# thilinarmtb/lsbench

Hardware: AMD Instinct MI355X
Metric: cg_solves_per_sec (higher is better)
Workload: dtype f64

## Files before the change

### include/lsbench_hip.h

```cpp
#ifndef LSBENCH_HIP_H
#define LSBENCH_HIP_H

#include "lsbench.h"
#include <stddef.h>

#ifdef __cplusplus
extern "C" {
#endif


struct lsbench {
  char *matrix;
  lsbench_solver_t solver;
  lsbench_ordering_t ordering;
  lsbench_precision_t precision;
  unsigned verbose, trials;
};

struct csr {
  unsigned nrows, base;
  unsigned *offs, *cols;
  double *vals;
};

// ... 200 lines not shown
void lsb_amg_free(struct lsb_amg_hier *h);
#define LSB_AMG_MCGS_COLOURS 16
int *lsb_amg_colour(const struct csr *A, unsigned *ncolours);
struct lsb_mcgs {
  unsigned n, ncolours;
  unsigned *cbeg;
  unsigned *rowid;
  unsigned *offs;
  unsigned *cols;
  double *vals;
};
struct lsb_mcgs *lsb_csr_mcgs(const struct csr *A, const int *colour, unsigned ncolours);
void lsb_mcgs_free(struct lsb_mcgs *M);
int lsb_mcgs_check(const struct csr *A, const int *colour, const struct lsb_mcgs *M, char *why, size_t whylen);
unsigned long long *lsb_csr_pack_f32(const struct csr *A);
#define LSB_SELL_ROWS 128
struct lsb_sell {
  unsigned nrows, nslice;
  unsigned long long stored;
  unsigned *sptr;
  int *cols;
  double *vals;
  short *codes;
  int *sbase;
  unsigned ncode_slots;
};
unsigned long long lsb_csr_sell_stored(const struct csr *A);
struct lsb_sell *lsb_csr_sellize(const struct csr *A);
struct lsb_sell *lsb_csr_sellize16(const struct csr *A, unsigned row_begin);
void lsb_sell_free(struct lsb_sell *S);
struct lsb_sell_vc {
  unsigned long long nslots;
  unsigned nval_slots;
  int *slots;
  double *vconst;
  double *vals;
};
struct lsb_sell_vc *lsb_sell16_value_slots(const struct lsb_sell *S);
void lsb_sell_vc_free(struct lsb_sell_vc *V);
#define LSB_TMPL_SLOTS 8
struct lsb_sell_tmpl {
  int nslots;
  int shaped;
  int base[LSB_TMPL_SLOTS];
  int kidx[LSB_TMPL_SLOTS];
  int kind[LSB_TMPL_SLOTS];
  int pad_[2];
  double cst[LSB_TMPL_SLOTS];
};
struct lsb_sell_tmpls {
  unsigned nslice, ntmpl, nfar;
  unsigned long long covered, shaped;
  unsigned long long nmask;
  unsigned long long kept_read;
  unsigned char *tid;
  unsigned *vbase;
  unsigned long long *mask;
  struct lsb_sell_tmpl *t;
};
struct lsb_sell_tmpls *lsb_sell16_templates(const struct lsb_sell *S, const struct lsb_sell_vc *V);
void lsb_sell_tmpls_free(struct lsb_sell_tmpls *T);
int lsb_tmpl_check(const struct lsb_sell *S, const struct lsb_sell_vc *V, const struct lsb_sell_tmpls *T,
                   unsigned row_begin, unsigned nrows, unsigned xlen, int deep, char *why, size_t whylen);
#define LSB_TMPL_COL_MAX 16
#define LSB_TMPL_COL_GRID(nfar) ((nfar) >= 2 ? 768u : 1280u)
#define LSB_TMPL_COL_TURN(nfar) (4u * LSB_TMPL_COL_GRID(nfar) / 8u)
#define LSB_SELL_GRID 1536u
#define LSB_TMPL_COL_DOWN 9
#define LSB_TMPL_COL_LOCKSTEP 0x80000000u
struct lsb_tmpl_cols {
  unsigned nitem, kmax, period;
  unsigned s_lo, s_hi;
  unsigned xbeg[9];
  unsigned *item;
  unsigned long long in_cols;
  int centre0;
  unsigned *down;
};
struct lsb_tmpl_cols *lsb_sell_tmpl_columns(const struct lsb_sell_tmpls *T, unsigned period, unsigned kmax);
struct lsb_tmpl_cols *lsb_sell_tmpl_columns_range(const struct lsb_sell_tmpls *T, unsigned period, unsigned kmax,
                                                  unsigned s_lo, unsigned s_hi);
void lsb_tmpl_cols_free(struct lsb_tmpl_cols *C);
int lsb_tmpl_cols_check(const struct lsb_sell_tmpls *T, const struct lsb_tmpl_cols *C, char *why, size_t whylen);
double lsb_csr_mean_scatter(const struct csr *A, unsigned row_begin);
void lsb_csr_col_hull(const struct csr *A, unsigned *lo, unsigned *hi);
struct lsb_xfer {
  int peer;
  size_t offset, count;
};
void lsb_plan_exchange(int me, int nall, const unsigned *hull,
                       struct lsb_xfer *recv, int *nrecv,
                       struct lsb_xfer *send, int *nsend);
struct csr *lsbench_matrix_synth(const char *spec, unsigned r0, unsigned r1,
                                 unsigned *n_global);


typedef struct lsb_hip_solver lsb_hip_solver;

lsb_hip_solver *lsb_hip_solver_create(const struct csr *A,
                                      const struct lsb_hip_opts *o);
lsb_hip_solver *lsb_hip_solver_create_dist(const struct csr *A_rows,
                                           unsigned row_begin,
                                           unsigned n_global,
                                           const struct lsb_hip_opts *o);
void lsb_hip_solver_destroy(lsb_hip_solver *s);

int lsb_hip_solver_solve(lsb_hip_solver *s, const double *b, double *x,
                         struct lsb_hip_result *res);
int lsb_hip_solver_solve_dev(lsb_hip_solver *s, const double *d_b, double *d_x,
                             struct lsb_hip_result *res);
int lsb_hip_solver_solve_x0(lsb_hip_solver *s, const double *b, double *x,
                            struct lsb_hip_result *res);
int lsb_hip_solver_solve_x0_dev(lsb_hip_solver *s, const double *d_b, double *d_x,
                                struct lsb_hip_result *res);
int lsb_hip_solver_start_relres(const lsb_hip_solver *s, unsigned nrhs, double *out);
int lsb_hip_solver_spmv_dev(lsb_hip_solver *s, const double *d_x, double *d_y);
int lsb_hip_solver_spmv_inner_dev(lsb_hip_solver *s, const double *d_x, double *d_y, double *d_dot);
int lsb_hip_solver_precond_dev(lsb_hip_solver *s, const double *d_r, double *d_z);
int lsb_hip_solver_amg_info(lsb_hip_solver *s, unsigned *levels, unsigned *tail_levels);
int lsb_hip_solver_amg_cheb_interval(lsb_hip_solver *s, unsigned level, double *lo, double *hi);
int lsb_hip_solver_amg_colours(lsb_hip_solver *s, unsigned level, unsigned *ncolours);
int lsb_hip_solver_amg_precision(lsb_hip_solver *s);
unsigned long long lsb_hip_solver_amg_cycle_bytes(const lsb_hip_solver *s);
int lsb_hip_solver_direct_info(const lsb_hip_solver *s, unsigned long long *entries, unsigned *height,
                               unsigned long long *bytes_per_round);
int lsb_hip_solver_cheb_interval(const lsb_hip_solver *s, double *lmin, double *lmax);
int lsb_hip_solver_time_spmv(lsb_hip_solver *s, int warm, int reps,
                             double *ms_avg);
int lsb_hip_solver_jacobi_sweep_dev(lsb_hip_solver *s, double w,
                                    const double *d_b, double *d_x);

int lsb_hip_solver_spmm_dev(lsb_hip_solver *s, unsigned nrhs, const double *d_X, size_t ldx,
                            double *d_Y, size_t ldy);
int lsb_hip_solver_solve_multi_dev(lsb_hip_solver *s, unsigned nrhs, const double *d_B, size_t ldb,
                                   double *d_X, size_t ldx, struct lsb_hip_result *res);
int lsb_hip_solver_solve_multi(lsb_hip_solver *s, unsigned nrhs, const double *B, size_t ldb,
                               double *X, size_t ldx, struct lsb_hip_result *res);
int lsb_hip_solver_solve_multi_x0_dev(lsb_hip_solver *s, unsigned nrhs, const double *d_B, size_t ldb,
                                      double *d_X, size_t ldx, struct lsb_hip_result *res);
unsigned long long lsb_hip_solver_multi_iteration_bytes(const lsb_hip_solver *s, unsigned nrhs);
int lsb_hip_solver_fsai_nnz(const lsb_hip_solver *s, unsigned long long *g, unsigned long long *gt);
int lsb_hip_solver_precond_multi_dev(lsb_hip_solver *s, unsigned nrhs, const double *d_R, size_t ldr,
                                     double *d_Z, size_t ldz);

int lsb_hip_solver_solve_direct_multi_dev(lsb_hip_solver *s, unsigned nrhs, const double *d_B, size_t ldb,
                                          double *d_X, size_t ldx, struct lsb_hip_result *res);
int lsb_hip_solver_solve_direct_multi(lsb_hip_solver *s, unsigned nrhs, const double *B, size_t ldb,
                                      double *X, size_t ldx, struct lsb_hip_result *res);
int lsb_hip_solver_direct_apply_multi_dev(lsb_hip_solver *s, unsigned nrhs, const double *d_R, size_t ldr,
                                          double *d_Z, size_t ldz);
unsigned long long lsb_hip_solver_direct_multi_round_bytes(const lsb_hip_solver *s, unsigned nrhs);

int lsb_hip_solver_amg_solve_multi_dev(lsb_hip_solver *s, unsigned nrhs, const double *d_B, size_t ldb,
                                       double *d_X, size_t ldx, struct lsb_hip_result *res);
int lsb_hip_solver_amg_solve_multi(lsb_hip_solver *s, unsigned nrhs, const double *B, size_t ldb,
                                   double *X, size_t ldx, struct lsb_hip_result *res);
int lsb_hip_solver_amg_cycle_multi_dev(lsb_hip_solver *s, unsigned nrhs, const double *d_R, size_t ldr,
                                       double *d_Z, size_t ldz);
unsigned long long lsb_hip_solver_amg_solve_multi_bytes(const lsb_hip_solver *s, unsigned nrhs);

int lsb_hip_solver_solve_block_dev(lsb_hip_solver *s, unsigned nrhs, const double *d_B, size_t ldb,
                                   double *d_X, size_t ldx, struct lsb_hip_result *res);
int lsb_hip_solver_solve_block(lsb_hip_solver *s, unsigned nrhs, const double *B, size_t ldb,
                               double *X, size_t ldx, struct lsb_hip_result *res);
unsigned long long lsb_hip_solver_block_iteration_bytes(const lsb_hip_solver *s, unsigned nrhs);
int lsb_hip_solver_block_norms(const lsb_hip_solver *s, unsigned nrhs, double *rr, double *bb);
// ... 79 lines not shown
```

### lsbench_amd/_lib.py

```python
import ctypes as C
import os
import subprocess

_CSRC = os.path.join(os.path.dirname(os.path.abspath(__file__)), "csrc")
LIB_PATH = os.path.join(_CSRC, "liblsbench_hip.so")
CORE_PATH = os.path.join(_CSRC, "liblsbench_core.so")
CORE_SYMBOLS = ("lsbench_matrix_read", "lsbench_matrix_print", "lsbench_matrix_free", "lsbench_init",
                "lsbench_get_matrix_name", "lsbench_bench", "lsbench_finalize")

UNIQUE_ID_BYTES = 128

SOLVER_HIP = 6
OP_CHOLMOD_UPPER, OP_RAW = 0, 1
PRECOND_JACOBI, PRECOND_NONE, PRECOND_L1JACOBI, PRECOND_CHEBYSHEV, PRECOND_BLOCKJACOBI, PRECOND_FSAI = 0, 1, 2, 3, 4, 5
PRECOND_AMG = 6
AMG_SMOOTH_L1JACOBI, AMG_SMOOTH_CHEB, AMG_SMOOTH_MCGS = 0, 1, 2
AMG_PREC_FP64, AMG_PREC_FP32 = 0, 1
KRYLOV_PCG, KRYLOV_GMRES, KRYLOV_PCG1, KRYLOV_AUTO, KRYLOV_BICGSTAB, KRYLOV_RICHARDSON = 0, 1, 2, 3, 4, 5
KRYLOV_DIRECT = 6
DIRECT_MAX_ENTRIES = 1 << 28
SPMV_AUTO, SPMV_ADAPTIVE, SPMV_SUBWAVE, SPMV_SCALAR, SPMV_PANEL, SPMV_SELL, SPMV_BINNED, SPMV_TWOPHASE = 0, 1, 2, 3, 4, 5, 6, 7
SELL_ROWS = 128
BIN_CHUNK = 2048
PB_COLS, PB_ROWS = 8192, 2048
# ... 33 lines not shown
                ("amg_theta", C.c_double), ("amg_sweeps", C.c_int), ("amg_coarse", C.c_int),
                ("amg_max_levels", C.c_int), ("amg_tail_rows", C.c_int),
                ("amg_precision", C.c_int),
                ("amg_smoother", C.c_int), ("amg_cheb_ratio", C.c_double)]
    _TAIL = {"fsai_blocks": (0, C.c_int)}
    _TAIL_BYTES = 8

    def __init__(self, *args, **kw):
        super().__init__(*args, **kw)
        C.resize(self, C.sizeof(type(self)) + self._TAIL_BYTES)
        C.memset(C.addressof(self) + C.sizeof(type(self)), 0, self._TAIL_BYTES)

    def _tail(self, name):
        off, ctype = self._TAIL[name]
        return ctype.from_address(C.addressof(self) + C.sizeof(type(self)) + off)

    fsai_blocks = property(lambda self: self._tail("fsai_blocks").value,
                           lambda self, v: setattr(self._tail("fsai_blocks"), "value", v))


class Result(C.Structure):
    _fields_ = [("iters", C.c_uint), ("status", C.c_int), ("relres", C.c_double),
                ("seconds", C.c_double), ("spmv_ms", C.c_double),
                ("spmv_samples", C.c_uint), ("corrections", C.c_uint),
                ("true_relres", C.c_double), ("spmvs", C.c_uint)]


class PanelCsr(C.Structure):
    _fields_ = [("npanels", C.c_uint), ("width", C.c_uint), ("npairs", C.c_uint),
                ("nrows", C.c_uint), ("pair_begin", C.POINTER(C.c_uint)),
                ("pair_row", C.POINTER(C.c_uint)), ("offs", C.POINTER(C.c_uint)),
                ("cols", C.POINTER(C.c_uint)), ("vals", C.POINTER(C.c_double))]


class Sell(C.Structure):
    _fields_ = [("nrows", C.c_uint), ("nslice", C.c_uint), ("stored", C.c_ulonglong),
                ("sptr", C.POINTER(C.c_uint)), ("cols", C.POINTER(C.c_int)),
                ("vals", C.POINTER(C.c_double)), ("codes", C.POINTER(C.c_short)),
                ("sbase", C.POINTER(C.c_int)), ("ncode_slots", C.c_uint)]


class SellVc(C.Structure):
    _fields_ = [("nslots", C.c_ulonglong), ("nval_slots", C.c_uint), ("slots", C.POINTER(C.c_int)),
                ("vconst", C.POINTER(C.c_double)), ("vals", C.POINTER(C.c_double))]


class FsaiPattern(C.Structure):
    _fields_ = [("n", C.c_uint), ("cap", C.c_uint), ("nnz", C.c_ulonglong), ("offs", C.POINTER(C.c_uint)),
                ("cols", C.POINTER(C.c_uint))]


class AmgLevel(C.Structure):
    _fields_ = [("n", C.c_uint), ("A", C.POINTER(CsrStruct)), ("P", C.POINTER(CsrStruct)),
                ("R", C.POINTER(CsrStruct))]


class AmgHier(C.Structure):
    _fields_ = [("nlev", C.c_uint), ("lv", C.POINTER(AmgLevel)), ("nc", C.c_uint),
                ("coarse_inv", C.POINTER(C.c_double))]


class Mcgs(C.Structure):
    _fields_ = [("n", C.c_uint), ("ncolours", C.c_uint), ("cbeg", C.POINTER(C.c_uint)),
                ("rowid", C.POINTER(C.c_uint)), ("offs", C.POINTER(C.c_uint)), ("cols", C.POINTER(C.c_uint)),
                ("vals", C.POINTER(C.c_double))]


class Skyinv(C.Structure):
    _fields_ = [("n", C.c_uint), ("perm", C.POINTER(C.c_uint)), ("first", C.POINTER(C.c_uint)),
                ("woff", C.POINTER(C.c_ulonglong)), ("vals", C.POINTER(C.c_double)),
                ("parent", C.POINTER(C.c_uint)), ("run_end", C.POINTER(C.c_uint))]


class SellTmpl(C.Structure):
    _fields_ = [("nslots", C.c_int), ("shaped", C.c_int), ("base", C.c_int * 8), ("kidx", C.c_int * 8),
                ("kind", C.c_int * 8), ("pad_", C.c_int * 2), ("cst", C.c_double * 8)]


class SellTmpls(C.Structure):
    _fields_ = [("nslice", C.c_uint), ("ntmpl", C.c_uint), ("nfar", C.c_uint), ("covered", C.c_ulonglong),
                ("shaped", C.c_ulonglong), ("nmask", C.c_ulonglong), ("kept_read", C.c_ulonglong),
                ("tid", C.POINTER(C.c_ubyte)), ("vbase", C.POINTER(C.c_uint)),
                ("mask", C.POINTER(C.c_ulonglong)), ("t", C.POINTER(SellTmpl))]


class TmplCols(C.Structure):
    _fields_ = [("nitem", C.c_uint), ("kmax", C.c_uint), ("period", C.c_uint), ("s_lo", C.c_uint), ("s_hi", C.c_uint),
                ("xbeg", C.c_uint * 9),
                ("item", C.POINTER(C.c_uint)), ("in_cols", C.c_ulonglong), ("centre0", C.c_int),
                ("down", C.POINTER(C.c_uint))]


class Binned(C.Structure):
    _fields_ = [("nbins", C.c_uint), ("width", C.c_uint), ("nrows", C.c_uint), ("nchunks", C.c_uint),
                ("chunk_cap", C.c_uint), ("nnz", C.c_ulonglong), ("bin_chunk", C.POINTER(C.c_uint)),
                ("chunk_begin", C.POINTER(C.c_uint)), ("rows", C.POINTER(C.c_uint)),
                ("cols", C.POINTER(C.c_uint)), ("vals", C.POINTER(C.c_double))]


class Pb(C.Structure):
    _fields_ = [("nrows", C.c_uint), ("ncols_lo", C.c_uint), ("nchunks", C.c_uint), ("nbins", C.c_uint),
                ("nitems", C.c_uint), ("npieces", C.c_uint), ("cols", C.c_uint), ("rows", C.c_uint),
                ("nnz", C.c_ulonglong), ("nent", C.c_ulonglong),
                ("vals", C.POINTER(C.c_double)), ("colw", C.POINTER(C.c_ushort)),
                ("grp_first", C.POINTER(C.c_uint)), ("grp_mask", C.POINTER(C.c_ulonglong)),
                ("delta", C.POINTER(C.c_uint)), ("item", C.POINTER(C.c_uint)),
                ("bin_ptr", C.POINTER(C.c_uint)), ("roww", C.POINTER(C.c_ushort))]


class Xfer(C.Structure):
    _fields_ = [("peer", C.c_int), ("offset", C.c_size_t), ("count", C.c_size_t)]


_vp, _u, _i, _d = C.c_void_p, C.c_uint, C.c_int, C.c_double
_csrp = C.POINTER(CsrStruct)

SIGNATURES = {
    "lsbench_matrix_read": (_csrp, [C.c_char_p]),
    "lsbench_matrix_print": (None, [_csrp]),
    "lsbench_matrix_free": (None, [_csrp]),
    "lsbench_init": (C.POINTER(LsbenchStruct), [_i, C.POINTER(C.c_char_p)]),
    "lsbench_get_matrix_name": (C.c_char_p, [C.POINTER(LsbenchStruct)]),
    "lsbench_bench": (None, [_csrp, C.POINTER(LsbenchStruct)]),
    "lsbench_finalize": (None, [C.POINTER(LsbenchStruct)]),
    "hip_cdna4_init": (_i, []),
    "hip_cdna4_finalize": (_i, []),
    "hip_cdna4_bench": (_i, [C.POINTER(C.c_double), _csrp, C.POINTER(C.c_double),
                             C.POINTER(LsbenchStruct)]),
    "lsb_hip_opts_default": (None, [C.POINTER(Opts)]),
    "lsb_hip_set_opts": (None, [C.POINTER(Opts)]),
    "lsb_hip_get_opts": (None, [C.POINTER(Opts)]),
    "lsb_hip_last_result": (None, [C.POINTER(Result)]),
    "lsb_hip_device_count": (_i, []),
    "lsb_csr_free": (None, [_csrp]),
    "lsb_csr_symmetrize_upper": (_csrp, [_csrp]),
    "lsb_csr_copy_base0": (_csrp, [_csrp]),
    "lsb_csr_row_slice": (_csrp, [_csrp, _u, _u]),
    "lsb_csr_partition_rows": (_i, [_csrp, _u, C.POINTER(_u)]),
    "lsb_csr_row_blocks": (_u, [_csrp, _u, C.POINTER(C.POINTER(_u))]),
    "lsb_csr_block_lanes": (None, [_csrp, C.POINTER(_u), _u, C.POINTER(C.c_ubyte)]),
    "lsb_csr_rcm": (_i, [_csrp, C.POINTER(_u)]),
    "lsb_csr_nd": (_i, [_csrp, C.POINTER(_u)]),
    "lsb_csr_nd_bounded": (_i, [_csrp, C.POINTER(_u), C.c_ulonglong, C.POINTER(C.c_ulonglong)]),
    "lsb_csr_skyline_count": (C.c_ulonglong, [_csrp, C.POINTER(_u), C.POINTER(_u)]),
    "lsb_csr_skyline_inverse": (C.POINTER(Skyinv), [_csrp, C.POINTER(_u), C.POINTER(_i)]),
    "lsb_skyinv_free": (None, [C.POINTER(Skyinv)]),
    "lsb_csr_permute_sym": (_csrp, [_csrp, C.POINTER(_u)]),
    "lsb_csr_bandwidth": (_u, [_csrp]),
    "lsb_csr_panelize": (C.POINTER(PanelCsr), [_csrp, _u]),
    "lsb_panel_csr_free": (None, [C.POINTER(PanelCsr)]),
    "lsb_csr_pbize": (C.POINTER(Pb), [_csrp]),
    "lsb_csr_pbize2": (C.POINTER(Pb), [_csrp, _u, _u]),
    "lsb_pb_free": (None, [C.POINTER(Pb)]),
    "lsb_pb_check": (_i, [C.POINTER(Pb), C.c_ulonglong, C.c_ulonglong, _i, C.c_char_p, C.c_size_t]),
    "lsb_csr_binize": (C.POINTER(Binned), [_csrp, _u]),
    "lsb_binned_free": (None, [C.POINTER(Binned)]),
    "lsb_csr_sell_stored": (C.c_ulonglong, [_csrp]),
    "lsb_csr_sellize": (C.POINTER(Sell), [_csrp]),
    "lsb_csr_sellize16": (C.POINTER(Sell), [_csrp, _u]),
    "lsb_sell_free": (None, [C.POINTER(Sell)]),
    "lsb_sell16_value_slots": (C.POINTER(SellVc), [C.POINTER(Sell)]),
    "lsb_sell_vc_free": (None, [C.POINTER(SellVc)]),
    "lsb_csr_fsai_pattern": (C.POINTER(FsaiPattern), [_csrp, _i, _u]),
    "lsb_fsai_pattern_free": (None, [C.POINTER(FsaiPattern)]),
    "lsb_amg_setup": (C.POINTER(AmgHier), [_csrp, _d, _u, _u]),
    "lsb_amg_aggregate": (C.POINTER(C.c_int), [_csrp, _d, C.POINTER(_u)]),
    "lsb_amg_free": (None, [C.POINTER(AmgHier)]),
    "lsb_amg_gershgorin": (_d, [_csrp]),
    "lsb_csr_pack_f32": (C.POINTER(C.c_ulonglong), [_csrp]),
    "lsb_amg_cheb_coeffs": (None, [_d, _d, _u, C.POINTER(_d), C.POINTER(_d)]),
    "lsb_amg_colour": (C.POINTER(C.c_int), [_csrp, C.POINTER(_u)]),
    "lsb_csr_mcgs": (C.POINTER(Mcgs), [_csrp, C.POINTER(C.c_int), _u]),
    "lsb_mcgs_free": (None, [C.POINTER(Mcgs)]),
    "lsb_mcgs_check": (_i, [_csrp, C.POINTER(C.c_int), C.POINTER(Mcgs), C.c_char_p, C.c_size_t]),
    "lsb_sell16_templates": (C.POINTER(SellTmpls), [C.POINTER(Sell), C.POINTER(SellVc)]),
    "lsb_sell_tmpls_free": (None, [C.POINTER(SellTmpls)]),
    "lsb_tmpl_check": (_i, [C.POINTER(Sell), C.POINTER(SellVc), C.POINTER(SellTmpls), _u, _u, _u, _i,
                            C.c_char_p, C.c_size_t]),
    "lsb_sell_tmpl_columns": (C.POINTER(TmplCols), [C.POINTER(SellTmpls), _u, _u]),
    "lsb_sell_tmpl_columns_range": (C.POINTER(TmplCols), [C.POINTER(SellTmpls), _u, _u, _u, _u]),
    "lsb_tmpl_cols_free": (None, [C.POINTER(TmplCols)]),
    "lsb_tmpl_cols_check": (_i, [C.POINTER(SellTmpls), C.POINTER(TmplCols), C.c_char_p, C.c_size_t]),
    "lsb_csr_mean_scatter": (_d, [_csrp, _u]),
    "lsb_csr_col_hull": (None, [_csrp, C.POINTER(_u), C.POINTER(_u)]),
    "lsb_plan_exchange": (None, [_i, _i, C.POINTER(_u), C.POINTER(Xfer), C.POINTER(_i),
                                 C.POINTER(Xfer), C.POINTER(_i)]),
    "lsbench_matrix_synth": (_csrp, [C.c_char_p, _u, _u, C.POINTER(_u)]),
    "lsb_hip_solver_create": (_vp, [_csrp, C.POINTER(Opts)]),
    "lsb_hip_solver_create_dist": (_vp, [_csrp, _u, _u, C.POINTER(Opts)]),
    "lsb_hip_solver_destroy": (None, [_vp]),
    "lsb_hip_solver_solve": (_i, [_vp, _vp, _vp, C.POINTER(Result)]),
    "lsb_hip_solver_solve_dev": (_i, [_vp, _vp, _vp, C.POINTER(Result)]),
    "lsb_hip_solver_solve_x0": (_i, [_vp, _vp, _vp, C.POINTER(Result)]),
    "lsb_hip_solver_solve_x0_dev": (_i, [_vp, _vp, _vp, C.POINTER(Result)]),
    "lsb_hip_solver_start_relres": (_i, [_vp, _u, C.POINTER(C.c_double)]),
    "lsb_hip_solver_spmv_dev": (_i, [_vp, _vp, _vp]),
    "lsb_hip_solver_spmv_inner_dev": (_i, [_vp, _vp, _vp, _vp]),
    "lsb_hip_solver_spmm_dev": (_i, [_vp, _u, _vp, C.c_size_t, _vp, C.c_size_t]),
    "lsb_hip_solver_solve_multi_dev": (_i, [_vp, _u, _vp, C.c_size_t, _vp, C.c_size_t, C.POINTER(Result)]),
    "lsb_hip_solver_solve_multi": (_i, [_vp, _u, _vp, C.c_size_t, _vp, C.c_size_t, C.POINTER(Result)]),
    "lsb_hip_solver_solve_multi_x0_dev": (_i, [_vp, _u, _vp, C.c_size_t, _vp, C.c_size_t, C.POINTER(Result)]),
    "lsb_hip_solver_multi_iteration_bytes": (C.c_ulonglong, [_vp, _u]),
    "lsb_hip_solver_solve_block_dev": (_i, [_vp, _u, _vp, C.c_size_t, _vp, C.c_size_t, C.POINTER(Result)]),
    "lsb_hip_solver_solve_block": (_i, [_vp, _u, _vp, C.c_size_t, _vp, C.c_size_t, C.POINTER(Result)]),
    "lsb_hip_solver_block_iteration_bytes": (C.c_ulonglong, [_vp, _u]),
    "lsb_hip_solver_block_norms": (_i, [_vp, _u, C.POINTER(C.c_double), C.POINTER(C.c_double)]),
    "lsb_hip_solver_solve_block_precond_dev": (_i, [_vp, _u, _vp, C.c_size_t, _vp, C.c_size_t, C.POINTER(Result)]),
    "lsb_hip_solver_solve_block_precond": (_i, [_vp, _u, _vp, C.c_size_t, _vp, C.c_size_t, C.POINTER(Result)]),
    "lsb_hip_solver_block_precond_iteration_bytes": (C.c_ulonglong, [_vp, _u]),
    "lsb_hip_solver_precond_multi_dev": (_i, [_vp, _u, _vp, C.c_size_t, _vp, C.c_size_t]),
    "lsb_hip_solver_fsai_nnz": (_i, [_vp, C.POINTER(C.c_ulonglong), C.POINTER(C.c_ulonglong)]),
    "lsb_hip_solver_precond_dev": (_i, [_vp, _vp, _vp]),
    "lsb_hip_solver_amg_info": (_i, [_vp, C.POINTER(_u), C.POINTER(_u)]),
    "lsb_hip_solver_amg_precision": (_i, [_vp]),
    "lsb_hip_solver_amg_cycle_bytes": (C.c_ulonglong, [_vp]),
    "lsb_hip_solver_direct_info": (_i, [_vp, C.POINTER(C.c_ulonglong), C.POINTER(_u), C.POINTER(C.c_ulonglong)]),
    "lsb_hip_solver_solve_direct_multi_dev": (_i, [_vp, _u, _vp, C.c_size_t, _vp, C.c_size_t, C.POINTER(Result)]),
    "lsb_hip_solver_solve_direct_multi": (_i, [_vp, _u, _vp, C.c_size_t, _vp, C.c_size_t, C.POINTER(Result)]),
    "lsb_hip_solver_direct_apply_multi_dev": (_i, [_vp, _u, _vp, C.c_size_t, _vp, C.c_size_t]),
    "lsb_hip_solver_direct_multi_round_bytes": (C.c_ulonglong, [_vp, _u]),
    "lsb_hip_solver_amg_solve_multi_dev": (_i, [_vp, _u, _vp, C.c_size_t, _vp, C.c_size_t, C.POINTER(Result)]),
    "lsb_hip_solver_amg_solve_multi": (_i, [_vp, _u, _vp, C.c_size_t, _vp, C.c_size_t, C.POINTER(Result)]),
    "lsb_hip_solver_amg_cycle_multi_dev": (_i, [_vp, _u, _vp, C.c_size_t, _vp, C.c_size_t]),
    "lsb_hip_solver_amg_solve_multi_bytes": (C.c_ulonglong, [_vp, _u]),
    "lsb_hip_solver_amg_cheb_interval": (_i, [_vp, _u, C.POINTER(_d), C.POINTER(_d)]),
    "lsb_hip_solver_amg_colours": (_i, [_vp, _u, C.POINTER(_u)]),
    "lsb_hip_solver_cheb_interval": (_i, [_vp, C.POINTER(_d), C.POINTER(_d)]),
    "lsb_hip_solver_time_spmv": (_i, [_vp, _i, _i, C.POINTER(_d)]),
    "lsb_hip_solver_jacobi_sweep_dev": (_i, [_vp, _d, _vp, _vp]),
    "lsb_hip_solver_nrows_local": (_u, [_vp]),
    "lsb_hip_solver_padded": (_i, [_vp]),
    "lsb_hip_solver_slab_mask": (_u, [_vp]),
    "lsb_csr_pad_lines": (_csrp, [_csrp, _u, C.POINTER(_u), C.POINTER(_u), C.POINTER(C.POINTER(C.c_int))]),
    "lsb_hip_solver_nrows_global": (_u, [_vp]),
    "lsb_hip_solver_nnz_local": (C.c_ulonglong, [_vp]),
    "lsb_hip_solver_nblocks": (_u, [_vp]),
    "lsb_hip_solver_spmv_variant": (_i, [_vp]),
    "lsb_hip_solver_spmv_flags": (_u, [_vp]),
    "lsb_hip_solver_spmv_grid": (_u, [_vp]),
    "lsb_hip_solver_spmv_period": (_u, [_vp]),
    "lsb_hip_solver_spmv_col_slices": (C.c_ulonglong, [_vp]),
    "lsb_hip_solver_sell_value_slots": (None, [_vp, C.POINTER(C.c_uint), C.POINTER(C.c_uint)]),
    "lsb_hip_solver_overlaps": (_i, [_vp]),
    "lsb_hip_solver_overlap": (_i, [_vp, C.POINTER(C.c_double)]),
    "lsb_hip_solver_comm_plan": (None, [_vp, C.POINTER(C.c_ulonglong)]),
    "lsb_hip_solver_spmv_layout_bytes": (C.c_ulonglong, [_vp]),
    "lsb_hip_solver_fused_p": (_i, [_vp]),
    "lsb_hip_solver_iteration_bytes": (C.c_ulonglong, [_vp]),
    "lsb_hip_solver_single_reduction": (_i, [_vp]),
    "lsb_hip_solver_blas1_nt": (_i, [_vp]),
    "lsb_hip_solver_comm": (_i, [_vp, C.POINTER(C.c_double), C.POINTER(C.c_double)]),
    "lsb_hip_stream": (_vp, []),
    "lsb_hip_comm_get_unique_id": (_i, [_vp]),
    "lsb_hip_comm_init_rank": (_i, [_vp, _i, _i]),
    "lsb_hip_comm_destroy": (_i, []),
    "lsb_hip_comm_rank": (_i, []),
    "lsb_hip_comm_size": (_i, []),
    "lsb_hip_comm_count": (_i, []),
    "hip_cdna4_set_option": (_i, [C.c_char_p, C.c_char_p]),
    "hip_cdna4_matrix_synth": (_csrp, [C.c_char_p]),
    "lsb_hip_comm_allreduce_sum_dev": (_i, [_vp, _i]),
    "lsb_hip_comm_barrier": (_i, []),
    "lsb_hip_spmv_csr_f64": (_i, [_i, _u, _vp, _vp, _vp, _vp, _vp, _u, _u, _u, _vp, _vp,
                                  _vp, _vp, _vp, _vp]),
    "lsb_hip_partials_capacity": (_u, []),
    "lsb_hip_dot_f64": (_i, [_u, _vp, _vp, _vp, _vp, _vp]),
    "lsb_hip_nrm2_f64": (_i, [_u, _vp, _vp, _vp, _vp]),
    "lsb_hip_axpy_f64": (_i, [_u, _vp, _vp, _vp, _vp]),
    "lsb_hip_xpay_f64": (_i, [_u, _vp, _vp, _vp, _vp]),
    "lsb_hip_jacobi_setup_f64": (_i, [_u, _u, _vp, _vp, _vp, _vp, _vp, _vp]),
    "lsb_hip_jacobi_apply_f64": (_i, [_u, _vp, _vp, _vp, _vp]),
    "lsb_hip_malloc": (_vp, [C.c_size_t]),
    "lsb_hip_free": (None, [_vp]),
    "lsb_hip_memcpy_h2d": (_i, [_vp, _vp, C.c_size_t]),
    "lsb_hip_memcpy_d2h": (_i, [_vp, _vp, C.c_size_t]),
    "lsb_hip_sync": (_i, []),
}

_LIB = None


def build(force=False):
    if force:
        subprocess.run(["make", "-s", "-C", _CSRC, "clean"], check=True)
    subprocess.run(["make", "-s", "-C", _CSRC, "all"], check=True)


def libc_free(ptr):
    libc = C.CDLL(None)
    libc.free.argtypes, libc.free.restype = [C.c_void_p], None
    libc.free(C.cast(ptr, C.c_void_p))


def load():
    global _LIB
    if _LIB is not None:
        return _LIB
    try:
        import torch
    except Exception:
        pass
    if not os.path.exists(LIB_PATH):
        raise LsbenchHipError(
            "%s not built: run `make -C lsbench_amd/csrc` or __graft_entry__.build(); "
            "there is no fallback path" % LIB_PATH)
    hip = C.CDLL(LIB_PATH, mode=C.RTLD_GLOBAL)
    core = C.CDLL(CORE_PATH, mode=C.RTLD_GLOBAL)

    class _Both:
        pass
    lib = _Both()
    lib.hip, lib.core = hip, core
    for name, (res, args) in SIGNATURES.items():
        fn = getattr(core if name in CORE_SYMBOLS else hip, name)
        fn.restype, fn.argtypes = res, args
        setattr(lib, name, fn)
# ... 11 lines not shown
```

### lsbench_amd/csrc/hip_kernels.hip

```cpp
#include "hip_kcommon.h"

__device__ __forceinline__ void spmv_publish(double *__restrict__ partials, double dot,
                                             double *sred, const lsb_ar_tail &tail) {
  if (!partials)
    return;
  double d[1] = {dot};
  wg_sum<1>(d, sred);
  if (tail.counter)
    ar_tail(partials, d[0], tail);
  else if (threadIdx.x == 0)
    partials[blockIdx.x] = d[0];
}

enum { SP_PREFETCH = 1, SP_NT = 2 };

template <int FLAGS, class T>
__device__ __forceinline__ T stream_load(const T *p) {
  if (FLAGS & SP_NT)
    return __builtin_nontemporal_load(p);
  return *p;
}

#define LSB_ISSUE_BLOCK(kk)                                                    \
  do {                                                                         \
// ... 1272 lines not shown
      const lsb_sell_tmpl *T = td + t;
      col_tmpl<NF> C;
      C.bc = T->base[NF + 1];
      C.k0 = T->cst[0], C.kc = T->cst[NF + 1], C.kL = T->cst[2 * NF + 2];
#pragma unroll
      for (int k = 0; k < NF - 1; k++) {
        C.bl[k] = T->base[1 + k], C.bh[k] = T->base[NF + 3 + k];
        C.kl[k] = T->cst[1 + k], C.kh[k] = T->cst[NF + 3 + k];
      }
      const int side_k[2] = {T->kidx[NF], T->kidx[NF + 2]}, side_kd[2] = {T->kind[NF], T->kind[NF + 2]};
      const bool down = col_walks_down(plan, dofs, it);
      const unsigned s0 = down ? s + (K - 1) * period : s;
      const long long D = down ? -(long long)P : (long long)P;
      const unsigned Du = (unsigned)D;
      long long gu = (long long)s0 * LSB_SELL_ROWS;
      unsigned lrow = s0 * LSB_SELL_ROWS;
      col_ops<NF> cur, nxt;
      sell_d2u cb = *(const sell_d2u *)(p + (gu + C.bc - D) + 2 * lane);
      sell_d2u c0 = *(const sell_d2u *)(p + (gu + C.bc) + 2 * lane);
      sell_d2u ca, cn;
      col_issue<NF, 2>(cur, ca, C, p, r, gu, lrow, D, n, lane, true);
      unsigned long long mk[2][2] = {{0ull, 0ull}, {0ull, 0ull}};
#pragma unroll
      for (int side = 0; side < 2; side++)
        if (side_k[side] >= 0 && side_kd[side] == 2) {
          const unsigned long long *mp = mask + 2 * ((size_t)mb + (unsigned)side_k[side]);
          mk[side][0] = mp[0], mk[side][1] = mp[1];
        }
      double vm0 = T->cst[NF], vm1 = vm0, vp0 = T->cst[NF + 2], vp1 = vp0;
      if (side_k[0] >= 0 || side_k[1] >= 0)
        tmpl_side_values(T, NF, 0u, lane, side_k, side_kd, mk, vals, 0, vm0, vm1, vp0, vp1);
      for (unsigned k = 0; k + 1 < K; k++) {
        col_issue<NF, 2>(nxt, cn, C, p, r, gu + D, lrow + Du, D, n, lane, true);
        double a0, a1;
        col_compute<NF, 0>(cur, down ? ca : cb, c0, down ? cb : ca, C, vm0, vm1, vp0, vp1, lane, a0, a1, nodot);
        COLR_FINISH(a0, a1, cur.xd, lrow);
        cb = c0, c0 = ca, ca = cn, cur = nxt;
        gu += D, lrow += Du;
      }
      double a0, a1;
      col_compute<NF, 0>(cur, down ? ca : cb, c0, down ? cb : ca, C, vm0, vm1, vp0, vp1, lane, a0, a1, nodot);
      COLR_FINISH(a0, a1, cur.xd, lrow);
    } else {
      for (unsigned k = 0; k < K; k++) {
        const unsigned sl = s + k * period, row = sl * LSB_SELL_ROWS + 2 * lane;
        const unsigned q0 = sptr[sl] / LSB_SELL_ROWS, len = (sptr[sl + 1] - sptr[sl]) / LSB_SELL_ROWS;
        const bool l0 = row < n, l1 = row + 1 < n;
        const double r0 = l0 ? r[row] : 0.0, r1 = l1 ? r[row + 1] : 0.0;
        double a0 = 0.0, a1 = 0.0;
        for (unsigned j = 0; j < len; j++) {
          const i4v rec2 = ((const i4v *)sbase)[q0 + j];
          if (rec2.z < 0) {
            const double kk = vconst[q0 + j];
            const sell_d2u pv = *(const sell_d2u *)(p + ((int)row + rec2.x));
            a0 = fma(kk, pv.x, a0), a1 = fma(kk, pv.y, a1);
          } else {
            const sell_d2v v = *((const sell_d2v *)(vals + (size_t)rec2.z * LSB_SELL_ROWS) + lane);
            const bool p0 = v.x != 0.0, p1 = v.y != 0.0;
            const double t0 = p[p0 ? (int)row + rec2.x : 0], t1 = p[p1 ? (int)row + 1 + rec2.x : 0];
            a0 = fma(v.x, p0 ? t0 : 0.0, a0), a1 = fma(v.y, p1 ? t1 : 0.0, a1);
          }
        }
        if (l0) {
          const double rn0 = r0 - alpha * a0;
          r[row] = rn0;
          acc[0] += rn0 * (dc * rn0), acc[1] += rn0 * rn0;
        }
        if (l1) {
          const double rn1 = r1 - alpha * a1;
          r[row + 1] = rn1;
          acc[0] += rn1 * (dc * rn1), acc[1] += rn1 * rn1;
        }
      }
    }
  }
#undef COLR_FINISH
  wg_sum<2>(acc, sred);
  if (threadIdx.x == 0) {
    partials2[2 * blockIdx.x + 0] = acc[0];
    partials2[2 * blockIdx.x + 1] = acc[1];
  }
}


__device__ __forceinline__ unsigned bin_pad(unsigned i) { return i + (i >> 3); }

template <int FLAGS, int BIN_U>
__global__ __launch_bounds__(WG) void k_spmv_binned(
    const unsigned *__restrict__ chunk_begin, unsigned nchunk, const unsigned *__restrict__ rows,
    const unsigned *__restrict__ cols, const double *__restrict__ vals,
    const double *__restrict__ x, double *__restrict__ y, const lsb_pcg_state *__restrict__ st) {
  constexpr unsigned CHUNK = BIN_U * WG;
  __shared__ double sprod[CHUNK + CHUNK / 8 + 8];
  __shared__ unsigned skey[CHUNK + CHUNK / 8 + 8];
  __shared__ double swv[4];
  __shared__ int swf[4];
  __shared__ double sred[4];
  const unsigned tid = threadIdx.x, lane = tid & 63u, wave = tid >> 6;
  const unsigned per = gridDim.x / NXCD;
  const unsigned w = (blockIdx.x % NXCD) * per + blockIdx.x / NXCD;
  if (w >= nchunk)
    return;
  const unsigned e0 = chunk_begin[w], cnt = chunk_begin[w + 1] - e0;
  unsigned r[BIN_U], c[BIN_U];
  double v[BIN_U];
  if (cnt <= CHUNK) {
#pragma unroll
    for (int u = 0; u < BIN_U; u++) {
      const unsigned t = tid + u * WG;
      if (t < cnt) {
        r[u] = stream_load<FLAGS>(rows + e0 + t);
        c[u] = stream_load<FLAGS>(cols + e0 + t);
        v[u] = stream_load<FLAGS>(vals + e0 + t);
      }
    }
  }
  if (st && st->status)
    return;
  if (cnt > CHUNK) {
    double s[1] = {0.0};
    for (unsigned j = e0 + tid; j < e0 + cnt; j += WG)
      s[0] += vals[j] * x[cols[j]];
    wg_sum<1>(s, sred);
    if (tid == 0)
      y[rows[e0]] += s[0];
    return;
  }
#pragma unroll
  for (int u = 0; u < BIN_U; u++) {
    const unsigned t = tid + u * WG;
    if (t < cnt) {
      double xv;
      if (FLAGS & 8)
        xv = __hip_atomic_load(x + c[u], __ATOMIC_RELAXED, __HIP_MEMORY_SCOPE_AGENT);
      else if (FLAGS & 16)
        xv = __builtin_nontemporal_load(x + c[u]);
      else
        xv = x[c[u]];
      sprod[bin_pad(t)] = v[u] * xv;
      skey[bin_pad(t)] = r[u];
    }
  }
  __syncthreads();
  const unsigned i0 = tid * BIN_U;
  const int nloc = i0 < cnt ? (int)min(cnt - i0, (unsigned)BIN_U) : 0;
  double first_sum = 0.0, acc = 0.0;
  unsigned first_key = 0, prevk = 0xFFFFFFFFu, nextk = 0xFFFFFFFEu;
  bool cont = false, has_boundary = false, closes = true;
  unsigned ok_[BIN_U];
  double ov[BIN_U];
  unsigned omask = 0;
  if (nloc > 0) {
    if (i0 > 0)
      prevk = skey[bin_pad(i0 - 1)];
    if (i0 + BIN_U < cnt)
      nextk = skey[bin_pad(i0 + BIN_U)];
    unsigned k[BIN_U + 1];
    double p[BIN_U];
#pragma unroll
    for (int j = 0; j < BIN_U; j++) {
      k[j] = j < nloc ? skey[bin_pad(i0 + j)] : 0u;
      p[j] = j < nloc ? sprod[bin_pad(i0 + j)] : 0.0;
    }
    cont = k[0] == prevk;
    first_key = k[0];
#pragma unroll
// ... 214 lines not shown
      if (epi.zout)
        kern = nt ? k_spmv_sell16<SP_NT, VT, true> : k_spmv_sell16<0, VT, true>;
      kern<<<L.g, WG, 0, s>>>(sptr, s0, ns, L.period, n, row_begin, xlen, (const short *)cols, sbase, v, vconst,
                              ulen, x, y, xdot, partials, st, L.tail, epi);
    } else {
      const auto kern = nt ? k_spmv_sell<SP_NT, VT> : k_spmv_sell<0, VT>;
      kern<<<L.g, WG, 0, s>>>(sptr, s0, ns, L.period, n, (const int *)cols, v, x, y, xdot, partials, st, L.tail);
    }
  };
  if (flags & LSB_SP_F32)
    launch((const float *)(const void *)vals);
  else
    launch(vals);
}

void lsb_k_spmv_tmpl(unsigned flags, unsigned grid_cap, unsigned period, const struct lsb_sell16_dev *c, unsigned s0,
                     unsigned ns, unsigned n, unsigned row_begin, unsigned xlen, const double *x, double *y,
                     const double *xdot, double *partials, unsigned *npartials, const struct lsb_pcg_state *st,
                     const struct lsb_ar_tail *tail_in, const struct lsb_cheb_epi *epi_in, void *stream) {
  const lsb_cheb_epi epi = epi_for(epi_in, partials || ((row_begin | s0) & 1u),
                                   "lsb_k_spmv_tmpl: the Chebyshev epilogue takes no dot and even row offsets");
  const sell_launch L = sell_prologue("lsb_k_spmv_tmpl", false, c, ns, n, grid_cap, 0, period, partials, npartials,
                                      tail_in);
  const int f32 = (flags & LSB_SP_F32) != 0, dot_is_x = xdot && xdot == x + row_begin;
  static decltype(&k_spmv_tmpl<0, false>) const kern[3][3] = {
      {k_spmv_tmpl<0, false>, k_spmv_tmpl<0, true>, k_spmv_tmpl<0, false, true>},
      {k_spmv_tmpl<1, false>, k_spmv_tmpl<1, true>, k_spmv_tmpl<1, false, true>},
      {k_spmv_tmpl<2, false>, k_spmv_tmpl<2, true>, k_spmv_tmpl<2, false, true>}};
  const int form = epi.zout ? 1 : (flags & LSB_SP_DEFER) ? 2 : 0;
  kern[c->tmpl.nfar][form]<<<L.g, WG, 0, (hipStream_t)stream>>>(
      c->sptr, s0, ns, L.period, n, row_begin, xlen, (const u4v *)c->tmpl.srec, c->tmpl.mask, c->tmpl.td, c->sbase,
      c->vals, f32, c->vconst, x, y, xdot, dot_is_x, partials, st, L.tail, epi);
}

void lsb_k_spmv_tmpl_col(unsigned flags, unsigned grid_cap, unsigned period, const unsigned *plan, unsigned nitem,
                         int centre0, unsigned n, unsigned row_begin, unsigned xlen, const struct lsb_sell16_dev *c,
                         const double *x, double *y, const double *xdot, double *partials, unsigned *npartials,
                         const struct lsb_pcg_state *st, const struct lsb_ar_tail *tail_in, void *stream) {
  if (period < NXCD || !plan)
    errx(EXIT_FAILURE, "lsb_k_spmv_tmpl_col: no column plan (period %u)", period);
  const sell_launch L = sell_prologue("lsb_k_spmv_tmpl_col", true, c, nitem, n, grid_cap, 0, period, partials,
                                      npartials, tail_in);
  const int f32 = (flags & LSB_SP_F32) != 0;
  const int dot = !partials || !xdot ? 0 : (xdot == x + row_begin && centre0) ? 1 : 2;
  static decltype(&k_spmv_tmpl_col<1, 0>) const kern[2][3] = {
      {k_spmv_tmpl_col<1, 0>, k_spmv_tmpl_col<1, 1>, k_spmv_tmpl_col<1, 2>},
      {k_spmv_tmpl_col<2, 0>, k_spmv_tmpl_col<2, 1>, k_spmv_tmpl_col<2, 2>}};
  kern[c->tmpl.nfar - 1][dot]<<<L.g, WG, 0, (hipStream_t)stream>>>(
      plan, L.period, n, row_begin, xlen, c->sptr, c->tmpl.mask, c->tmpl.td, c->sbase, c->vals, f32, c->vconst, x, y,
      xdot, partials, st, L.tail);
}

void lsb_k_pcg_col_px(unsigned grid_cap, unsigned period, const unsigned *plan, unsigned nitem, unsigned n,
                      const struct lsb_sell16_dev *c, const double *r, const double *pold, double *pnew, double *x,
                      int xupd, double dc, double *partials, unsigned *npartials, struct lsb_pcg_state *st, int parity,
                      const double *parts2, unsigned nparts2, void *stream) {
  if (period < NXCD || !plan || pold == pnew)
    errx(EXIT_FAILURE, "lsb_k_pcg_col_px: no column plan (period %u) or one direction buffer", period);
  const unsigned nfar = c->tmpl.nfar;
  const sell_launch L = sell_prologue("lsb_k_pcg_col_px", true, c, nitem, n, grid_cap, LSB_TMPL_COL_GRID(nfar), period,
                                      partials, npartials, NULL);
  static decltype(&k_pcg_col_px<1, 3, false>) const kern[2][2] = {
      {k_pcg_col_px<1, 3, false>, k_pcg_col_px<1, 3, true>},
      {k_pcg_col_px<2, 3, false>, k_pcg_col_px<2, 3, true>}};
  kern[nfar - 1][xupd != 0]<<<L.g, WG, 0, (hipStream_t)stream>>>(
      plan, L.period, n, c->sptr, c->tmpl.mask, c->tmpl.td, c->sbase, c->vals, c->vconst, r, pold, pnew, x, dc,
      partials, st, parity, parts2, nparts2);
}

void lsb_k_pcg_col_r(unsigned grid_cap, unsigned period, const unsigned *plan, unsigned nitem, unsigned n,
                     const struct lsb_sell16_dev *c, const double *p, double *r, double dc, struct lsb_pcg_state *st,
                     int parity, int pbuf, int xtwo, int rev, const double *pq_parts, unsigned npq, double *partials2,
                     unsigned *npartials, void *stream) {
  if (period < NXCD || !plan)
    errx(EXIT_FAILURE, "lsb_k_pcg_col_r: no column plan (period %u)", period);
  const sell_launch L = sell_prologue("lsb_k_pcg_col_r", true, c, nitem, n, grid_cap, LSB_TMPL_COL_GRID(1), period,
                                      partials2, npartials, NULL);
  const auto kern = c->tmpl.nfar == 1 ? k_pcg_col_r<1> : k_pcg_col_r<2>;
  kern<<<L.g, WG, 0, (hipStream_t)stream>>>(plan, L.period, n, c->sptr, c->tmpl.mask, c->tmpl.td, c->sbase, c->vals,
                                            c->vconst, p, r, dc, st, parity, pbuf, xtwo, rev != 0, pq_parts, npq,
                                            partials2);
}

}
```

### lsbench_amd/csrc/hip_pcg.c

```c
#define _GNU_SOURCE
#include "hip_solver.h"

enum pcg_form pcg_choose_form(const lsb_hip_solver *sv) {
  const struct shard *s = &sv->sh[0];
  const struct lsb_hip_opts *o = &sv->o;
  if (o->krylov == LSB_KRYLOV_GMRES || o->krylov == LSB_KRYLOV_BICGSTAB || o->krylov == LSB_KRYLOV_RICHARDSON ||
      o->krylov == LSB_KRYLOV_DIRECT)
    return PCG_NONE;
  if (o->precond == LSB_PRECOND_FSAI && !sv->multi && !s->mixed && s->variant == LSB_SPMV_SUBWAVE &&
      s->fs_g.variant == LSB_SPMV_SUBWAVE && s->fs_gt.variant == LSB_SPMV_SUBWAVE && o->sample_spmv <= 0 &&
      o->krylov != LSB_KRYLOV_PCG1 && !getenv("LSBENCH_HIP_NO_FSAI_FUSE"))
    return PCG_FSAI3;
  if (generic_precond(sv))
    return PCG_GENERIC;
  if (o->krylov == LSB_KRYLOV_PCG1 || (o->krylov == LSB_KRYLOV_AUTO && sv->multi))
    return PCG_CG1;
  if (sv->multi || s->mixed || getenv("LSBENCH_HIP_NO_FUSE_P"))
    return PCG_CLASSIC;
  if (s->sell_form == SELL_COL && s->dinv_uniform && s->c16.tmpl.nfar >= 1 && s->c16.tmpl.nfar <= 2 &&
      s->row_begin == 0 && s->n == s->n_glob && o->precond == LSB_PRECOND_JACOBI && !getenv("LSBENCH_HIP_NO_FUSE_PX"))
    return PCG_COL;
  return s->variant == LSB_SPMV_SUBWAVE && o->sample_spmv <= 0 ? PCG_SUBWAVE : PCG_CLASSIC;
}

void form_vecs(lsb_hip_solver *sv, enum pcg_form f) {
  for (int i = 0; i < sv->nshard; i++) {
    struct shard *s = &sv->sh[i];
    if (!s->d_p1 && (f == PCG_SUBWAVE || f == PCG_COL || f == PCG_CG1 || f == PCG_FSAI3))
      s->d_p1 = shard_vec(s, s->n);
    if (!s->d_s1 && f == PCG_CG1)
      s->d_s1 = shard_vec(s, s->n);
    if (!s->d_r1 && f == PCG_FSAI3)
      s->d_r1 = shard_vec(s, s->n);
  }
}

void sample_open(lsb_hip_solver *sv, int k) {
  if (k >= 0)
    LSB_CHK_HIP(hipEventRecord(sv->ev[4 * k], g_stream));
}

void sample_close(lsb_hip_solver *sv, int k) {
  for (int e = 1; e < 4 && k >= 0; e++)
    LSB_CHK_HIP(hipEventRecord(sv->ev[4 * k + e], g_stream));
}

static void spmv_pq(lsb_hip_solver *sv, int sample) {
  if (sv->multi) {
    exchange_and_spmv(sv, sample);
    allreduce_pq(sv, 1, 0);
    return;
  }
  struct shard *s = &sv->sh[0];
  sample_open(sv, sample);
  spmv_shard(s, s->d_pfull, s->d_q, s->d_pfull + s->row_begin, s->d_parts_pq, &s->npq, s->d_st);
  sample_close(sv, sample);
}

static void reduce_rz(lsb_hip_solver *sv, int gated) {
  if (!sv->multi)
    return;
  for (int i = 0; i < sv->nshard; i++) {
    struct shard *s = &sv->sh[i];
    lsb_k_reduce_final(s->d_parts2, s->np2, 2, s->d_scal + 1, 0, gated ? s->d_st : NULL, g_stream);
  }
  allreduce_scal(sv, 1, 2, gated);
}

static void init_state(lsb_hip_solver *sv) {
  reduce_rz(sv, 0);
  for (int i = 0; i < sv->nshard; i++) {
    struct shard *s = &sv->sh[i];
    lsb_k_pcg_init_state(s->d_st, sv->multi ? s->d_scal + 1 : s->d_parts2, sv->multi ? 1u : s->np2, sv->tol_run,
                         (int)sv->o.maxit, g_stream);
  }
}

static void classic_enqueue_init(lsb_hip_solver *sv, const double *d_b, double *d_x) {
  for (int i = 0; i < sv->nshard; i++) {
    struct shard *s = &sv->sh[i];
    const size_t o = s->row_begin - sv->row_first;
    lsb_k_pcg_init(s->n, d_b + o, DINV(s), d_x + o, s->d_r, s->d_pfull + s->row_begin, s->d_parts2, &s->np2,
                   g_stream);
  }
  init_state(sv);
}

static void classic_enqueue_iter(lsb_hip_solver *sv, double *d_x, int parity, int sample) {
  spmv_pq(sv, sample);
  for (int i = 0; i < sv->nshard; i++) {
    struct shard *s = &sv->sh[i];
    const size_t o = s->row_begin - sv->row_first;
    lsb_k_pcg_update_xr(s->n, s->d_pfull + s->row_begin, s->d_q, DINV(s), d_x + o, s->d_r, s->d_st, parity,
                        sv->multi ? s->d_scal : s->d_parts_pq, sv->multi ? 1u : s->npq, s->d_parts2, &s->np2,
                        sv->nt_mask, g_stream);
  }
  reduce_rz(sv, 1);
  for (int i = 0; i < sv->nshard; i++) {
    struct shard *s = &sv->sh[i];
    lsb_k_pcg_update_p(s->n, s->d_r, DINV(s), s->d_pfull + s->row_begin, s->d_pfull + s->row_begin, s->d_st,
                       parity, sv->multi ? s->d_scal + 1 : s->d_parts2, sv->multi ? 1u : s->np2, sv->nt_mask, g_stream);
  }
// ... 16 lines not shown
    lsb_k_dot2(s->n, s->d_r, s->d_z, s->d_parts2, &s->np2, NULL, g_stream);
  }
  init_state(sv);
}

static void gen_enqueue_iter(lsb_hip_solver *sv, double *d_x, int parity, int sample) {
  spmv_pq(sv, sample);
  for (int i = 0; i < sv->nshard; i++) {
    struct shard *s = &sv->sh[i];
    const size_t o = s->row_begin - sv->row_first;
    lsb_k_pcg_update_xr(s->n, s->d_pfull + s->row_begin, s->d_q, NULL, 1.0, d_x + o, s->d_r, s->d_st,
                        parity, sv->multi ? s->d_scal : s->d_parts_pq, sv->multi ? 1u : s->npq,
                        s->d_parts2, &s->np2, sv->nt_mask, g_stream);
  }
  precond_apply(sv, 1);
  for (int i = 0; i < sv->nshard; i++) {
    struct shard *s = &sv->sh[i];
    lsb_k_dot2(s->n, s->d_r, s->d_z, s->d_parts2, &s->np2, s->d_st, g_stream);
  }
  reduce_rz(sv, 1);
  for (int i = 0; i < sv->nshard; i++) {
    struct shard *s = &sv->sh[i];
    lsb_k_pcg_update_p(s->n, s->d_z, NULL, 1.0, s->d_pfull + s->row_begin, s->d_pfull + s->row_begin,
                       s->d_st, parity, sv->multi ? s->d_scal + 1 : s->d_parts2,
                       sv->multi ? 1u : s->np2, sv->nt_mask, g_stream);
  }
}

static void fsai_enqueue_iter(lsb_hip_solver *sv, double *d_x, int parity, int pos) {
  struct shard *s = &sv->sh[0];
  double *pb[2] = {s->d_pfull, s->d_p1}, *rb[2] = {s->d_r, s->d_r1};
  if (pos & 1) {
    sv->pcur = 0, sv->rcur = 0;
    spmv_shard(s, pb[0], s->d_q, pb[0], s->d_parts_pq, &s->npq, s->d_st);
  } else {
    lsb_k_spmv_subwave_p(s->n, s->csr.offs, s->csr.cols, s->csr.vals, s->lanes, s->d_z, NULL, 1.0, pb[sv->pcur],
                         pb[sv->pcur ^ 1], s->d_q, s->d_parts_pq, &s->npq, s->d_st, parity ^ 1, s->d_parts2,
                         s->np2, g_stream);
    sv->pcur ^= 1;
  }
  lsb_k_fsai_xr_gr(s->n, s->fs_g.offs, s->fs_g.cols, s->fs_g.vals, s->fs_g.lanes, pb[sv->pcur], s->d_q, d_x,
                   rb[sv->rcur], rb[sv->rcur ^ 1], s->d_fst, s->d_st, parity, s->d_parts_pq, s->npq, g_stream);
  sv->rcur ^= 1;
  lsb_k_fsai_gt_dots(s->n, s->fs_gt.offs, s->fs_gt.cols, s->fs_gt.vals, s->fs_gt.lanes, s->d_fst, s->d_z,
                     rb[sv->rcur], s->d_parts2, &s->np2, s->d_st, g_stream);
  if (pos & 2) {
    lsb_k_pcg_update_p(s->n, s->d_z, NULL, 1.0, pb[sv->pcur], pb[0], s->d_st, parity, s->d_parts2, s->np2,
                       sv->nt_mask, g_stream);
    if (sv->rcur)
      LSB_CHK_HIP(hipMemcpyAsync(s->d_r, s->d_r1, (size_t)s->n * sizeof(double), hipMemcpyDeviceToDevice,
                                 g_stream));
  }
}

static void subwave_enqueue_iter(lsb_hip_solver *sv, double *d_x, int parity, int pos) {
  struct shard *s = &sv->sh[0];
  double *buf[2] = {s->d_pfull, s->d_p1};
  if (pos & 1) {
    sv->pcur = 0;
    spmv_shard(s, buf[0], s->d_q, buf[0], s->d_parts_pq, &s->npq, s->d_st);
  } else {
    lsb_k_spmv_subwave_p(s->n, s->csr.offs, s->csr.cols, s->csr.vals, s->lanes, s->d_r, DINV(s),
                         buf[sv->pcur], buf[sv->pcur ^ 1], s->d_q, s->d_parts_pq, &s->npq, s->d_st,
                         parity ^ 1, s->d_parts2, s->np2, g_stream);
    sv->pcur ^= 1;
  }
  lsb_k_pcg_update_xr(s->n, buf[sv->pcur], s->d_q, DINV(s), d_x, s->d_r, s->d_st, parity,
                      s->d_parts_pq, s->npq, s->d_parts2, &s->np2, sv->nt_mask, g_stream);
  if (pos & 2)
    lsb_k_pcg_update_p(s->n, s->d_r, DINV(s), buf[sv->pcur], buf[0], s->d_st, parity, s->d_parts2,
                       s->np2, sv->nt_mask, g_stream);
}

static void col_enqueue_iter(lsb_hip_solver *sv, double *d_x, int parity, int pos, int sample) {
  struct shard *s = &sv->sh[0];
  double *buf[2] = {s->d_pfull, s->d_p1};
  if (sample >= 0)
    sv->samp_skip[sample] = (pos & 1) != 0;
  if (pos & 1) {
    sv->pcur = 0;
    spmv_shard(s, buf[0], s->d_q, buf[0], s->d_parts_pq, &s->npq, s->d_st);
  } else {
    sample_open(sv, sample);
    lsb_k_pcg_col_px(s->sp_grid, s->col.period, s->col.plan, s->col.items, s->n, &s->c16, s->d_r, buf[sv->pcur],
                     buf[sv->pcur ^ 1], d_x,  parity == 0,
                     s->dinv_const, s->d_parts_pq, &s->npq, s->d_st, parity ^ 1, s->d_parts2, s->np2, g_stream);
    sample_close(sv, sample);
    sv->pcur ^= 1;
  }
  lsb_k_pcg_col_r(s->sp_grid, s->col.period, s->col.plan, s->col.items, s->n, &s->c16, buf[sv->pcur], s->d_r,
                  s->dinv_const, s->d_st,
                  parity, sv->pcur,  parity != 0,  1,
                  s->d_parts_pq, s->npq, s->d_parts2, &s->np2, g_stream);
  if (pos & 2) {
    lsb_k_pcg_xfix(s->n, buf[0], buf[1], d_x, s->d_st, g_stream);
    lsb_k_pcg_update_p(s->n, s->d_r, DINV(s), buf[sv->pcur], buf[0], s->d_st, parity, s->d_parts2, s->np2,
                       sv->nt_mask, g_stream);
  }
}

static void cg1_enqueue_init(lsb_hip_solver *sv, const double *d_b, double *d_x) {
  sv->ar_fold = can_fold_allreduce(sv), sv->ar_pending = 0, sv->fold_next = 0;
  for (int i = 0; i < sv->nshard; i++) {
    struct shard *s = &sv->sh[i];
    const size_t o = s->row_begin - sv->row_first, bytes = (size_t)s->n * sizeof(double);
    if (sv->cg1_implicit)
      lsb_k_pcg_init(s->n, d_b + o, DINV(s), d_x + o, s->d_pfull + s->row_begin, s->d_r,
                     s->d_parts2, &s->np2, g_stream);
    else
      lsb_k_pcg_init(s->n, d_b + o, DINV(s), d_x + o, s->d_r, s->d_pfull + s->row_begin,
                     s->d_parts2, &s->np2, g_stream);
    LSB_CHK_HIP(hipMemsetAsync(s->d_p1, 0, bytes, g_stream));
    LSB_CHK_HIP(hipMemsetAsync(s->d_s1, 0, bytes, g_stream));
  }
  init_state(sv);
  spmv_pq(sv, -1);
}

static void cg1_enqueue_iter(lsb_hip_solver *sv, double *d_x, int parity, int sample) {
  for (int i = 0; i < sv->nshard; i++) {
    struct shard *s = &sv->sh[i];
    const size_t o = s->row_begin - sv->row_first;
    double *gr_in = s->d_parts2 + (size_t)parity * 2 * LSB_MAX_PARTIALS;
    double *gr_out = s->d_parts2 + (size_t)(parity ^ 1) * 2 * LSB_MAX_PARTIALS;
    unsigned np2 = 0;
    struct lsb_ar_collect col;
    if (sv->ar_pending)
      lsb_p2p_fold_collect(sv->p2p[i], &col);
    lsb_k_cg1_update(s->n, sv->cg1_implicit ? NULL : s->d_pfull + s->row_begin, s->d_q, DINV(s),
                     s->d_p1, s->d_s1, d_x + o,
                     sv->cg1_implicit ? s->d_pfull + s->row_begin : s->d_r, s->d_st, parity,
                     sv->multi ? s->d_scal + 1 : gr_in,
                     sv->multi ? 1u : s->np2, sv->multi ? s->d_scal : s->d_parts_pq,
                     sv->multi ? 1u : s->npq, sv->ar_pending ? &col : NULL, gr_out, &np2, sv->nt_mask, g_stream);
    s->ar2_parts = gr_out, s->ar2_n = np2, s->ar2_width = 2;
  }
  if (sv->multi) {
    sv->fold_next = sv->ar_fold == 2;
    exchange_and_spmv(sv, sample);
  } else {
    struct shard *s = &sv->sh[0];
    sample_open(sv, sample);
    spmv_shard(s, s->d_pfull, s->d_q, s->d_pfull + s->row_begin, s->d_parts_pq, &s->npq, s->d_st);
    sample_close(sv, sample);
  }
  if (sv->multi && sv->ar_fold) {
    if (sv->ar_fold == 1)
      allreduce_pq_contribute(sv);
    sv->ar_pending = 1;
  } else if (sv->multi)
    allreduce_pq(sv, 3, 1);
}

static void pcg_enqueue_init(lsb_hip_solver *sv, enum pcg_form form, const double *d_b, double *d_x) {
  form_vecs(sv, sv->form);
  switch (form) {
  case PCG_CG1:
    cg1_enqueue_init(sv, d_b, d_x);
    break;
  case PCG_GENERIC:
  case PCG_FSAI3:
    gen_enqueue_init(sv, d_b, d_x);
    break;
  default:
    classic_enqueue_init(sv, d_b, d_x);
  }
}

static void pcg_enqueue_iter(lsb_hip_solver *sv, enum pcg_form form, double *d_x, int parity, int sample, int pos) {
  switch (form) {
  case PCG_FSAI3:
    fsai_enqueue_iter(sv, d_x, parity, pos);
    break;
  case PCG_GENERIC:
    gen_enqueue_iter(sv, d_x, parity, sample);
    break;
// ... 329 lines not shown
```

### lsbench_amd/csrc/hip_solver.c

```c
#define _GNU_SOURCE
#include "hip_solver.h"
#define NXCD_HOST 8u

void choose_spmv(struct shard *s, const struct lsb_hip_opts *o) {
  const unsigned mean = s->n ? (unsigned)((s->nnz + s->n - 1) / s->n) : 1;
  int v = o->spmv_variant;
  if (v == LSB_SPMV_AUTO)
    v = s->nnz <= 500000ull ? LSB_SPMV_SUBWAVE : LSB_SPMV_ADAPTIVE;
  if (v == LSB_SPMV_PANEL && !s->panel.n)
    v = LSB_SPMV_ADAPTIVE;
  if (v == LSB_SPMV_BINNED && !s->bins.n)
    v = LSB_SPMV_ADAPTIVE;
  if (v == LSB_SPMV_TWOPHASE && !s->tp.bins)
    v = LSB_SPMV_ADAPTIVE;
  if (v == LSB_SPMV_SELL && !s->sell.sptr)
    v = LSB_SPMV_ADAPTIVE;
  s->variant = v;
  s->lanes = row_lanes(mean);
}

static float *upload_f32(const double *v, size_t cnt, int *exact) {
  float *f = (float *)malloc((cnt ? cnt : 1) * sizeof(float));
  if (!f)
    errx(EXIT_FAILURE, "hip_cdna4: out of host memory for the fp32 matrix values");
// ... 191 lines not shown
}

static struct lsb_sell *c16_build(struct shard *s, const struct csr *G, struct lsb_sell_vc **vc) {
  struct lsb_sell16_dev *c = &s->c16;
  struct lsb_sell *H = getenv("LSBENCH_HIP_NO_C16") ? NULL : lsb_csr_sellize16(G, s->row_begin);
  if (H && H->stored > s->nnz + s->nnz / 8)
    lsb_sell_free(H), H = NULL;
  if (!H)
    return NULL;
  c->sptr = (unsigned *)dev_upload(H->sptr, ((size_t)H->nslice + 1) * sizeof(unsigned));
  c->codes = (short *)dev_upload(H->codes, ((size_t)H->ncode_slots + 1) * LSB_SELL_ROWS * sizeof(short));
  c->ulen = H->nslice ? (H->sptr[1] - H->sptr[0]) / LSB_SELL_ROWS : 0;
  for (unsigned k = 0; k < H->nslice && c->ulen; k++)
    if ((H->sptr[k + 1] - H->sptr[k]) / LSB_SELL_ROWS != c->ulen)
      c->ulen = 0;
  struct lsb_sell_vc *V = getenv("LSBENCH_HIP_NO_VCONST") ? NULL : lsb_sell16_value_slots(H);
  if (V && (unsigned long long)V->nval_slots * 8 > V->nslots * 7)
    lsb_sell_vc_free(V), V = NULL;
  if (V) {
    const size_t nv = ((size_t)V->nval_slots + 1) * LSB_SELL_ROWS;
    if (s->mixed)
      for (unsigned long long q = 0; q < V->nslots; q++)
        V->vconst[q] = (double)(float)V->vconst[q];
    c->sbase = (int *)dev_upload(V->slots, 4 * ((size_t)V->nslots + 1) * sizeof(int));
    c->vconst = (double *)dev_upload(V->vconst, ((size_t)V->nslots + 1) * sizeof(double));
    c->vals = s->mixed ? (double *)upload_f32(V->vals, nv, NULL) : (double *)dev_upload(V->vals, nv * sizeof(double));
    c->vslots = V->nval_slots, c->slots = (unsigned)V->nslots;
    c->bytes = (unsigned long long)V->nslots * 24;
  } else {
    c->sbase = (int *)dev_upload(H->sbase, 2 * ((size_t)H->stored / LSB_SELL_ROWS + 1) * sizeof(int));
    c->vals = s->mixed ? (double *)upload_f32(H->vals, (size_t)H->stored + LSB_SELL_ROWS, NULL)
                       : (double *)dev_upload(H->vals, ((size_t)H->stored + LSB_SELL_ROWS) * sizeof(double));
    c->vslots = c->slots = (unsigned)(H->stored / LSB_SELL_ROWS);
    c->bytes = (unsigned long long)c->slots * 8;
  }
  c->bytes += (unsigned long long)H->ncode_slots * LSB_SELL_ROWS * sizeof(short) +
              (unsigned long long)c->vslots * LSB_SELL_ROWS * (s->mixed ? 4 : 8) +
              (c->ulen ? 0ull : ((unsigned long long)H->nslice + 1) * 4);
  *vc = V;
  return H;
}
static void tmpl_free(struct lsb_tmpl_dev *t) {
  lsb_hip_free(t->srec), lsb_hip_free(t->td), lsb_hip_free(t->mask);
  memset(t, 0, sizeof *t);
}
static void c16_free(struct lsb_sell16_dev *c) {
  lsb_hip_free(c->sptr), lsb_hip_free(c->codes), lsb_hip_free(c->sbase), lsb_hip_free(c->vals);
  lsb_hip_free(c->vconst), tmpl_free(&c->tmpl);
  memset(c, 0, sizeof *c);
}

static struct lsb_sell_tmpls *tmpl_build(struct shard *s, struct lsb_sell *H, struct lsb_sell_vc *V) {
  struct lsb_tmpl_dev *t = &s->c16.tmpl;
  struct lsb_sell_tmpls *TT = getenv("LSBENCH_HIP_NO_TMPL") ? NULL : lsb_sell16_templates(H, V);
  {
    char why[256];
    if (lsb_tmpl_check(H, V, TT, s->row_begin, s->n, s->n_glob, 0, why, sizeof why))
      errx(EXIT_FAILURE, "hip_cdna4: sliced-ELL layout breaks a bound its kernels rely on: %s", why);
  }
  if (!TT)
    return NULL;
  if (s->mixed)
    for (unsigned k = 0; k < TT->ntmpl; k++)
      for (int j = 0; j < TT->t[k].nslots; j++)
        TT->t[k].cst[j] = (double)(float)TT->t[k].cst[j];
  unsigned *rec = lsb_calloc(unsigned, 4 * ((size_t)TT->nslice + 1));
  for (unsigned k = 0; k < TT->nslice; k++)
    rec[4 * (size_t)k] = TT->tid[k], rec[4 * (size_t)k + 1] = TT->vbase[2 * (size_t)k],
                   rec[4 * (size_t)k + 2] = TT->vbase[2 * (size_t)k + 1];
  t->srec = (unsigned *)dev_upload(rec, 4 * ((size_t)TT->nslice + 1) * sizeof(unsigned));
  LSB_CHK_HIP(hipStreamSynchronize(g_stream));
  free(rec);
  t->mask = (unsigned long long *)dev_upload(TT->mask, 2 * ((size_t)TT->nmask + 1) * sizeof(unsigned long long));
  t->td = (struct lsb_sell_tmpl *)dev_upload(TT->t, (size_t)TT->ntmpl * sizeof(struct lsb_sell_tmpl));
  t->nfar = TT->nfar;
  t->bytes = 16ull * TT->nslice + (unsigned long long)TT->ntmpl * sizeof(struct lsb_sell_tmpl) + 16ull * TT->nmask +
             TT->kept_read * LSB_SELL_ROWS * (s->mixed ? 4ull : 8ull);
  for (unsigned k = 0; k < H->nslice; k++)
    if (TT->tid[k] == 255)
      t->bytes += (unsigned long long)(H->sptr[k + 1] - H->sptr[k]) / LSB_SELL_ROWS * 24 + 8;
  return TT;
}

static void col_build(struct shard *s, const struct lsb_sell *H, const struct lsb_sell_vc *V,
                      const struct lsb_sell_tmpls *TT) {
  struct shard_col *c = &s->col;
  if (!c->period || getenv("LSBENCH_HIP_NO_COL"))
    return;
  const char *ek = getenv("LSBENCH_HIP_COL_K");
  unsigned kauto = TT->nfar >= 2 ? TT->nslice / 5120u : TT->nslice / 15000u;
  kauto = kauto < 4u ? 4u : kauto > 16u ? 16u : kauto;
  const unsigned kmax = ek ? (unsigned)atoi(ek) : kauto;
  for (int w = 0; w < 2; w++) {
    if (w == 1 && !(c->plan && s->sell.split.ok && (s->sell.split.first > 0 || s->sell.split.last < TT->nslice)))
      break;
    struct lsb_tmpl_cols *CC = w == 0 ? lsb_sell_tmpl_columns(TT, c->period, kmax)
                                      : lsb_sell_tmpl_columns_range(TT, c->period, kmax, s->sell.split.first,
                                                                    s->sell.split.last);
    if (!CC)
      break;
    char why[256];
    if (lsb_tmpl_cols_check(TT, CC, why, sizeof why))
      errx(EXIT_FAILURE, "hip_cdna4: z-column plan breaks a rule its kernel relies on: %s", why);
    const size_t nw = 16 + 4 * ((size_t)CC->nitem + 1), nd = CC->down ? ((size_t)CC->nitem + 31) / 32 : 0;
    unsigned *plan = lsb_calloc(unsigned, nw + nd);
    memcpy(plan, CC->xbeg, sizeof CC->xbeg);
    memcpy(plan + 16, CC->item, 4 * (size_t)CC->nitem * sizeof(unsigned));
    if (nd) {
      plan[LSB_TMPL_COL_DOWN] = (unsigned)nw;
      memcpy(plan + nw, CC->down, nd * sizeof(unsigned));
    }
    unsigned *d = (unsigned *)dev_upload(plan, (nw + nd) * sizeof(unsigned));
    LSB_CHK_HIP(hipStreamSynchronize(g_stream));
    free(plan);
    if (w == 0) {
      c->plan = d, c->items = CC->nitem, c->centre0 = CC->centre0, c->slices = CC->in_cols;
      c->bytes = 16ull * CC->nitem + (unsigned long long)TT->ntmpl * sizeof(struct lsb_sell_tmpl);
      for (unsigned q = 0; q < CC->nitem; q++) {
        const unsigned sl = CC->item[4 * (size_t)q], run = CC->item[4 * (size_t)q + 1] & ~LSB_TMPL_COL_LOCKSTEP;
        if (run >= 2) {
          const struct lsb_sell_tmpl *t = &TT->t[TT->tid[sl]];
          for (int j = 0; j < t->nslots; j++)
            c->bytes += t->kind[j] == 2 ? 16ull : 0ull;
        } else {
          const unsigned q0 = H->sptr[sl] / LSB_SELL_ROWS, len = (H->sptr[sl + 1] - H->sptr[sl]) / LSB_SELL_ROWS;
          c->bytes += 24ull * len + 8;
          for (unsigned j = 0; j < len; j++)
            if (V->slots[4 * ((size_t)q0 + j) + 2] >= 0)
              c->bytes += LSB_SELL_ROWS * (s->mixed ? 4ull : 8ull);
        }
      }
    } else {
      c->plan_in = d, c->items_in = CC->nitem;
      c->centre0 &= CC->centre0;
    }
    lsb_tmpl_cols_free(CC);
  }
}
static void col_free(struct shard_col *c) {
  lsb_hip_free(c->plan), lsb_hip_free(c->plan_in);
  memset(c, 0, sizeof *c);
}

double *shard_vec(struct shard *s, size_t count) {
  const size_t bytes = ((count ? count : 1) * sizeof(double) + 255u) & ~(size_t)255u;
  if (s->d_slab && s->slab_used + bytes <= s->slab_cap) {
    double *p = (double *)(s->d_slab + s->slab_used);
    s->slab_used += bytes;
    return p;
  }
  return (double *)lsb_hip_malloc(bytes);
}
void shard_vec_free(struct shard *s, void *p) {
  if (p && !(s->d_slab && (char *)p >= s->d_slab && (char *)p < s->d_slab + s->slab_cap))
    lsb_hip_free(p);
}

void shard_upload(struct shard *s, const struct csr *S, unsigned r0,
                         unsigned r1, int local, unsigned row_begin,
                         unsigned n_glob, const struct lsb_hip_opts *o) {
  const unsigned a = local ? 0 : r0, b = local ? S->nrows : r1;
  const unsigned n = b - a, j0 = S->offs[a], j1 = S->offs[b];
  const unsigned base = S->base;
  s->row_begin = row_begin, s->n = n, s->nnz = j1 - j0, s->n_glob = n_glob;
  int *offs = (int *)malloc(((size_t)n + 1) * sizeof(int));
  int *cols = (int *)malloc(((size_t)s->nnz + 1) * sizeof(int));
  unsigned lo = 0xFFFFFFFFu, hi = 0;
  for (unsigned i = 0; i <= n; i++)
    offs[i] = (int)(S->offs[a + i] - j0);
  for (unsigned j = j0; j < j1; j++) {
    const unsigned c = S->cols[j] - base;
    if (c >= n_glob)
      errx(EXIT_FAILURE, "column %u outside the %u-column operator", c, n_glob);
    cols[j - j0] = (int)c;
    if (c < lo)
      lo = c;
    if (c + 1 > hi)
      hi = c + 1;
  }
  if (s->nnz == 0)
    lo = hi = row_begin;
  s->col_lo = lo, s->col_hi = hi;
  if ((unsigned long long)s->nnz > 0x7FFFFFFFull || n_glob > 0x7FFFFFFFu)
    errx(EXIT_FAILURE, "shard too large for int32 device indices");
  s->mixed = o->precision == LSB_PREC_MIXED, s->exact32 = 1;
  struct csr G = {n, 0, (unsigned *)offs, (unsigned *)cols, (double *)(S->vals + j0)};
  csr_build(s, &G);
  const char *e = getenv("LSBENCH_HIP_PANEL_COLS");
  const unsigned width = e ? (unsigned)strtoul(e, NULL, 10) : 524288u;
  const int scattered = s->nnz > 4000000ull && (double)(hi - lo) * 8.0 > 16.0e6 &&
                        lsb_csr_mean_scatter(&G, row_begin) > 1.0e6;
  if (width && o->spmv_variant == LSB_SPMV_PANEL)
    panel_build(&s->panel, &G, width);
  if (width && (o->spmv_variant == LSB_SPMV_BINNED || (o->spmv_variant == LSB_SPMV_AUTO && scattered)))
    bins_build(&s->bins, &G, width);
  if (o->spmv_variant == LSB_SPMV_TWOPHASE || (o->spmv_variant == LSB_SPMV_AUTO && scattered))
    tp_build(&s->tp, &G, n_glob);
  sell_build(s, &G, o);
  if (s->sell.sptr) {
    struct lsb_sell_vc *V = NULL;
    struct lsb_sell *H = c16_build(s, &G, &V);
    struct lsb_sell_tmpls *TT = V ? tmpl_build(s, H, V) : NULL;
    if (TT)
      col_build(s, H, V, TT);
    LSB_CHK_HIP(hipStreamSynchronize(g_stream));
    lsb_sell_tmpls_free(TT), lsb_sell_vc_free(V), lsb_sell_free(H);
  }
  precond_shard_blocks(s, offs, cols, S->vals + j0, o);
  LSB_CHK_HIP(hipStreamSynchronize(g_stream));
  free(offs), free(cols);

  const int fused_p = n == n_glob && o->nvirt <= 1 && o->precision == LSB_PREC_FP64 &&
                      o->precond == LSB_PRECOND_JACOBI && (o->krylov == LSB_KRYLOV_PCG || o->krylov == LSB_KRYLOV_AUTO);
  {
    size_t cnt = 3 * (size_t)n + n_glob;
    if (n_glob > n || o->nvirt > 1 || o->krylov == LSB_KRYLOV_PCG1)
      cnt += 2 * (size_t)n;
    if (o->precond == LSB_PRECOND_CHEBYSHEV)
      cnt += 2 * (size_t)n_glob + (size_t)n;
    else if (o->precond == LSB_PRECOND_BLOCKJACOBI)
      cnt += (size_t)n;
    else if (o->precond == LSB_PRECOND_FSAI)
      cnt += 4 * (size_t)n;
    else if (o->precond == LSB_PRECOND_AMG)
      cnt += 3 * (size_t)n;
    if (o->krylov == LSB_KRYLOV_BICGSTAB)
      cnt += 3 * (size_t)n + n_glob;
    if (fused_p)
      cnt += (size_t)n;
    if (s->slab_bx)
      cnt += 2 * (size_t)n;
    if (o->krylov != LSB_KRYLOV_GMRES && !getenv("LSBENCH_HIP_NO_SLAB") && (size_t)n * sizeof(double) <= ((size_t)160 << 20)) {
      s->slab_cap = cnt * sizeof(double) + 16 * 256;
      if (hipMalloc((void **)&s->d_slab, s->slab_cap) != hipSuccess)
        s->d_slab = NULL, s->slab_cap = 0, (void)hipGetLastError();
    }
  }
  s->d_dinv = shard_vec(s, n);
  s->d_r = shard_vec(s, n);
  s->d_q = shard_vec(s, n);
  s->d_pfull = shard_vec(s, n_glob);
  LSB_CHK_HIP(hipMemsetAsync(s->d_pfull, 0, (size_t)n_glob * sizeof(double), g_stream));
  if (fused_p) {
    s->d_p1 = shard_vec(s, n);
    LSB_CHK_HIP(hipMemsetAsync(s->d_p1, 0, (size_t)n * sizeof(double), g_stream));
  }
  s->d_parts_pq = (double *)lsb_hip_malloc(3 * LSB_MAX_PARTIALS * sizeof(double));
  s->d_parts2 = (double *)lsb_hip_malloc(4 * LSB_MAX_PARTIALS * sizeof(double));
  s->d_st = (struct lsb_pcg_state *)lsb_hip_malloc(sizeof(struct lsb_pcg_state));
  LSB_CHK_HIP(hipMemsetAsync(s->d_st, 0, sizeof(struct lsb_pcg_state), g_stream));
  s->d_st_aux = (struct lsb_pcg_state *)lsb_hip_malloc(sizeof(struct lsb_pcg_state));
  LSB_CHK_HIP(hipMemsetAsync(s->d_st_aux, 0, sizeof(struct lsb_pcg_state), g_stream));
  choose_spmv(s, o);

  if (o->precond == LSB_PRECOND_JACOBI || o->precond == LSB_PRECOND_L1JACOBI ||
      o->precond == LSB_PRECOND_CHEBYSHEV) {
    int *d_nz = (int *)lsb_hip_malloc(sizeof(int)), nz = 0;
    LSB_CHK_HIP(hipMemsetAsync(d_nz, 0, sizeof(int), g_stream));
    if (o->precond == LSB_PRECOND_L1JACOBI)
      lsb_k_l1_setup(n, s->csr.offs, s->csr.vals, s->d_dinv, d_nz, g_stream);
    else
      lsb_k_jacobi_setup(n, row_begin, s->csr.offs, s->csr.cols, s->csr.vals, s->d_dinv, d_nz,
                         g_stream);
    LSB_CHK_HIP(hipMemcpyAsync(&nz, d_nz, sizeof(int), hipMemcpyDeviceToHost, g_stream));
    LSB_CHK_HIP(hipStreamSynchronize(g_stream));
    lsb_hip_free(d_nz);
    if (nz)
      errx(EXIT_FAILURE, "hip_cdna4: %d rows have no non-zero %s; "
                         "Jacobi preconditioning needs one (cf. the stored-diagonal "
                         "assumption of src/cholmod-impl.h:13)", nz,
           o->precond == LSB_PRECOND_L1JACOBI ? "entry" : "diagonal entry");
  } else {
    double *ones = (double *)malloc((size_t)(n ? n : 1) * sizeof(double));
    for (unsigned i = 0; i < n; i++)
      ones[i] = 1.0;
    LSB_CHK_HIP(hipMemcpy(s->d_dinv, ones, (size_t)n * sizeof(double), hipMemcpyHostToDevice));
    free(ones);
  }
  if (n && !getenv("LSBENCH_HIP_NO_UNIFORM_DINV")) {
    double *h = (double *)malloc((size_t)n * sizeof(double));
    LSB_CHK_HIP(hipMemcpy(h, s->d_dinv, (size_t)n * sizeof(double), hipMemcpyDeviceToHost));
    int same = 1;
    for (unsigned i = 1; i < n && same; i++)
      same = h[i] == h[0];
    s->dinv_uniform = same, s->dinv_const = h[0];
    free(h);
  }
}

void shard_free(struct shard *s) {
  csr_free(&s->csr), panel_free(&s->panel), bins_free(&s->bins), tp_free(&s->tp);
  sell32_free(&s->sell), c16_free(&s->c16), col_free(&s->col);
  shard_vec_free(s, s->d_dinv), shard_vec_free(s, s->d_r);
  shard_vec_free(s, s->d_q), shard_vec_free(s, s->d_pfull), lsb_hip_free(s->d_parts_pq);
  shard_vec_free(s, s->d_p1), shard_vec_free(s, s->d_s1), shard_vec_free(s, s->d_r1);
  lsb_hip_free(s->d_parts2), lsb_hip_free(s->d_st), lsb_hip_free(s->d_st_aux);
  precond_free_shard(s);
  lsb_hip_free(s->d_slab);
  s->d_slab = NULL;
  free(s->recv), free(s->send);
}

void plan_exchange(struct shard *s, int me, int nall, const unsigned *hull) {
  s->recv = lsb_calloc(struct lsb_xfer, nall);
  s->send = lsb_calloc(struct lsb_xfer, nall);
  lsb_plan_exchange(me, nall, hull, s->recv, &s->nrecv, s->send, &s->nsend);
}

lsb_hip_solver *solver_alloc(int nshard, const struct lsb_hip_opts *o) {
  lsb_hip_solver *sv = lsb_calloc(lsb_hip_solver, 1);
  sv->nshard = nshard;
  sv->sh = lsb_calloc(struct shard, nshard);
  sv->o = *o;
  LSB_CHK_HIP(hipHostMalloc((void **)&sv->h_st, 2 * sizeof(struct lsb_pcg_state), 0));
  return sv;
}

void solver_finish_setup(lsb_hip_solver *sv) {
  sv->d_scal_all = (double *)lsb_hip_malloc((size_t)sv->nshard * SCAL_STRIDE * sizeof(double));
  LSB_CHK_HIP(hipMemsetAsync(sv->d_scal_all, 0,
                             (size_t)sv->nshard * SCAL_STRIDE * sizeof(double), g_stream));
  for (int i = 0; i < sv->nshard; i++)
    sv->sh[i].d_scal = sv->d_scal_all + (size_t)i * SCAL_STRIDE;
  sv->d_tmp = (double *)lsb_hip_malloc((size_t)sv->n_here * sizeof(double));
  for (int i = 0; i < 4 * MAX_SAMPLES; i++)
    LSB_CHK_HIP(hipEventCreate(&sv->ev[i]));
  LSB_CHK_HIP(hipEventCreate(&sv->ev_t0));
  LSB_CHK_HIP(hipEventCreate(&sv->ev_t1));
  LSB_CHK_HIP(hipEventCreateWithFlags(&sv->ev_poll[0], hipEventDisableTiming));
  LSB_CHK_HIP(hipEventCreateWithFlags(&sv->ev_poll[1], hipEventDisableTiming));
  LSB_CHK_HIP(hipEventCreateWithFlags(&sv->ev_vec, hipEventDisableTiming));
  LSB_CHK_HIP(hipEventCreateWithFlags(&sv->ev_halo, hipEventDisableTiming));
  sv->have_events = 1;
  LSB_CHK_HIP(hipStreamSynchronize(g_stream));
  for (int i = 0; i < sv->nshard; i++)
    tune_spmv(sv, &sv->sh[i]);
  LSB_CHK_HIP(hipStreamSynchronize(g_stream));
  {
    const double c = sv->sh[0].dinv_const;
    int same = 1;
    for (int i = 0; i < sv->nshard; i++)
      same &= sv->sh[i].dinv_uniform && sv->sh[i].dinv_const == c;
    if (sv->dist) {
      const int P = lsb_hip_comm_size();
      unsigned mine[3], *all = lsb_calloc(unsigned, 3 * (size_t)P);
      mine[0] = (unsigned)same;
      memcpy(mine + 1, &c, sizeof c);
      lsb_hip_comm_allgather_u32(mine, 3, all);
      for (int q = 0; q < P; q++)
        same &= all[3 * q] && all[3 * q + 1] == all[1] && all[3 * q + 2] == all[2];
      free(all);
    }
    sv->cg1_implicit = same;
  }
  tune_blas1_nt(sv);
  precond_setup(sv);
  sv->driver = solve_driver_for(sv->o.krylov);
  sv->form = pcg_choose_form(sv);
  sv->overlap_on = -1;
  p2p_setup(sv);
  overlap_setup(sv);
  persist_setup(sv);
}

static void bicgstab_check_precond(const struct lsb_hip_opts *o) {
  if (o->krylov == LSB_KRYLOV_BICGSTAB && o->precond != LSB_PRECOND_JACOBI && o->precond != LSB_PRECOND_NONE &&
      o->precond != LSB_PRECOND_L1JACOBI)
    errx(EXIT_FAILURE, "hip_cdna4: --krylov bicgstab runs with --precond jacobi, l1 or none (Chebyshev, "
                       "block-Jacobi, FSAI and AMG run under PCG)");
}

static struct lsb_hip_opts solver_opts(const struct lsb_hip_opts *o_in, int sharded) {
  struct lsb_hip_opts o;
  if (o_in)
    o = *o_in;
  else
    lsb_hip_get_opts(&o);
  if (o.precision == LSB_PREC_MIXED && (o.krylov == LSB_KRYLOV_GMRES || o.krylov == LSB_KRYLOV_BICGSTAB)) {
    if (!sharded)
      warnx("hip_cdna4: mixed precision is an iterative refinement around CG; %s runs in fp64",
            o.krylov == LSB_KRYLOV_GMRES ? "GMRES" : "BiCGSTAB");
    o.precision = LSB_PREC_FP64;
  }
  bicgstab_check_precond(&o);
  richardson_check(&o, sharded);
  direct_check(&o, sharded);
  if (o.precision == LSB_PREC_MIXED && o.precond == LSB_PRECOND_AMG) {
    if (!sharded)
      warnx("hip_cdna4: --precond amg runs in fp64");
    o.precision = LSB_PREC_FP64;
  }
  return o;
}

lsb_hip_solver *lsb_hip_solver_create(const struct csr *A,
                                      const struct lsb_hip_opts *o_in) {
  if (!lsb_initialized || !A || A->nrows == 0)
    return NULL;
  struct lsb_hip_opts o = solver_opts(o_in, 0);
  struct csr *S = o.op_mode == LSB_OP_CHOLMOD_UPPER ? lsb_csr_symmetrize_upper(A)
                                                    : lsb_csr_copy_base0(A);
  const unsigned n_user = S->nrows;
  unsigned dir_height = 0;
  double dir_seconds = 0.0;
  struct lsb_skyinv *dirW = o.krylov == LSB_KRYLOV_DIRECT ? direct_factor(S, &o, &dir_height, &dir_seconds) : NULL;
  int *padmap = NULL;
  {
    const char *e = getenv("LSBENCH_HIP_PAD_LINES");
    const int want = e ? atoi(e) : (S->nrows >= 1000000u ? 1 : 0);
    if (want && !o.reorder && o.krylov != LSB_KRYLOV_DIRECT) {
      unsigned nx = 0, nxp = 0;
      struct csr *Sp = lsb_csr_pad_lines(S, LSB_SELL_ROWS, &nx, &nxp, &padmap);
      if (Sp) {
        if (o.verbose)
          fprintf(stderr, "hip_cdna4: grid lines of %u rows padded to %u (%u -> %u rows)\n", nx, nxp, S->nrows,
                  Sp->nrows);
        lsb_csr_free(S);
        S = Sp;
      }
    }
  }
  int P = o.nvirt > 1 ? o.nvirt : 1;
  if ((unsigned)P > S->nrows / 2)
    P = 1;
  lsb_hip_solver *sv = solver_alloc(P, &o);
  sv->n_user = n_user;
  if (padmap) {
    sv->d_perm = (int *)dev_upload(padmap, (size_t)S->nrows * sizeof(int));
    LSB_CHK_HIP(hipStreamSynchronize(g_stream));
    free(padmap);
    sv->padded = 1;
  }
  if (o.reorder) {
    unsigned *perm = (unsigned *)malloc((size_t)S->nrows * sizeof(unsigned));
    if (!perm || lsb_csr_rcm(S, perm))
      errx(EXIT_FAILURE, "hip_cdna4: out of memory computing the RCM ordering");
    struct csr *Sp = lsb_csr_permute_sym(S, perm);
    if (o.verbose)
      fprintf(stderr, "hip_cdna4: RCM bandwidth %u -> %u\n", lsb_csr_bandwidth(S),
              lsb_csr_bandwidth(Sp));
    lsb_csr_free(S);
    S = Sp;
    sv->d_perm = (int *)dev_upload(perm, (size_t)S->nrows * sizeof(int));
    LSB_CHK_HIP(hipStreamSynchronize(g_stream));
    free(perm);
  }
  sv->n_glob = sv->n_here = S->nrows, sv->row_first = 0;
  sv->dist = 0, sv->multi = P > 1;
  unsigned *bounds = lsb_calloc(unsigned, (size_t)P + 1);
  lsb_csr_partition_rows(S, (unsigned)P, bounds);
  unsigned *hull = lsb_calloc(unsigned, 4 * (size_t)P);
  sv->sh[0].slab_bx = sv->d_perm && P == 1;
  for (int q = 0; q < P; q++) {
    shard_upload(&sv->sh[q], S, bounds[q], bounds[q + 1], 0, bounds[q], S->nrows, &o);
    hull[4 * q] = bounds[q], hull[4 * q + 1] = bounds[q + 1] - bounds[q];
    hull[4 * q + 2] = sv->sh[q].col_lo, hull[4 * q + 3] = sv->sh[q].col_hi;
  }
  if (sv->sh[0].slab_bx) {
    sv->d_xp = shard_vec(&sv->sh[0], S->nrows);
    sv->d_bp = shard_vec(&sv->sh[0], S->nrows);
  } else if (sv->d_perm) {
    sv->d_bp = (double *)lsb_hip_malloc((size_t)S->nrows * sizeof(double));
    sv->d_xp = (double *)lsb_hip_malloc((size_t)S->nrows * sizeof(double));
  }
  for (int q = 0; q < P; q++) {
    plan_exchange(&sv->sh[q], q, P, hull);
    for (int k = 0; k < sv->sh[q].nrecv; k++)
      if (sv->sh[q].recv[k].count > sv->agree_halo)
        sv->agree_halo = (unsigned)sv->sh[q].recv[k].count;
  }
  free(hull), free(bounds);
  lsb_csr_free(S);
  solver_finish_setup(sv);
  if (dirW)
    direct_upload(sv, dirW, dir_height, dir_seconds);
  return sv;
}

lsb_hip_solver *lsb_hip_solver_create_dist(const struct csr *A_rows,
                                           unsigned row_begin,
                                           unsigned n_global,
                                           const struct lsb_hip_opts *o_in) {
  if (!lsb_initialized || !A_rows)
    return NULL;
  struct lsb_hip_opts o = solver_opts(o_in, 1);
  const int P = lsb_hip_comm_size(), me = lsb_hip_comm_rank();
  lsb_hip_solver *sv = solver_alloc(1, &o);
  sv->n_glob = n_global, sv->n_here = sv->n_user = A_rows->nrows, sv->row_first = row_begin;
  const char *alone = getenv("LSBENCH_HIP_DIST_ALONE");
  sv->dist = sv->multi = P > 1 || (alone && atoi(alone) > 0);
  shard_upload(&sv->sh[0], A_rows, 0, 0, 1, row_begin, n_global, &o);
  unsigned mine[4] = {row_begin, A_rows->nrows, sv->sh[0].col_lo, sv->sh[0].col_hi};
  unsigned *hull = lsb_calloc(unsigned, 4 * (size_t)P);
  lsb_hip_comm_allgather_u32(mine, 4, hull);
  {
    unsigned nz = (unsigned)sv->sh[0].nnz, *allnz = lsb_calloc(unsigned, (size_t)P);
    lsb_hip_comm_allgather_u32(&nz, 1, allnz);
    for (int q = 0; q < P; q++) {
      if (allnz[q] > sv->agree_nnz)
        sv->agree_nnz = allnz[q];
      if (hull[4 * q + 1] > sv->agree_n)
        sv->agree_n = hull[4 * q + 1];
    }
    free(allnz);
  }
  unsigned expect = 0;
  int full = 1, equal = 1;
  for (int q = 0; q < P; q++) {
    if (hull[4 * q] != expect)
      errx(EXIT_FAILURE, "hip_cdna4: rank %d owns rows from %u, expected %u "
                         "(row ranges must tile the operator in rank order)",
           q, hull[4 * q], expect);
    expect += hull[4 * q + 1];
    full &= hull[4 * q + 2] == 0 && hull[4 * q + 3] == n_global;
    equal &= hull[4 * q + 1] == hull[1];
  }
  if (expect != n_global)
    errx(EXIT_FAILURE, "hip_cdna4: shards cover %u rows, operator has %u", expect, n_global);
  plan_exchange(&sv->sh[0], me, P, hull);
  if (P > 1 && full && equal) {
    sv->sh[0].nsend = 1, sv->sh[0].send[0].peer = -1;
    sv->sh[0].send[0].offset = row_begin, sv->sh[0].send[0].count = A_rows->nrows;
    sv->sh[0].nrecv = 0;
  }
  free(hull);
  {
    unsigned h = 0, *allh = lsb_calloc(unsigned, (size_t)P);
    for (int k = 0; k < sv->sh[0].nrecv; k++)
      if (sv->sh[0].recv[k].count > h)
        h = (unsigned)sv->sh[0].recv[k].count;
    lsb_hip_comm_allgather_u32(&h, 1, allh);
    for (int q = 0; q < P; q++)
      if (allh[q] > sv->agree_halo)
        sv->agree_halo = allh[q];
    free(allh);
// ... 35 lines not shown
  lsb_hip_free(sv->d_scal_all), lsb_hip_free(sv->d_tmp);
  lsb_hip_free(sv->d_vr), lsb_hip_free(sv->d_ve);
  lsb_hip_free(sv->d_x0r), lsb_hip_free(sv->d_x0e);
  free(sv->start_rr);
  lsb_hip_free(sv->ps.d_wgrow), lsb_hip_free(sv->ps.d_ug), lsb_hip_free(sv->ps.d_shared);
  lsb_hip_free(sv->d_perm);
  for (int i = 0; sv->gm && i < sv->nshard; i++) {
    lsb_hip_free(sv->gm[i].V), lsb_hip_free(sv->gm[i].parts);
    lsb_hip_free(sv->gm[i].ax), lsb_hip_free(sv->gm[i].st);
  }
  free(sv->gm);
  lsb_hip_free(sv->gm_red);
  if (sv->gm_hst)
    LSB_CHK_HIP(hipHostFree(sv->gm_hst));
  LSB_CHK_HIP(hipHostFree(sv->h_st));
  free(sv->sh), free(sv);
}

unsigned lsb_hip_solver_nrows_local(const lsb_hip_solver *s) { return s->n_user; }
unsigned lsb_hip_solver_slab_mask(const lsb_hip_solver *sv) {
  const struct shard *s = &sv->sh[0];
  const void *v[5] = {s->d_r, s->d_pfull, s->d_p1, sv->d_xp, sv->d_bp};
  unsigned m = 0;
  for (int k = 0; k < 5; k++)
    if (v[k] && s->d_slab && (const char *)v[k] >= s->d_slab && (const char *)v[k] < s->d_slab + s->slab_cap)
      m |= 1u << k;
  return m;
}
int lsb_hip_solver_padded(const lsb_hip_solver *s) { return s->padded ? (int)(s->n_here - s->n_user) : 0; }
unsigned lsb_hip_solver_nrows_global(const lsb_hip_solver *s) { return s->n_glob; }
unsigned long long lsb_hip_solver_nnz_local(const lsb_hip_solver *s) {
  unsigned long long z = 0;
  for (int i = 0; i < s->nshard; i++)
    z += s->sh[i].nnz;
  return z;
}
unsigned lsb_hip_solver_nblocks(const lsb_hip_solver *s) { return s->sh[0].csr.nblk; }
int lsb_hip_solver_spmv_variant(const lsb_hip_solver *s) { return s->sh[0].variant; }
unsigned lsb_hip_solver_spmv_flags(const lsb_hip_solver *s) { return s->sh[0].sp_flags; }
unsigned lsb_hip_solver_spmv_grid(const lsb_hip_solver *s) { return s->sh[0].sp_grid; }
unsigned lsb_hip_solver_spmv_period(const lsb_hip_solver *s) { return s->sh[0].sp_period; }
unsigned long long lsb_hip_solver_spmv_col_slices(const lsb_hip_solver *s) { return s->sh[0].col.slices; }
void lsb_hip_solver_sell_value_slots(const lsb_hip_solver *s, unsigned *kept, unsigned *total) {
  const struct shard *h = &s->sh[0];
  const int on = h->sell_form >= SELL_16;
  if (kept)
    *kept = on ? h->c16.vslots : 0;
  if (total)
    *total = on ? h->c16.slots : 0;
}
void lsb_hip_solver_comm_plan(const lsb_hip_solver *s, unsigned long long plan[8]) {
  const struct shard *h = &s->sh[0];
  memset(plan, 0, 8 * sizeof plan[0]);
  plan[0] = (unsigned long long)lsb_hip_comm_count();
  plan[6] = (unsigned long long)s->nshard;
  if (!s->multi)
    return;
  plan[5] = h->nsend == 1 && h->send[0].peer == -1;
  if (plan[5]) {
    const unsigned long long P = s->dist ? (unsigned long long)lsb_hip_comm_size() : (unsigned long long)s->nshard;
    plan[1] = plan[2] = P - 1;
    plan[3] = (P - 1) * h->send[0].count * 8ull, plan[4] = h->send[0].count * 8ull;
  } else {
    plan[1] = (unsigned long long)h->nrecv, plan[2] = (unsigned long long)h->nsend;
    for (int k = 0; k < h->nrecv; k++)
      plan[3] += h->recv[k].count * 8ull;
    for (int k = 0; k < h->nsend; k++)
      plan[4] += h->send[k].count * 8ull;
  }
  plan[7] = (unsigned long long)can_overlap(s);
}
int lsb_hip_solver_overlap(const lsb_hip_solver *s, double us[2]) {
  if (us)
    us[0] = s->overlap_us[0], us[1] = s->overlap_us[1];
  return can_overlap(s);
}
int lsb_hip_solver_fused_p(const lsb_hip_solver *s) { return s->form == PCG_COL ? 2 : s->form == PCG_SUBWAVE; }
int lsb_hip_solver_blas1_nt(const lsb_hip_solver *s) { return s->nt_mask; }
unsigned long long lsb_hip_solver_spmv_layout_bytes(const lsb_hip_solver *s) {
  const struct shard *h = &s->sh[0];
  if (h->variant == LSB_SPMV_TWOPHASE || h->variant == LSB_SPMV_BINNED)
    return 0;
  const unsigned long long m[] = {12ull * h->nnz + 4ull * ((unsigned long long)h->n + 1),
                                  h->sell.bytes, h->c16.bytes, h->c16.tmpl.bytes, h->col.bytes};
  return m[h->sell_form] + 16ull * h->n;
}
int lsb_hip_solver_overlaps(const lsb_hip_solver *s) { return can_overlap(s); }
int lsb_hip_solver_comm(const lsb_hip_solver *s, double *p2p_us, double *rccl_us) {
  if (p2p_us)
    *p2p_us = s->p2p_us;
  if (rccl_us)
    *rccl_us = s->rccl_us;
  return !s->multi ? 0 : !s->p2p_on ? 1 : s->p2p_halo ? 3 : 2;
}


void sell_launch(struct shard *s, unsigned s0, unsigned ns, const double *xfull, double *y,
                        const double *xdot, double *partials, unsigned *np,
                        const struct lsb_pcg_state *st) {
  const unsigned f32 = s->mixed ? LSB_SP_F32 : 0u;
  const struct shard_col *c = &s->col;
  const int col_all = s0 == 0 && ns == s->sell.nslice;
  const int col_in = c->plan_in && s0 == s->sell.split.first && ns == s->sell.split.last - s->sell.split.first;
  if (s->sell_form == SELL_COL && (col_all || col_in) && !s->epi.zout)
    lsb_k_spmv_tmpl_col(s->sp_flags | f32, s->sp_grid, c->period, col_all ? c->plan : c->plan_in,
                        col_all ? c->items : c->items_in, c->centre0, s->n, s->row_begin, s->n_glob, &s->c16, xfull,
                        y, xdot, partials, np, st, &s->tail, g_stream);
  else if (s->sell_form >= SELL_TMPL)
    lsb_k_spmv_tmpl(s->sp_flags | f32, (s->sp_flags & LSB_SP_COL) ? LSB_SELL_GRID : s->sp_grid, s->sp_period, &s->c16, s0, ns,
                    s->n, s->row_begin, s->n_glob, xfull, y, xdot, partials, np, st, &s->tail, &s->epi, g_stream);
  else if (s->sell_form == SELL_16)
    lsb_k_spmv_sell(s->sp_flags | f32, s->sp_grid, s->sp_period, s->c16.sptr, s0, ns, s->n, s->row_begin, s->n_glob,
                    s->c16.codes, s->c16.sbase, s->c16.vals, s->c16.vconst, s->c16.ulen, xfull, y, xdot, partials, np,
                    st, &s->tail, &s->epi, g_stream);
  else
    lsb_k_spmv_sell((s->sp_flags & ~LSB_SP_C16) | f32, s->sp_grid, s->sp_period, s->sell.sptr, s0, ns, s->n,
                    s->row_begin, s->n_glob, s->sell.cols, NULL, s->sell.vals, NULL, 0, xfull, y, xdot, partials, np,
                    st, &s->tail, NULL, g_stream);
}

void spmv_shard(struct shard *s, const double *xfull, double *y,
                       const double *xdot, double *partials, unsigned *np,
                       const struct lsb_pcg_state *st) {
  if (s->variant == LSB_SPMV_PANEL || s->variant == LSB_SPMV_BINNED) {
    const struct shard_panel *pl = &s->panel;
    const struct shard_bins *bn = &s->bins;
    LSB_CHK_HIP(hipMemsetAsync(y, 0, (size_t)s->n * sizeof(double), g_stream));
    for (unsigned p = 0; s->variant == LSB_SPMV_PANEL && p < pl->n; p++) {
      const unsigned b0 = pl->blk[p], nb = pl->blk[p + 1] - b0;
      if (nb)
        lsb_k_spmv(LSB_SPMV_ADAPTIVE, s->n, pl->offs, pl->cols, pl->vals, pl->rowblk + b0, pl->blklanes + b0, nb,
                   s->lanes, s->sp_flags, s->sp_grid, xfull, y, NULL, NULL, NULL, st, pl->rowmap, NULL, g_stream);
    }
    for (unsigned b = 0; s->variant == LSB_SPMV_BINNED && b < bn->n; b++)
      lsb_k_spmv_binned(s->sp_flags, bn->cap, bn->chunk, bn->chunk_h[b], bn->chunk_h[b + 1] - bn->chunk_h[b],
                        bn->rows, bn->cols, bn->vals, xfull, y, st, g_stream);
    if (partials)
      lsb_k_dot(s->n, y, xdot, partials, np, g_stream);
    return;
  }
  if (s->variant == LSB_SPMV_SELL) {
    sell_launch(s, 0, s->sell.nslice, xfull, y, xdot, partials, np, st);
    return;
  }
  if (s->variant == LSB_SPMV_TWOPHASE) {
    const struct shard_tp *t = &s->tp;
    lsb_k_spmv_twophase(t->items, t->item, t->vals, t->colw, t->first, t->mask, t->delta, t->roww, t->col_lo,
                        t->cols, t->rows, t->bins, t->binptr, t->prod, s->n, xfull, t->xlen, y, xdot, partials, np,
                        t->binparts, st, g_stream);
    return;
  }
  const int f32 = s->mixed && (s->variant == LSB_SPMV_ADAPTIVE || s->variant == LSB_SPMV_SUBWAVE);
  lsb_k_spmv(s->variant, s->n, s->csr.offs, s->csr.cols, f32 ? (const double *)s->csr.vals32 : s->csr.vals,
             s->csr.rowblk, s->csr.blklanes, s->csr.nblk, s->lanes, s->sp_flags | (f32 ? LSB_SP_F32 : 0u),
             s->sp_grid, xfull, y, xdot, partials, np, st, NULL, &s->tail, g_stream);
}

struct halo_split shard_split(const struct shard *s, unsigned *count) {
  if (count)
    *count = s->variant == LSB_SPMV_SELL ? s->sell.nslice : s->csr.nblk;
  return s->variant == LSB_SPMV_SELL ? s->sell.split : s->variant == LSB_SPMV_ADAPTIVE ? s->csr.split : (struct halo_split){0};
}

void spmv_shard_exact(struct shard *s, const double *xfull, double *y, const double *xdot,
                      double *partials, unsigned *np, const struct lsb_pcg_state *st) {
  if (!s->mixed) {
    spmv_shard(s, xfull, y, xdot, partials, np, st);
    return;
  }
  const int v = s->nnz <= 500000ull ? LSB_SPMV_SUBWAVE : LSB_SPMV_ADAPTIVE;
  lsb_k_spmv(v, s->n, s->csr.offs, s->csr.cols, s->csr.vals, s->csr.rowblk, s->csr.blklanes, s->csr.nblk, s->lanes,
             LSB_SP_PREFETCH | LSB_SP_NT, 0, xfull, y, xdot, partials, np, st, NULL, NULL, g_stream);
}

static int sell_form(const struct shard *s) {
  const unsigned f = s->sp_flags;
  return s->variant != LSB_SPMV_SELL               ? SELL_NONE
         : !(f & LSB_SP_C16) || !s->c16.codes      ? SELL_32
         : !(f & LSB_SP_TMPL) || !s->c16.tmpl.srec ? SELL_16
         : (f & LSB_SP_COL) && s->col.plan         ? SELL_COL
                                                   : SELL_TMPL;
}

static void time_spmv(lsb_hip_solver *sv, struct shard *s) {
  const struct lsb_hip_opts *o = &sv->o;
  float best = 1e30f;
  unsigned bf = s->sp_flags, np;
  int bv = s->variant;
  const unsigned grid0 = s->sp_grid;
  unsigned bg = grid0, bp = 0;
  struct {
    int v;
    unsigned f, g, p;
  } cand[32];
  memset(cand, 0, sizeof cand);
  int ncand = 0;
  const int any = o->spmv_variant == LSB_SPMV_AUTO;
#define CAND(V, F, G, P)                                                                       \
  do {                                                                                         \
    if (ncand >= (int)(sizeof cand / sizeof cand[0]))                                          \
      errx(EXIT_FAILURE, "hip_cdna4: SpMV timing pass: candidate table too small");            \
    cand[ncand].v = (V), cand[ncand].f = (F), cand[ncand].g = (G), cand[ncand].p = (P), ncand++; \
  } while (0)
  if (any || s->variant == LSB_SPMV_ADAPTIVE)
    for (unsigned f = 0; f < 4; f++)
      CAND(LSB_SPMV_ADAPTIVE, f, grid0, 0);
  if (s->panel.n && (any || s->variant == LSB_SPMV_PANEL))
    for (unsigned f = 0; f < 4; f++)
      CAND(LSB_SPMV_PANEL, f, grid0, 0);
  if (s->tp.bins && (any || s->variant == LSB_SPMV_TWOPHASE))
    CAND(LSB_SPMV_TWOPHASE, 0, grid0, 0);
  if (s->bins.n && (any || s->variant == LSB_SPMV_BINNED)) {
    static const unsigned bf[] = {LSB_SP_NT, 0};
    for (unsigned k = 0; k < sizeof bf / sizeof bf[0]; k++)
      CAND(LSB_SPMV_BINNED, bf[k], grid0, 0);
  }
  const unsigned period = s->sell.period;
  if (s->sell.sptr && (any || s->variant == LSB_SPMV_SELL))
    for (unsigned c16 = 0; c16 <= (s->c16.codes ? LSB_SP_C16 : 0u); c16 += LSB_SP_C16) {
      CAND(LSB_SPMV_SELL, c16 | LSB_SP_NT, grid0, 0);
      CAND(LSB_SPMV_SELL, c16, grid0, 0);
      if (o->spmv_grid <= 0)
        CAND(LSB_SPMV_SELL, c16 | LSB_SP_NT, LSB_SELL_GRID, 0);
      if (period) {
        CAND(LSB_SPMV_SELL, c16 | LSB_SP_NT, grid0, period);
        CAND(LSB_SPMV_SELL, c16, grid0, period);
      }
      if (c16 && s->c16.tmpl.srec) {
        const unsigned f = c16 | LSB_SP_NT | LSB_SP_TMPL;
        CAND(LSB_SPMV_SELL, f, grid0, 0);
        if (o->spmv_grid <= 0)
          CAND(LSB_SPMV_SELL, f, LSB_SELL_GRID, 0);
        if (period) {
          CAND(LSB_SPMV_SELL, f, grid0, period);
          if (o->spmv_grid <= 0)
            CAND(LSB_SPMV_SELL, f, LSB_SELL_GRID, period);
        }
        if (s->c16.tmpl.nfar >= 1 && s->nnz >= 16000000ull) {
          const unsigned fd = f | LSB_SP_DEFER, gd = o->spmv_grid <= 0 ? LSB_SELL_GRID : grid0;
          CAND(LSB_SPMV_SELL, fd, gd, 0);
          if (period)
            CAND(LSB_SPMV_SELL, fd, gd, period);
        }
        if (s->col.plan) {
          if (o->spmv_grid <= 0) {
            const unsigned gcol = LSB_TMPL_COL_GRID(s->c16.tmpl.nfar);
            CAND(LSB_SPMV_SELL, f | LSB_SP_COL, 768, 0);
            if (gcol > 768) {
              CAND(LSB_SPMV_SELL, f | LSB_SP_COL, 1024, 0);
              CAND(LSB_SPMV_SELL, f | LSB_SP_COL, gcol, 0);
            }
          } else
            CAND(LSB_SPMV_SELL, f | LSB_SP_COL, grid0, 0);
        }
      }
    }
#undef CAND
  for (int ci = 0; ci < ncand; ci++) {
    s->variant = cand[ci].v, s->sp_flags = cand[ci].f, s->sp_grid = cand[ci].g, s->sp_period = cand[ci].p;
    s->sell_form = sell_form(s);
    spmv_shard(s, s->d_pfull, s->d_q, s->d_pfull + s->row_begin, s->d_parts_pq, &np, NULL);
    LSB_CHK_HIP(hipEventRecord(sv->ev_t0, g_stream));
    const int reps = 5;
    for (int r = 0; r < reps; r++)
      spmv_shard(s, s->d_pfull, s->d_q, s->d_pfull + s->row_begin, s->d_parts_pq, &np, NULL);
    LSB_CHK_HIP(hipEventRecord(sv->ev_t1, g_stream));
    LSB_CHK_HIP(hipEventSynchronize(sv->ev_t1));
    float ms = 0.f;
    LSB_CHK_HIP(hipEventElapsedTime(&ms, sv->ev_t0, sv->ev_t1));
    ms *= 3.0f / reps;
    if (o->verbose > 1)
      fprintf(stderr, "hip_cdna4: spmv tune form=%d flags=%u grid=%u period=%u: %.1f us\n", s->variant,
              s->sp_flags, s->sp_grid, s->sp_period, ms * 1e3f / 3);
    if (!(s->sp_flags & LSB_SP_NT))
      ms *= 1.03f;
    if (pcg_choose_form(sv) == PCG_COL)
      ms *= 0.85f;
    if (ms < best)
      best = ms, bf = s->sp_flags, bv = s->variant, bg = s->sp_grid, bp = s->sp_period;
  }
  s->sp_grid = bg;
  s->sp_period = bp;
  s->variant = bv;
  s->sp_flags = bf;
  const int sell = bv == LSB_SPMV_SELL;
  if (any && bv != LSB_SPMV_TWOPHASE)
    tp_free(&s->tp);
  if (any && bv != LSB_SPMV_BINNED)
    bins_free(&s->bins);
  if (!(sell && (bf & LSB_SP_TMPL)))
    tmpl_free(&s->c16.tmpl);
  if (!(sell && (bf & LSB_SP_C16)))
    c16_free(&s->c16);
  if (!(sell && (bf & LSB_SP_COL)))
    col_free(&s->col);
  if (any && !(sell && !(bf & LSB_SP_C16)))
    sell32_free(&s->sell);
}

void tune_spmv(lsb_hip_solver *sv, struct shard *s) {
  const struct lsb_hip_opts *o = &sv->o;
  s->sp_flags = LSB_SP_PREFETCH | LSB_SP_NT;
  s->sp_grid = o->spmv_grid > 0 ? (unsigned)o->spmv_grid : LSB_MAX_PARTIALS;
  if (getenv("LSBENCH_HIP_FORCE_PERIOD"))
    s->sp_period = s->sell.period;
  if (o->spmv_tune >= 0)
    s->sp_flags = (unsigned)o->spmv_tune & (31u | LSB_SP_TMPL | LSB_SP_DEFER | LSB_SP_COL);
  else if ((s->variant == LSB_SPMV_ADAPTIVE || s->variant == LSB_SPMV_PANEL || s->variant == LSB_SPMV_SELL ||
            s->variant == LSB_SPMV_BINNED || s->variant == LSB_SPMV_TWOPHASE) &&
           s->nnz >= 4000000ull)
    time_spmv(sv, s);
  s->sell_form = sell_form(s);
}

int lsb_hip_solver_spmv_dev(lsb_hip_solver *sv, const double *d_x, double *d_y) {
  if (!lsb_initialized)
    return 1;
  if (!sv || !d_x || !d_y)
    return 2;
  double *d_yout = NULL;
  if (sv->d_perm) {
    lsb_k_perm_gather(sv->n_here, sv->d_perm, d_x, sv->d_bp, g_stream);
    d_x = sv->d_bp, d_yout = d_y, d_y = sv->d_xp;
  }
  gather_x(sv, d_x);
  for (int i = 0; i < sv->nshard; i++) {
    struct shard *s = &sv->sh[i];
    spmv_shard_exact(s, s->d_pfull, d_y + (s->row_begin - sv->row_first), NULL, NULL, NULL, NULL);
  }
  if (d_yout)
    lsb_k_perm_scatter(sv->n_here, sv->d_perm, d_y, d_yout, g_stream);
  drain_stream(sv, "lsb_hip_solver_spmv_dev");
  check_aux_status(sv, "lsb_hip_solver_spmv_dev");
  return 0;
}

int lsb_hip_solver_spmv_inner_dev(lsb_hip_solver *sv, const double *d_x, double *d_y, double *d_dot) {
  if (!lsb_initialized)
    return 1;
  if (!sv || !d_x || !d_y || (d_dot && sv->nshard > 1))
    return 2;
  double *d_yout = NULL;
  if (sv->d_perm) {
    lsb_k_perm_gather(sv->n_here, sv->d_perm, d_x, sv->d_bp, g_stream);
    d_x = sv->d_bp, d_yout = d_y, d_y = sv->d_xp;
  }
  for (int i = 0; i < sv->nshard; i++)
    LSB_CHK_HIP(hipMemsetAsync(&sv->sh[i].d_st->status, 0, sizeof(int), g_stream));
  gather_x(sv, d_x);
  const int split = can_overlap(sv);
  for (int i = 0; i < sv->nshard; i++) {
    struct shard *s = &sv->sh[i];
    double *y = d_y + (s->row_begin - sv->row_first);
    unsigned np = 0;
    s->npq = 0;
    for (int part = 0; part < (split ? 3 : 1); part++) {
      if (split)
        spmv_range(s, part, y, s->d_parts_pq + s->npq, &np, s->d_st);
      else
        spmv_shard(s, s->d_pfull, y, s->d_pfull + s->row_begin, s->d_parts_pq, &np, s->d_st);
      s->npq += np;
    }
  }
  if (d_dot)
    lsb_k_reduce_final(sv->sh[0].d_parts_pq, sv->sh[0].npq, 1, d_dot, 0, NULL, g_stream);
  if (d_yout)
    lsb_k_perm_scatter(sv->n_here, sv->d_perm, d_y, d_yout, g_stream);
  drain_stream(sv, "lsb_hip_solver_spmv_inner_dev");
  check_aux_status(sv, "lsb_hip_solver_spmv_inner_dev");
  return 0;
}

int lsb_hip_solver_time_spmv(lsb_hip_solver *sv, int warm, int reps, double *ms_avg) {
  if (!lsb_initialized)
    return 1;
  if (!sv || reps < 1 || !ms_avg)
    return 2;
  struct shard *s = &sv->sh[0];
// ... 47 lines not shown
```

### lsbench_amd/csrc/hip_solver.h

```cpp
#ifndef HIP_SOLVER_H
#define HIP_SOLVER_H

#define __HIP_PLATFORM_AMD__ 1
#include <hip/hip_runtime_api.h>
#include <math.h>
#include <stddef.h>
#include <string.h>
#include <strings.h>
#include <time.h>

#include "lsb_impl.h"

#define LSB_INTERNAL __attribute__((visibility("hidden")))

extern LSB_INTERNAL int lsb_initialized;
extern LSB_INTERNAL __thread hipStream_t g_stream;
extern LSB_INTERNAL __thread struct lsb_hip_result g_last;
LSB_INTERNAL hipStream_t comm_stream(void);
LSB_INTERNAL void rank_thread_attach(int device);
LSB_INTERNAL void rank_thread_detach(void);
LSB_INTERNAL int bench_multi(double *x, struct csr *A, const double *r, const struct lsbench *cb,
                             const struct lsb_hip_opts *o, int ngpus);

#define SCAL_STRIDE 8
#define MAX_SAMPLES 64
#define LSB_NGRAPH 4

struct graph_cache {
  struct {
    hipGraphExec_t exec;
    int count;
    const void *key;
  } e[LSB_NGRAPH];
  int next;
};

struct amg_vecs;
struct block_work {
  unsigned kp;
  char *mem;
  double *b, *x, *p, *q;
  union {
    double *r;
    double *w;
  };
  double *z, *t;
  char *zmem, *amg_mem;
  struct amg_vecs *av;
  struct graph_cache g;
};

struct halo_split {
  unsigned first, last;
  int ok;
};
enum { SELL_NONE, SELL_32, SELL_16, SELL_TMPL, SELL_COL };
enum pcg_form {
  PCG_NONE,
  PCG_CLASSIC,
  PCG_SUBWAVE,
  PCG_COL,
  PCG_CG1,
  PCG_GENERIC,
  PCG_FSAI3,
};

typedef int solve_dev_fn(lsb_hip_solver *sv, const double *d_b, double *d_x, struct lsb_hip_result *res);
struct solve_driver {
  solve_dev_fn *solve;
  int (*run)(lsb_hip_solver *sv, const double *d_b, double *d_x, struct lsb_hip_result *res, int round);
};

struct amg_vecs {
  void *b, *out, *tmp, *r, *d;
};

struct shard {
  char *d_slab;
  size_t slab_cap, slab_used;
  int slab_bx;
  unsigned row_begin, n;
  unsigned long long nnz;
  unsigned n_glob;
  unsigned col_lo, col_hi;
  int variant, sell_form;
  unsigned lanes;
  unsigned sp_flags, sp_grid, sp_period;
  int mixed, exact32;
  struct shard_csr {
    int *offs, *cols, *rowblk;
    unsigned char *blklanes;
    double *vals;
    float *vals32;
    unsigned nblk;
    struct halo_split split;
  } csr;
  struct shard_panel {
    unsigned n;
    unsigned *blk;
    int *offs, *cols, *rowmap, *rowblk;
    unsigned char *blklanes;
    double *vals;
  } panel;
  struct shard_bins {
    unsigned n, cap;
    unsigned *chunk_h;
    unsigned *chunk, *rows, *cols;
    double *vals;
  } bins;
  struct shard_tp {
    unsigned items, bins, col_lo, xlen, cols, rows;
    unsigned *item, *binptr, *first, *delta;
    unsigned long long *mask;
    unsigned short *colw, *roww;
    double *vals, *prod, *binparts;
  } tp;
  struct shard_sell {
    unsigned nslice;
    unsigned period;
    struct halo_split split;
    unsigned *sptr;
    int *cols;
    double *vals;
    unsigned long long bytes;
  } sell;
  struct lsb_sell16_dev c16;
  struct shard_col {
    unsigned period;
    unsigned *plan, *plan_in;
    unsigned items, items_in;
    int centre0;
    unsigned long long slices;
    unsigned long long bytes;
  } col;
  double *d_dinv, *d_r, *d_q, *d_pfull;
  double *d_p1, *d_s1;
  unsigned npq, np2;
  const double *ar2_parts;
  unsigned ar2_n, ar2_width;
  struct lsb_cheb_epi epi;
  double *d_zfull2;
  struct lsb_ar_tail tail;
  int dinv_uniform;
  double dinv_const;
  double *d_parts_pq, *d_parts2;
  double *d_scal;
  struct lsb_pcg_state *d_st;
  struct lsb_pcg_state *d_st_aux;
  double *d_zfull, *d_z;
  double *d_chd;
  double *d_binv, *d_bjpart;
  unsigned bj_bs;
  struct fsai_csr {
    int *offs, *cols, *rowblk;
    unsigned char *blklanes;
    double *vals;
    unsigned nblk, lanes;
    int variant;
    unsigned long long nnz;
  } fs_g, fs_gt;
  double *d_fst;
  double *d_r1;
  unsigned fs_maxrow;
  struct amg_dev {
    unsigned nlev, tail, nu, nc, clanes;
    int prec, cheb, mcgs;
    unsigned mcgs_cap;
    unsigned long long mcgs_bytes;
    struct amg_lv {
      unsigned n;
      union amg_mat {
        struct lsb_amg_mat d;
        struct amg_mat32 f;
      } A, P, R;
      const void *minv;
      double lo, hi, c1[16], c2[16];
      unsigned ncol, ncol_found, *cbeg;
      union amg_mat C;
      const int *rowid;
      const unsigned char *colour8;
    } *lv;
    struct amg_vecs *vec;
    struct lsb_amg_lvdev *d_lv;
    void *d_cinv;
    void **mem;
    unsigned nmem;
    double setup_s;
    unsigned long long cycle_mat_bytes, cycle_vec_rows;
    unsigned long long cycle_bytes32;
  } *amg;
  struct lsb_xfer *recv, *send;
  int nrecv, nsend;
};

struct lsb_hip_solver {
  unsigned n_glob;
  unsigned n_here;
  unsigned n_user;
  int padded;
  unsigned row_first;
  int nshard;
  int dist;
  int multi;
  struct shard *sh;
  double *d_scal_all;
  struct lsb_hip_opts o;
  struct lsb_pcg_state *h_st;
  struct graph_cache graphs;
#define LSB_MAX_CORRECTIONS 6
#define LSB_MIXED_INNER_TOL 1e-5
  unsigned hint_iters[LSB_MAX_CORRECTIONS + 1];
  double tol_run;
  int verify_run;
  double *d_vr, *d_ve;
  double *d_x0r, *d_x0e;
  double *start_rr;
  unsigned start_n, start_cap;
// ... 313 lines not shown
```

### lsbench_amd/csrc/lsb_impl.h

```cpp
#ifndef LSB_IMPL_H
#define LSB_IMPL_H

#include "lsbench_hip.h"
#include <err.h>
#include <stdint.h>
#include <stdio.h>
#include <stdlib.h>

#ifdef __cplusplus
extern "C" {
#endif

#define lsb_calloc(T, n) ((T *)calloc((size_t)(n) > 0 ? (size_t)(n) : 1, sizeof(T)))

struct lsb_pcg_state {
  double rz[2];
  double bb;
  double thresh2;
  double rr;
  double pq;
  double alpha[2];
  int iters;
  int status;
  int maxit;
// ... 29 lines not shown
  double bnorm, thresh, beta, resid, hnorm;
  double g[LSB_GMRES_MAX_RESTART + 1];
  double cs[LSB_GMRES_MAX_RESTART], sn[LSB_GMRES_MAX_RESTART], y[LSB_GMRES_MAX_RESTART];
  double R[LSB_GMRES_MAX_RESTART * LSB_GMRES_MAX_RESTART];
  int iters, status, maxit, restart, jlast, cycle_open;
};

struct lsb_bcg_state {
  struct lsb_pcg_state c;
  double rho[2];
  double alpha, omega;
  int half;
  int nspmv;
};

#define LSB_MRHS_MAX 8
struct lsb_mrhs_state {
  struct lsb_pcg_state c[LSB_MRHS_MAX];
  double true_relres[LSB_MRHS_MAX];
  double tol;
  int corrections[LSB_MRHS_MAX];
  int running;
  int nspmm;
  double start_relres[LSB_MRHS_MAX];
};

#define LSB_MAX_PARTIALS 2048
#define LSB_STREAM_GRID_CAP 768
#define LSB_BLOCK_NNZ 2048

void lsb_k_spmv(int variant, unsigned n, const int *offs, const int *cols,
                const double *vals, const int *rowblk,
                const unsigned char *blklanes, unsigned nblk,
                unsigned lanes_per_row, unsigned flags, unsigned grid_cap,
                const double *x, double *y, const double *xdot,
                double *partials, unsigned *npartials,
                const struct lsb_pcg_state *st, const int *rowmap,
                const struct lsb_ar_tail *tail, void *stream);
int lsb_k_spmv_has_tail(int variant);
unsigned lsb_k_spmv_grid(int variant, unsigned n, unsigned nblk,
                         unsigned lanes_per_row, unsigned grid_cap);
#define LSB_SP_PREFETCH 1u
#define LSB_SP_NT 2u
#define LSB_SP_C16 4u
#define LSB_SP_F32 32u
void lsb_k_spmv_sell(unsigned flags, unsigned grid_cap, unsigned period, const unsigned *sptr,
                     unsigned s0, unsigned ns, unsigned n, unsigned row_begin, unsigned xlen,
                     const void *cols,
                     const int *sbase, const double *vals, const double *vconst, unsigned ulen,
                     const double *x, double *y, const double *xdot, double *partials,
                     unsigned *npartials,
                     const struct lsb_pcg_state *st, const struct lsb_ar_tail *tail,
                     const struct lsb_cheb_epi *epi, void *stream);
#define LSB_SP_TMPL 64u
#define LSB_SP_DEFER 128u
struct lsb_sell16_dev {
  unsigned *sptr;
  short *codes;
  int *sbase;
  double *vals;
  double *vconst;
  unsigned vslots, slots, ulen;
  unsigned long long bytes;
  struct lsb_tmpl_dev {
    unsigned *srec;
    unsigned long long *mask;
    struct lsb_sell_tmpl *td;
    unsigned nfar;
    unsigned long long bytes;
  } tmpl;
};
void lsb_k_spmv_tmpl(unsigned flags, unsigned grid_cap, unsigned period, const struct lsb_sell16_dev *c, unsigned s0,
                     unsigned ns, unsigned n, unsigned row_begin, unsigned xlen, const double *x, double *y,
                     const double *xdot, double *partials, unsigned *npartials, const struct lsb_pcg_state *st,
                     const struct lsb_ar_tail *tail, const struct lsb_cheb_epi *epi, void *stream);
void lsb_k_pcg_col_px(unsigned grid_cap, unsigned period, const unsigned *plan, unsigned nitem, unsigned n,
                      const struct lsb_sell16_dev *c, const double *r, const double *pold, double *pnew, double *x,
                      int xupd, double dc, double *partials, unsigned *npartials, struct lsb_pcg_state *st, int parity,
                      const double *parts2, unsigned nparts2, void *stream);
void lsb_k_pcg_col_r(unsigned grid_cap, unsigned period, const unsigned *plan, unsigned nitem, unsigned n,
                     const struct lsb_sell16_dev *c, const double *p, double *r, double dc, struct lsb_pcg_state *st,
                     int parity, int pbuf, int xtwo, int rev, const double *pq_parts, unsigned npq, double *partials2,
                     unsigned *npartials, void *stream);
void lsb_k_pcg_xfix(unsigned n, const double *p0, const double *p1, double *x, const struct lsb_pcg_state *st,
                    void *stream);
#define LSB_SP_COL 256u
void lsb_k_spmv_tmpl_col(unsigned flags, unsigned grid_cap, unsigned period, const unsigned *plan, unsigned nitem,
                         int centre0, unsigned n, unsigned row_begin, unsigned xlen, const struct lsb_sell16_dev *c,
                         const double *x, double *y, const double *xdot, double *partials, unsigned *npartials,
                         const struct lsb_pcg_state *st, const struct lsb_ar_tail *tail, void *stream);
void lsb_k_spmv_binned(unsigned flags, unsigned chunk_cap, const unsigned *chunk_begin, unsigned c0,
                       unsigned nchunk, const unsigned *rows, const unsigned *cols, const double *vals,
                       const double *x, double *y, const struct lsb_pcg_state *st, void *stream);
void lsb_k_spmv_twophase(unsigned nitems, const unsigned *item, const double *vals,
                         const unsigned short *colw, const unsigned *grp_first,
                         const unsigned long long *grp_mask, const unsigned *delta,
                         const unsigned short *roww, unsigned col_lo, unsigned cols, unsigned rows,
                         unsigned nbins, const unsigned *bin_ptr, double *prod, unsigned n,
                         const double *x, unsigned xlen, double *y, const double *xdot,
                         double *partials, unsigned *npartials, double *binparts,
                         const struct lsb_pcg_state *st, void *stream);
unsigned lsb_k_twophase_groups(unsigned nbins);
void lsb_k_reduce_final(const double *partials, unsigned nparts, unsigned width,
                        double *out, int take_sqrt,
                        const struct lsb_pcg_state *st, void *stream);
void lsb_k_reduce_final2(const double *pa, unsigned na, unsigned wa, double *outa,
                         const double *pb, unsigned nb, unsigned wb, double *outb,
                         const struct lsb_pcg_state *st, void *stream);
void lsb_k_dot(unsigned n, const double *a, const double *b, double *partials,
               unsigned *npartials, void *stream);
void lsb_k_axpy(unsigned n, const double *alpha, const double *x, double *y,
                void *stream);
void lsb_k_xpay(unsigned n, const double *beta, const double *x, double *y,
                void *stream);
void lsb_k_jacobi_setup(unsigned n, unsigned row_begin, const int *offs,
                        const int *cols, const double *vals, double *dinv,
                        int *nzero, void *stream);
void lsb_k_l1_setup(unsigned n, const int *offs, const double *vals, double *dinv, int *nzero,
                    void *stream);
void lsb_k_jacobi_apply(unsigned n, const double *dinv, const double *r,
                        double *z, void *stream);
void lsb_k_jacobi_sweep(unsigned n, double w, const double *dinv,
                        const double *b, const double *ax, double *x,
                        void *stream);
void lsb_k_pcg_init(unsigned n, const double *b, const double *dinv, double dc, double *x,
                    double *r, double *p, double *partials2,
                    unsigned *npartials, void *stream);
void lsb_k_pcg_init_state(struct lsb_pcg_state *st, const double *partials2,
                          unsigned nparts, double tol, int maxit,
                          void *stream);
void lsb_k_resid_csr2(unsigned n, const int *offs, const int *cols, const double *vals, unsigned lanes,
                      const double *xfull, const double *b, double *q, double *partials, unsigned *npartials,
                      void *stream);
void lsb_k_x0_start(unsigned n, const double *b, const double *q, double *r0, double *partials2,
                    unsigned *npartials, void *stream);
void lsb_k_pcg_update_xr(unsigned n, const double *p, const double *q,
                         const double *dinv, double dc, double *x, double *r,
                         struct lsb_pcg_state *st, int parity,
                         const double *pq_parts, unsigned npq,
                         double *partials2, unsigned *npartials, unsigned nt, void *stream);
void lsb_k_spmv_subwave_p(unsigned n, const int *offs, const int *cols, const double *vals,
                          unsigned lanes_per_row, const double *r, const double *dinv, double dc,
                          const double *pold, double *pnew, double *y, double *partials,
                          unsigned *npartials, struct lsb_pcg_state *st, int parity,
                          const double *parts2, unsigned nparts2, void *stream);
void lsb_k_pcg_update_p(unsigned n, const double *r, const double *dinv, double dc,
                        const double *pin, double *p, struct lsb_pcg_state *st, int parity,
                        const double *parts2, unsigned nparts2, unsigned nt, void *stream);
void lsb_k_cg1_update(unsigned n, double *u, const double *w, const double *dinv, double dc,
                      double *p,
                      double *s, double *x, double *r, struct lsb_pcg_state *st, int parity,
                      const double *parts_gr, unsigned ngr, const double *parts_d, unsigned nd,
                      const struct lsb_ar_collect *collect, double *partials2, unsigned *npartials,
                      unsigned nt, void *stream);
unsigned lsb_k_blas1_grid(unsigned n);
void lsb_k_fill_index(unsigned n, unsigned first, double *v, void *stream);
void lsb_k_perm_gather(unsigned n, const int *perm, const double *src, double *dst,
                       void *stream);
void lsb_k_perm_scatter(unsigned n, const int *perm, const double *src, double *dst,
                        void *stream);
void lsb_k_vreduce(double *base, unsigned stride, unsigned nshard, unsigned off,
                   unsigned cnt, void *stream);

unsigned lsb_k_gm_grid(unsigned n);
void lsb_k_gm_resid(unsigned n, const double *b, const double *ax, double *v0,
                    double *partials, const struct lsb_gmres_state *st, void *stream);
// ... 281 lines not shown
```

### lsbench_amd/csrc/lsb_operator.c

```c
#include "lsb_impl.h"
#include <string.h>
#ifdef _OPENMP
#include <omp.h>
#else
static inline int omp_get_max_threads(void) { return 1; }
#endif

static struct csr *csr_alloc(unsigned nrows, unsigned long long nnz) {
  if (nnz > 0xFFFFFFFFull)
    errx(EXIT_FAILURE, "CSR with %llu non-zeros does not fit 32-bit offsets "
                       "(reference layout, src/lsbench-impl.h:22-26)", nnz);
  struct csr *S = lsb_calloc(struct csr, 1);
  S->nrows = nrows, S->base = 0;
  S->offs = lsb_calloc(unsigned, (size_t)nrows + 1);
  S->cols = lsb_calloc(unsigned, (size_t)nnz);
  S->vals = lsb_calloc(double, (size_t)nnz);
  if (!S->offs || !S->cols || !S->vals)
    errx(EXIT_FAILURE, "out of host memory for a %u-row / %llu-nnz CSR", nrows, nnz);
  return S;
}

void lsb_csr_free(struct csr *A) {
  if (!A)
    return;
  free(A->offs), free(A->cols), free(A->vals);
  free(A);
}

struct csr *lsb_csr_symmetrize_upper(const struct csr *A) {
  const unsigned n = A->nrows, base = A->base;
  unsigned *first_upper = lsb_calloc(unsigned, (size_t)n + 1);
  unsigned long long *cnt = lsb_calloc(unsigned long long, (size_t)n + 1);
  for (unsigned i = 0; i < n; i++) {
    unsigned j = A->offs[i];
    const unsigned je = A->offs[i + 1];
    while (j < je && A->cols[j] - base < i)
      j++;
    first_upper[i] = j;
    for (; j < je; j++) {
      const unsigned c = A->cols[j] - base;
      if (c >= n)
        errx(EXIT_FAILURE, "column %u of row %u is outside the %u x %u matrix",
             c + base, i + base, n, n);
      cnt[i]++;
      if (c != i)
        cnt[c]++;
    }
  }
  unsigned long long nnz = 0;
  for (unsigned i = 0; i < n; i++)
    nnz += cnt[i];
  struct csr *S = csr_alloc(n, nnz);
  unsigned *fill = lsb_calloc(unsigned, (size_t)n + 1);
  unsigned long long acc = 0;
  for (unsigned i = 0; i < n; i++) {
    S->offs[i] = (unsigned)acc, fill[i] = (unsigned)acc;
    acc += cnt[i];
  }
  S->offs[n] = (unsigned)acc;
  for (unsigned i = 0; i < n; i++) {
    for (unsigned j = first_upper[i]; j < A->offs[i + 1]; j++) {
      const unsigned c = A->cols[j] - base;
      if (c != i) {
        S->cols[fill[c]] = i, S->vals[fill[c]] = A->vals[j];
        fill[c]++;
      }
    }
  }
  for (unsigned i = 0; i < n; i++) {
    for (unsigned j = first_upper[i]; j < A->offs[i + 1]; j++) {
      S->cols[fill[i]] = A->cols[j] - base, S->vals[fill[i]] = A->vals[j];
      fill[i]++;
    }
  }
  free(first_upper), free(cnt), free(fill);
  return S;
}

struct csr *lsb_csr_copy_base0(const struct csr *A) {
  const unsigned n = A->nrows, nnz = A->offs[n];
  struct csr *S = csr_alloc(n, nnz);
  memcpy(S->offs, A->offs, ((size_t)n + 1) * sizeof(unsigned));
  memcpy(S->vals, A->vals, (size_t)nnz * sizeof(double));
  for (unsigned j = 0; j < nnz; j++)
    S->cols[j] = A->cols[j] - A->base;
  return S;
}

struct csr *lsb_csr_pad_lines(const struct csr *S, unsigned slice, unsigned *nx_out, unsigned *nxp_out, int **map_out) {
  if (!S || S->base != 0 || slice < 2 || S->nrows < 4 * slice)
    return NULL;
  const unsigned n = S->nrows;
  unsigned nx = 0;
  for (unsigned r = 0; r < n && !nx; r++)
    if (S->offs[r + 1] > S->offs[r] && S->cols[S->offs[r + 1] - 1] > r + 1)
      nx = S->cols[S->offs[r + 1] - 1] - r;
  if (nx < 2 * slice || n % nx || n / nx < 3)
    return NULL;
  const unsigned ny = n / nx, nxp = (nx + slice - 1) / slice * slice;
  if (nxp == nx || (unsigned long long)(nxp - nx) * 16 > nx || (unsigned long long)ny * nxp > 0x7fffffffull)
    return NULL;
  double val[5] = {0, 0, 0, 0, 0};
  int have[5] = {0, 0, 0, 0, 0};
  for (unsigned r = 0; r < n; r++) {
    int diag = 0;
    for (unsigned k = S->offs[r]; k < S->offs[r + 1]; k++) {
      const long long d = (long long)S->cols[k] - (long long)r;
      const int w = d == -(long long)nx ? 0 : d == -1 ? 1 : d == 0 ? 2 : d == 1 ? 3 : d == (long long)nx ? 4 : -1;
      if (w < 0 || (w == 1 && r % nx == 0) || (w == 3 && r % nx == nx - 1))
        return NULL;
      if (!have[w])
        val[w] = S->vals[k], have[w] = 1;
      else if (memcmp(&val[w], &S->vals[k], sizeof(double)))
        return NULL;
      diag |= w == 2;
    }
    if (!diag)
      return NULL;
  }
  if (!have[0] || !have[1] || !have[3] || !have[4] || val[2] == 0.0)
    return NULL;
  const unsigned np = ny * nxp;
  const unsigned long long cap = (unsigned long long)S->offs[n] + 5ull * (unsigned long long)ny * (nxp - nx);
  if (cap > 0xffffffffull)
    return NULL;
  struct csr *Pd = csr_alloc(np, (unsigned)cap);
  int *map = (int *)malloc((size_t)np * sizeof(int));
  if (!map)
    errx(EXIT_FAILURE, "lsb_csr_pad_lines: out of memory");
  unsigned at = 0;
  for (unsigned j = 0; j < ny; j++)
    for (unsigned i = 0; i < nxp; i++) {
      const unsigned row = j * nxp + i;
      Pd->offs[row] = at;
      if (i < nx) {
        const unsigned r = j * nx + i;
        map[row] = (int)r;
        for (unsigned k = S->offs[r]; k < S->offs[r + 1]; k++) {
          const unsigned c = S->cols[k];
          Pd->cols[at] = c / nx * nxp + c % nx, Pd->vals[at] = S->vals[k], at++;
        }
      } else {
        map[row] = -1;
        if (j > 0)
          Pd->cols[at] = row - nxp, Pd->vals[at] = val[0], at++;
        if (i > nx)
          Pd->cols[at] = row - 1, Pd->vals[at] = val[1], at++;
        Pd->cols[at] = row, Pd->vals[at] = val[2], at++;
        if (i + 1 < nxp)
          Pd->cols[at] = row + 1, Pd->vals[at] = val[3], at++;
        if (j + 1 < ny)
          Pd->cols[at] = row + nxp, Pd->vals[at] = val[4], at++;
      }
    }
  Pd->offs[np] = at;
  if (nx_out)
    *nx_out = nx;
  if (nxp_out)
    *nxp_out = nxp;
  if (map_out)
    *map_out = map;
  else
    free(map);
  return Pd;
}

struct csr *lsb_csr_row_slice(const struct csr *A, unsigned r0, unsigned r1) {
  if (r1 > A->nrows || r0 > r1)
    return NULL;
  const unsigned j0 = A->offs[r0], j1 = A->offs[r1];
  struct csr *S = csr_alloc(r1 - r0, j1 - j0);
  for (unsigned i = r0; i <= r1; i++)
    S->offs[i - r0] = A->offs[i] - j0;
  memcpy(S->vals, A->vals + j0, (size_t)(j1 - j0) * sizeof(double));
  for (unsigned j = j0; j < j1; j++)
    S->cols[j - j0] = A->cols[j] - A->base;
  return S;
}

static unsigned lower_bound_offs(const unsigned *offs, unsigned n,
                                 unsigned long long target) {
  unsigned lo = 0, hi = n;
  while (lo < hi) {
    unsigned mid = lo + (hi - lo) / 2;
    if (offs[mid] < target)
      lo = mid + 1;
    else
      hi = mid;
  }
  return lo;
}

int lsb_csr_partition_rows(const struct csr *A, unsigned nparts,
                           unsigned *bounds) {
  if (nparts == 0)
    return 2;
  const unsigned n = A->nrows;
  const unsigned long long nnz = A->offs[n];
  bounds[0] = 0;
  for (unsigned p = 1; p < nparts; p++) {
    unsigned r = lower_bound_offs(A->offs, n, nnz * p / nparts);
    r &= ~1u;
    if (r < bounds[p - 1])
      r = bounds[p - 1];
    bounds[p] = r;
  }
  bounds[nparts] = n;
  return 0;
}

unsigned lsb_csr_row_blocks(const struct csr *A, unsigned cap,
                            unsigned **rowblk_out) {
  const unsigned n = A->nrows;
  size_t capb = (size_t)(A->offs[n] / (cap ? cap : 1)) * 2 + 16, nb = 0;
  unsigned *rb = (unsigned *)malloc(capb * sizeof(unsigned));
  unsigned r = 0;
  rb[nb++] = 0;
  while (r < n) {
    const unsigned long long lim = (unsigned long long)A->offs[r] + cap;
    unsigned lo = r + 1, hi = n;
    unsigned e = r + 1;
    if (A->offs[e] <= lim) {
      lo = r + 1, hi = n;
      while (lo < hi) {
        unsigned mid = lo + (hi - lo + 1) / 2;
        if (A->offs[mid] <= lim)
          lo = mid;
        else
          hi = mid - 1;
      }
      e = lo;
    }
    if (nb + 1 >= capb) {
      capb *= 2;
      rb = (unsigned *)realloc(rb, capb * sizeof(unsigned));
    }
    rb[nb++] = e;
    r = e;
  }
  *rowblk_out = rb;
  return (unsigned)(nb - 1);
}

void lsb_csr_col_hull(const struct csr *A, unsigned *lo_out, unsigned *hi_out) {
  unsigned lo = 0xFFFFFFFFu, hi = 0;
  const unsigned nnz = A->offs[A->nrows];
  for (unsigned j = 0; j < nnz; j++) {
// ... 1270 lines not shown
```

Measured before the change: 1.158.

## Add symmetric five-point stencil record layout with column-walk SpMV and PCG kernels

Adds a compact per-slice record format for symmetric 5-point operators that stores only the diagonal, east and north coefficients (plus an optional inverse diagonal) and gets west/south from neighbouring rows. New column-walking SpMV and fused PCG update kernels use this format, with register pipelining across a column of slices. The goal is to roughly halve matrix bytes read per iteration compared with the SELL template path. It depends on exact symmetry and on the padding checks, and adds a new code path with more complex boundary handling.

```diff
diff --git a/include/lsbench_hip.h b/include/lsbench_hip.h
--- a/include/lsbench_hip.h
+++ b/include/lsbench_hip.h
@@ -306,6 +306,17 @@
                                                   unsigned s_lo, unsigned s_hi);
 void lsb_tmpl_cols_free(struct lsb_tmpl_cols *C);
 int lsb_tmpl_cols_check(const struct lsb_sell_tmpls *T, const struct lsb_tmpl_cols *C, char *why, size_t whylen);
+struct lsb_sym5 {
+  unsigned nrows, nslice, period, rs;
+  double *rec;
+};
+struct csr *lsb_csr_pad_lines_sym(const struct csr *S, unsigned slice, unsigned *nx, unsigned *nxp, int **map);
+struct lsb_sym5 *lsb_csr_sym5(const struct csr *Sp, unsigned nxp, int with_dinv);
+void lsb_sym5_free(struct lsb_sym5 *Y);
+struct lsb_sell_tmpls *lsb_sym5_pattern(const struct lsb_sym5 *Y);
+int lsb_sym5_check(const struct csr *Sp, const struct lsb_sym5 *Y, const struct lsb_tmpl_cols *C, char *why,
+                   size_t whylen);
+#define LSB_SYM_COL_GRID 768u
 double lsb_csr_mean_scatter(const struct csr *A, unsigned row_begin);
 void lsb_csr_col_hull(const struct csr *A, unsigned *lo, unsigned *hi);
 struct lsb_xfer {
diff --git a/lsbench_amd/_lib.py b/lsbench_amd/_lib.py
--- a/lsbench_amd/_lib.py
+++ b/lsbench_amd/_lib.py
@@ -139,6 +139,11 @@
                 ("shaped", C.c_ulonglong), ("nmask", C.c_ulonglong), ("kept_read", C.c_ulonglong),
                 ("tid", C.POINTER(C.c_ubyte)), ("vbase", C.POINTER(C.c_uint)),
                 ("mask", C.POINTER(C.c_ulonglong)), ("t", C.POINTER(SellTmpl))]
+
+
+class Sym5(C.Structure):
+    _fields_ = [("nrows", C.c_uint), ("nslice", C.c_uint), ("period", C.c_uint), ("rs", C.c_uint),
+                ("rec", C.POINTER(C.c_double))]
 
 
 class TmplCols(C.Structure):
@@ -289,6 +294,11 @@
     "lsb_hip_solver_padded": (_i, [_vp]),
     "lsb_hip_solver_slab_mask": (_u, [_vp]),
     "lsb_csr_pad_lines": (_csrp, [_csrp, _u, C.POINTER(_u), C.POINTER(_u), C.POINTER(C.POINTER(C.c_int))]),
+    "lsb_csr_pad_lines_sym": (_csrp, [_csrp, _u, C.POINTER(_u), C.POINTER(_u), C.POINTER(C.POINTER(C.c_int))]),
+    "lsb_csr_sym5": (C.POINTER(Sym5), [_csrp, _u, _i]),
+    "lsb_sym5_free": (None, [C.POINTER(Sym5)]),
+    "lsb_sym5_pattern": (C.POINTER(SellTmpls), [C.POINTER(Sym5)]),
+    "lsb_sym5_check": (_i, [_csrp, C.POINTER(Sym5), C.POINTER(TmplCols), C.c_char_p, C.c_size_t]),
     "lsb_hip_solver_nrows_global": (_u, [_vp]),
     "lsb_hip_solver_nnz_local": (C.c_ulonglong, [_vp]),
     "lsb_hip_solver_nblocks": (_u, [_vp]),
diff --git a/lsbench_amd/csrc/hip_kernels.hip b/lsbench_amd/csrc/hip_kernels.hip
--- a/lsbench_amd/csrc/hip_kernels.hip
+++ b/lsbench_amd/csrc/hip_kernels.hip
@@ -1378,6 +1378,426 @@
   }
 }
 
+constexpr int SYM_WGS = LSB_SYM_COL_GRID / 256;
+static_assert(SYM_WGS * 256 == LSB_SYM_COL_GRID, "the resident grid is whole workgroups per CU on 256 CUs");
+template <int RS> __device__ __forceinline__ double sym_at(const double *__restrict__ rec, long long row, int w) {
+  return rec[(row >> 7) * (RS * LSB_SELL_ROWS) + w * LSB_SELL_ROWS + (row & 127)];
+}
+__device__ __forceinline__ double sym_sel(double v, double x) { return v != 0.0 ? x : 0.0; }
+__device__ __forceinline__ void sym_rows(const sell_d2v &sv, double w0, double w1, const sell_d2v &d, const sell_d2v &e,
+                                         const sell_d2v &nv, const sell_d2u &below, double up, const sell_d2u &c,
+                                         double dn, const sell_d2u &above, double &a0, double &a1) {
+  a0 = fma(sv.x, sym_sel(sv.x, below.x), 0.0), a1 = fma(sv.y, sym_sel(sv.y, below.y), 0.0);
+  a0 = fma(w0, sym_sel(w0, up), a0), a1 = fma(w1, sym_sel(w1, c.x), a1);
+  a0 = fma(d.x, c.x, a0), a1 = fma(d.y, c.y, a1);
+  a0 = fma(e.x, sym_sel(e.x, c.y), a0), a1 = fma(e.y, sym_sel(e.y, dn), a1);
+  a0 = fma(nv.x, sym_sel(nv.x, above.x), a0), a1 = fma(nv.y, sym_sel(nv.y, above.y), a1);
+}
+template <int RS, typename F>
+__device__ __forceinline__ void sym_single(const double *__restrict__ rec, unsigned g, unsigned P, unsigned lane, F opnd,
+                                           double &a0, double &a1) {
+  const unsigned row = g + 2 * lane;
+  const double *R = rec + (size_t)g * RS + 2 * lane;
+  const sell_d2v d = *(const sell_d2v *)R, e = *(const sell_d2v *)(R + LSB_SELL_ROWS),
+                 nv = *(const sell_d2v *)(R + 2 * LSB_SELL_ROWS);
+  const sell_d2v sv = *(const sell_d2v *)(g >= P ? R - (size_t)P * RS + 2 * LSB_SELL_ROWS : R + 2 * LSB_SELL_ROWS);
+  const double s0 = g >= P ? sv.x : 0.0, s1 = g >= P ? sv.y : 0.0;
+  const double wl = sym_at<RS>(rec, row ? row - 1 : 0, 1), w0 = row ? wl : 0.0, w1 = e.x;
+  const double c0 = opnd(row), c1 = opnd(row + 1);
+  a0 = fma(s0, sym_sel(s0, opnd(s0 != 0.0 ? row - P : row)), 0.0), a1 = fma(s1, sym_sel(s1, opnd(s1 != 0.0 ? row + 1 - P : row)), 0.0);
+  a0 = fma(w0, sym_sel(w0, opnd(w0 != 0.0 ? row - 1 : row)), a0), a1 = fma(w1, sym_sel(w1, c0), a1);
+  a0 = fma(d.x, c0, a0), a1 = fma(d.y, c1, a1);
+  a0 = fma(e.x, sym_sel(e.x, c1), a0), a1 = fma(e.y, sym_sel(e.y, opnd(e.y != 0.0 ? row + 2 : row)), a1);
+  a0 = fma(nv.x, sym_sel(nv.x, opnd(nv.x != 0.0 ? row + P : row)), a0), a1 = fma(nv.y, sym_sel(nv.y, opnd(nv.y != 0.0 ? row + 1 + P : row)), a1);
+}
+
+template <int RS> struct symc_ops {
+  sell_d2v d, e, nl;
+  sell_d2v di;
+  double xe, we;
+  sell_d2v xd;
+};
+template <int RS, int DOT, bool DI>
+__device__ __forceinline__ void symc_issue(symc_ops<RS> &o, sell_d2u &cnext, const double *__restrict__ rec,
+                                           const double *__restrict__ x, const double *__restrict__ xdot, long long gu,
+                                           long long D, bool down, unsigned lane) {
+  cnext = *(const sell_d2u *)(x + (gu + D) + 2 * lane);
+  const double *R = rec + gu * RS + 2 * lane;
+  o.d = *(const sell_d2v *)R, o.e = *(const sell_d2v *)(R + LSB_SELL_ROWS);
+  o.nl = *(const sell_d2v *)(rec + (down ? gu + D : gu) * RS + 2 * LSB_SELL_ROWS + 2 * lane);
+  if (RS == 4 && DI)
+    o.di = *(const sell_d2v *)(R + 3 * LSB_SELL_ROWS);
+  o.xe = x[lane < 32u ? gu - 1 : gu + (long long)LSB_SELL_ROWS];
+  o.we = rec[(gu - (long long)LSB_SELL_ROWS) * RS + 2 * LSB_SELL_ROWS - 1];
+  if (DOT == 2)
+    o.xd = *(const sell_d2v *)(xdot + gu + 2 * lane);
+}
+template <int RS>
+__device__ __forceinline__ void symc_compute(const symc_ops<RS> &o, const sell_d2v &nprev, bool down, const sell_d2u &cb,
+                                             const sell_d2u &c, const sell_d2u &ca, unsigned lane, double &a0, double &a1) {
+  double up = lane_above(c.y), dn = lane_below(c.x), w0 = lane_above(o.e.y);
+  if (lane == 0)
+    up = o.xe, w0 = o.we;
+  if (lane == 63)
+    dn = o.xe;
+  const sell_d2v sv = down ? o.nl : nprev, nv = down ? nprev : o.nl;
+  sym_rows(sv, w0, o.e.x, o.d, o.e, nv, down ? ca : cb, up, c, dn, down ? cb : ca, a0, a1);
+}
+
+template <int RS, int DOT>
+__global__ __launch_bounds__(WG, SYM_WGS) void k_spmv_symcol(
+    const unsigned *__restrict__ plan, unsigned period, unsigned n, const double *__restrict__ rec,
+    const double *__restrict__ x, double *__restrict__ y, const double *__restrict__ xdot, double *__restrict__ partials,
+    const lsb_pcg_state *__restrict__ st, const lsb_ar_tail tail) {
+  __shared__ double sred[4];
+  const unsigned tid = threadIdx.x, lane = tid & 63u, wave = tid >> 6;
+  const unsigned gx = gridDim.x / NXCD, xcd = blockIdx.x % NXCD, slot = blockIdx.x / NXCD;
+  const unsigned i0 = plan[xcd], i1 = plan[xcd + 1];
+  const u4v *__restrict__ items = (const u4v *)(plan + LSB_COL_HEAD);
+  const unsigned dofs = plan[LSB_TMPL_COL_DOWN];
+  const int stopped = st ? st->status : 0;
+  const unsigned P = period * LSB_SELL_ROWS;
+  double dot = 0.0;
+  for (unsigned g = slot; i0 + 4 * g < i1; g += gx) {
+    const unsigned it = __builtin_amdgcn_readfirstlane(i0 + 4 * g + wave);
+    if (it >= i1)
+      continue;
+    const u4v item = items[it];
+    const unsigned s = __builtin_amdgcn_readfirstlane(item.x);
+    const unsigned K = __builtin_amdgcn_readfirstlane(item.y) & ~LSB_TMPL_COL_LOCKSTEP;
+    if (K >= 3) {
+      const bool down = col_walks_down(plan, dofs, it);
+      const unsigned s0 = down ? s + (K - 1) * period : s;
+      const long long D = down ? -(long long)P : (long long)P;
+      long long gu = (long long)s0 * LSB_SELL_ROWS;
+      symc_ops<RS> cur, nxt;
+      sell_d2u cb = *(const sell_d2u *)(x + (gu - D) + 2 * lane);
+      sell_d2u c0 = *(const sell_d2u *)(x + gu + 2 * lane);
+      sell_d2v nprev = *(const sell_d2v *)(rec + (down ? gu : gu - D) * RS + 2 * LSB_SELL_ROWS + 2 * lane);
+      sell_d2u ca, cn;
+      symc_issue<RS, DOT, false>(cur, ca, rec, x, xdot, gu, D, down, lane);
+      if (stopped)
+        return;
+      for (unsigned k = 0; k + 1 < K; k++) {
+        symc_issue<RS, DOT, false>(nxt, cn, rec, x, xdot, gu + D, D, down, lane);
+        double a0, a1;
+        symc_compute<RS>(cur, nprev, down, cb, c0, ca, lane, a0, a1);
+        {
+          const sell_d2v o = {a0, a1};
+          *(sell_d2v *)(y + gu + 2 * lane) = o;
+        }
+        if (DOT == 1)
+          dot = fma(a0, c0.x, dot), dot = fma(a1, c0.y, dot);
+        else if (DOT == 2)
+          dot = fma(a0, cur.xd.x, dot), dot = fma(a1, cur.xd.y, dot);
+        nprev = cur.nl, cb = c0, c0 = ca, ca = cn, cur = nxt;
+        gu += D;
+      }
+      double a0, a1;
+      symc_compute<RS>(cur, nprev, down, cb, c0, ca, lane, a0, a1);
+      {
+        const sell_d2v o = {a0, a1};
+        *(sell_d2v *)(y + gu + 2 * lane) = o;
+      }
+      if (DOT == 1)
+        dot = fma(a0, c0.x, dot), dot = fma(a1, c0.y, dot);
+      else if (DOT == 2)
+        dot = fma(a0, cur.xd.x, dot), dot = fma(a1, cur.xd.y, dot);
+    } else {
+      if (stopped)
+        return;
+      for (unsigned k = 0; k < K; k++) {
+        const unsigned g0 = (s + k * period) * LSB_SELL_ROWS, row = g0 + 2 * lane;
+        double a0, a1;
+        sym_single<RS>(rec, g0, P, lane, [&](unsigned i) { return x[i]; }, a0, a1);
+        const sell_d2v o = {a0, a1};
+        *(sell_d2v *)(y + row) = o;
+        if (DOT)
+          dot = fma(a0, xdot[row], dot), dot = fma(a1, xdot[row + 1], dot);
+      }
+    }
+  }
+  if (stopped)
+    return;
+  spmv_publish(partials, dot, sred, tail);
+}
+
+template <int RS> struct symp_c {
+  sell_d2u rn, pn;
+  sell_d2v da;
+  sell_d2v d;
+  sell_d2v xn, sn;
+  sell_d2v e, nl;
+  double re, pe, de, we;
+};
+template <int RS, bool WITH_X, int NT>
+__device__ __forceinline__ void symp_issue(symp_c<RS> &o, const double *__restrict__ rec, const double *__restrict__ r,
+                                           const double *__restrict__ pold, const double *__restrict__ x,
+                                           const double *pstale, long long gu, long long D, bool down, unsigned lane) {
+  const long long ga = gu + D;
+  o.rn = *(const sell_d2u *)(r + ga + 2 * lane);
+  o.pn = *(const sell_d2u *)(pold + ga + 2 * lane);
+  o.da = *(const sell_d2v *)(rec + ga * RS + (RS == 4 ? 3 * LSB_SELL_ROWS : 0) + 2 * lane);
+  const double *R = rec + gu * RS + 2 * lane;
+  if (RS == 4)
+    o.d = *(const sell_d2v *)R;
+  o.e = *(const sell_d2v *)(R + LSB_SELL_ROWS);
+  o.nl = *(const sell_d2v *)(rec + (down ? ga : gu) * RS + 2 * LSB_SELL_ROWS + 2 * lane);
+  if (WITH_X) {
+    if (NT & 1) {
+      o.xn = __builtin_nontemporal_load((const sell_d2v *)(x + ga + 2 * lane));
+      o.sn = __builtin_nontemporal_load((const sell_d2v *)(pstale + ga + 2 * lane));
+    } else {
+      o.xn = *(const sell_d2v *)(x + ga + 2 * lane);
+      o.sn = *(const sell_d2v *)(pstale + ga + 2 * lane);
+    }
+  }
+  const long long e = lane < 32u ? gu - 1 : gu + (long long)LSB_SELL_ROWS;
+  o.re = r[e], o.pe = pold[e], o.de = sym_at<RS>(rec, e, RS == 4 ? 3 : 0);
+  o.we = rec[(gu - (long long)LSB_SELL_ROWS) * RS + 2 * LSB_SELL_ROWS - 1];
+}
+template <int RS> __device__ __forceinline__ double sym_inv(double d) { return RS == 4 ? d : 1.0 / d; }
+template <int RS, bool OWNED, bool XUPD>
+__device__ __forceinline__ void symp_compute(const symp_c<RS> &o, const sell_d2v &d0, const sell_d2v &nprev,
+                                             const sell_d2u &pb, const sell_d2u &p0, sell_d2u &pp, bool down, double beta,
+                                             double alpha, double alpha2, unsigned lane, colp_out &out, double &dot) {
+  pp.x = pnew_of(sym_inv<RS>(o.da.x), o.rn.x, beta, o.pn.x), pp.y = pnew_of(sym_inv<RS>(o.da.y), o.rn.y, beta, o.pn.y);
+  if (OWNED) {
+    if (XUPD)
+      out.x.x = (o.xn.x + alpha2 * o.sn.x) + alpha * o.pn.x, out.x.y = (o.xn.y + alpha2 * o.sn.y) + alpha * o.pn.y;
+    out.p.x = pp.x, out.p.y = pp.y;
+  }
+  const double edge = pnew_of(sym_inv<RS>(o.de), o.re, beta, o.pe);
+  double up = lane_above(p0.y), dn = lane_below(p0.x), w0 = lane_above(o.e.y);
+  if (lane == 0)
+    up = edge, w0 = o.we;
+  if (lane == 63)
+    dn = edge;
+  const sell_d2v sv = down ? o.nl : nprev, nv = down ? nprev : o.nl;
+  double a0, a1;
+  sym_rows(sv, w0, o.e.x, RS == 4 ? o.d : d0, o.e, nv, down ? pp : pb, up, p0, dn, down ? pb : pp, a0, a1);
+  out.q.x = a0, out.q.y = a1;
+  dot = fma(a0, p0.x, dot), dot = fma(a1, p0.y, dot);
+}
+
+#define SYMP_ST(PTR, V, BIT) slice_store16<(NT & (BIT)) ? COL_ST_PX : ST_KEEP>((PTR), lane, (V))
+#define SYMP_STORE(OUT, GROW)                                                                  \
+  do {                                                                                         \
+    if (XUPD)                                                                                  \
+      SYMP_ST(x + (GROW), (OUT).x, 1);                                                         \
+    SYMP_ST(pnew + (GROW), (OUT).p, 2);                                                        \
+  } while (0)
+template <int RS, int NT, bool XUPD>
+__global__ __launch_bounds__(WG, SYM_WGS) void k_pcg_symcol_px(
+    const unsigned *__restrict__ plan, unsigned period, unsigned n, const double *__restrict__ rec,
+    const double *__restrict__ r, const double *__restrict__ pold, double *pnew, double *__restrict__ x,
+    double *__restrict__ partials, lsb_pcg_state *__restrict__ st, int parity, const double *__restrict__ parts2,
+    unsigned nparts2) {
+  __shared__ double sred[8];
+  const unsigned tid = threadIdx.x, lane = tid & 63u, wave = tid >> 6;
+  const unsigned gx = gridDim.x / NXCD, xcd = blockIdx.x % NXCD, slot = blockIdx.x / NXCD;
+  const int stopped = st->status;
+  const double rz_old = st->rz[parity], thresh2 = st->thresh2, alpha = st->alpha[0], alpha2 = st->alpha[1];
+  const unsigned i0 = plan[xcd], i1 = plan[xcd + 1];
+  double v[2];
+  wg_sum_parts<2, COL_PARTS_U>(parts2, nparts2, v, sred);
+  if (stopped)
+    return;
+  const double rz_new = v[0], rr = v[1];
+  const bool conv = rr <= thresh2;
+  if (blockIdx.x == 0 && threadIdx.x == 0) {
+    const int it = st->iters + 1;
+    st->iters = it;
+    st->rr = rr;
+    st->rz[parity ^ 1] = rz_new;
+    if (conv)
+      st->status = LSB_STATUS_CONVERGED;
+    else {
+      if (XUPD)
+        st->xpend = 0;
+      if (it >= st->maxit)
+        st->pad = 1;
+    }
+  }
+  if (conv)
+    return;
+  const double beta = rz_new / rz_old;
+  const u4v *__restrict__ items = (const u4v *)(plan + LSB_COL_HEAD);
+  const unsigned dofs = plan[LSB_TMPL_COL_DOWN];
+  const unsigned P = period * LSB_SELL_ROWS;
+  double dot = 0.0;
+  for (unsigned g = slot; i0 + 4 * g < i1; g += gx) {
+    const unsigned it = __builtin_amdgcn_readfirstlane(i0 + 4 * g + wave);
+    if (it >= i1)
+      continue;
+    const u4v item = items[it];
+    const unsigned s = __builtin_amdgcn_readfirstlane(item.x);
+    const unsigned K = __builtin_amdgcn_readfirstlane(item.y) & ~LSB_TMPL_COL_LOCKSTEP;
+    if (K >= 3) {
+      const bool down = col_walks_down(plan, dofs, it);
+      const unsigned s0 = down ? s + (K - 1) * period : s;
+      const long long D = down ? -(long long)P : (long long)P;
+      long long gu = (long long)s0 * LSB_SELL_ROWS;
+      const sell_d2u rb = *(const sell_d2u *)(r + (gu - D) + 2 * lane);
+      const sell_d2u pb = *(const sell_d2u *)(pold + (gu - D) + 2 * lane);
+      const sell_d2v db = *(const sell_d2v *)(rec + (gu - D) * RS + (RS == 4 ? 3 * LSB_SELL_ROWS : 0) + 2 * lane);
+      const sell_d2u r0 = *(const sell_d2u *)(r + gu + 2 * lane), o0 = *(const sell_d2u *)(pold + gu + 2 * lane);
+      const sell_d2v dc0 = *(const sell_d2v *)(rec + gu * RS + (RS == 4 ? 3 * LSB_SELL_ROWS : 0) + 2 * lane);
+      sell_d2v nprev = *(const sell_d2v *)(rec + (down ? gu : gu - D) * RS + 2 * LSB_SELL_ROWS + 2 * lane);
+      sell_d2v x0 = {0.0, 0.0}, s0v = {0.0, 0.0};
+      if (XUPD)
+        x0 = *(const sell_d2v *)(x + gu + 2 * lane), s0v = *(const sell_d2v *)(pnew + gu + 2 * lane);
+      symp_c<RS> c0, c1;
+      symp_issue<RS, XUPD, NT>(c0, rec, r, pold, x, pnew, gu, D, down, lane);
+      sell_d2u pm, p0, pp;
+      pm.x = pnew_of(sym_inv<RS>(db.x), rb.x, beta, pb.x), pm.y = pnew_of(sym_inv<RS>(db.y), rb.y, beta, pb.y);
+      p0.x = pnew_of(sym_inv<RS>(dc0.x), r0.x, beta, o0.x), p0.y = pnew_of(sym_inv<RS>(dc0.y), r0.y, beta, o0.y);
+      sell_d2v d0 = dc0;
+      colp_out res;
+      res.x.x = (x0.x + alpha2 * s0v.x) + alpha * o0.x, res.x.y = (x0.y + alpha2 * s0v.y) + alpha * o0.y;
+      res.p.x = p0.x, res.p.y = p0.y;
+      SYMP_STORE(res, gu);
+      for (unsigned k = 0; k + 2 < K; k++) {
+        symp_issue<RS, XUPD, NT>(c1, rec, r, pold, x, pnew, gu + D, D, down, lane);
+        symp_compute<RS, true, XUPD>(c0, d0, nprev, pm, p0, pp, down, beta, alpha, alpha2, lane, res, dot);
+        SYMP_STORE(res, gu + D);
+        nprev = c0.nl, d0 = c0.da, pm = p0, p0 = pp, c0 = c1;
+        gu += D;
+      }
+      symp_issue<RS, false, NT>(c1, rec, r, pold, x, pnew, gu + D, D, down, lane);
+      symp_compute<RS, true, XUPD>(c0, d0, nprev, pm, p0, pp, down, beta, alpha, alpha2, lane, res, dot);
+      SYMP_STORE(res, gu + D);
+      nprev = c0.nl, d0 = c0.da, pm = p0, p0 = pp, c0 = c1;
+      gu += D;
+      symp_compute<RS, false, XUPD>(c0, d0, nprev, pm, p0, pp, down, beta, alpha, alpha2, lane, res, dot);
+    } else {
+      for (unsigned k = 0; k < K; k++) {
+        const unsigned g0 = (s + k * period) * LSB_SELL_ROWS, row = g0 + 2 * lane;
+        const auto pn = [&](unsigned i) {
+          return pnew_of(sym_inv<RS>(sym_at<RS>(rec, i, RS == 4 ? 3 : 0)), r[i], beta, pold[i]);
+        };
+        const double o0 = pold[row], o1 = pold[row + 1];
+        double x0 = 0.0, x1 = 0.0, t0 = 0.0, t1 = 0.0;
+        if (XUPD)
+          x0 = x[row], x1 = x[row + 1], t0 = pnew[row], t1 = pnew[row + 1];
+        double a0, a1;
+        sym_single<RS>(rec, g0, P, lane, pn, a0, a1);
+        const double n0 = pn(row), n1 = pn(row + 1);
+        pnew[row] = n0, pnew[row + 1] = n1;
+        if (XUPD)
+          x[row] = (x0 + alpha2 * t0) + alpha * o0, x[row + 1] = (x1 + alpha2 * t1) + alpha * o1;
+        dot = fma(a0, n0, dot), dot = fma(a1, n1, dot);
+      }
+    }
+  }
+  if (partials) {
+    double d[1] = {dot};
+    wg_sum<1>(d, sred);
+    if (threadIdx.x == 0)
+      partials[blockIdx.x] = d[0];
+  }
+}
+#undef SYMP_STORE
+#undef SYMP_ST
+
+template <int RS>
+__global__ __launch_bounds__(WG, SYM_WGS) void k_pcg_symcol_r(
+    const unsigned *__restrict__ plan, unsigned period, unsigned n, const double *__restrict__ rec,
+    const double *__restrict__ p, double *__restrict__ r, lsb_pcg_state *__restrict__ st, int parity, int pbuf, int xtwo,
+    int rev, const double *__restrict__ pq_parts, unsigned npq, double *__restrict__ partials2) {
+  __shared__ double sred[8];
+  const unsigned tid = threadIdx.x, lane = tid & 63u, wave = tid >> 6;
+  const unsigned gx = gridDim.x / NXCD, xcd = blockIdx.x % NXCD, slot = blockIdx.x / NXCD;
+  const int stopped = st->status, pad = st->pad;
+  const double rz = st->rz[parity];
+  const unsigned i0 = plan[xcd], i1 = plan[xcd + 1];
+  double pqv[1];
+  wg_sum_parts<1, COL_PARTS_U>(pq_parts, npq, pqv, sred);
+  if (stopped)
+    return;
+  if (pad) {
+    if (blockIdx.x == 0 && threadIdx.x == 0)
+      st->status = LSB_STATUS_MAXIT;
+    return;
+  }
+  const double pq = pqv[0];
+  if (!(pq != 0.0) || !isfinite(pq)) {
+    if (blockIdx.x == 0 && threadIdx.x == 0)
+      st->status = LSB_STATUS_BREAKDOWN;
+    return;
+  }
+  const double alpha = rz / pq;
+  if (blockIdx.x == 0 && threadIdx.x == 0)
+    st->pq = pq, st->alpha[1] = st->alpha[0], st->alpha[0] = alpha, st->xpend = (xtwo ? 3 : 1) + pbuf;
+  const u4v *__restrict__ items = (const u4v *)(plan + LSB_COL_HEAD);
+  const unsigned dofs = plan[LSB_TMPL_COL_DOWN];
+  const unsigned P = period * LSB_SELL_ROWS;
+  double acc[2] = {0.0, 0.0};
+#define SYMR_FINISH(A0, A1, RV, DV, GROW)                                                      \
+  do {                                                                                         \
+    sell_d2v rn_;                                                                              \
+    rn_.x = (RV).x - alpha * (A0), rn_.y = (RV).y - alpha * (A1);                              \
+    slice_store16<COL_ST_R>(r + (GROW), lane, rn_);                                            \
+    acc[0] += rn_.x * (sym_inv<RS>((DV).x) * rn_.x);                                           \
+    acc[0] += rn_.y * (sym_inv<RS>((DV).y) * rn_.y);                                           \
+    acc[1] += rn_.x * rn_.x;                                                                   \
+    acc[1] += rn_.y * rn_.y;                                                                   \
+  } while (0)
+  const unsigned G = (i1 - i0 + 3u) / 4u;
+  for (unsigned j = slot; j < G; j += gx) {
+    const unsigned g = rev ? G - 1u - j : j;
+    const unsigned it = __builtin_amdgcn_readfirstlane(i0 + 4 * g + wave);
+    if (it >= i1)
+      continue;
+    const u4v item = items[it];
+    const unsigned s = __builtin_amdgcn_readfirstlane(item.x);
+    const unsigned K = __builtin_amdgcn_readfirstlane(item.y) & ~LSB_TMPL_COL_LOCKSTEP;
+    if (K >= 3) {
+      const bool down = col_walks_down(plan, dofs, it);
+      const unsigned s0 = down ? s + (K - 1) * period : s;
+      const long long D = down ? -(long long)P : (long long)P;
+      long long gu = (long long)s0 * LSB_SELL_ROWS;
+      symc_ops<RS> cur, nxt;
+      sell_d2u cb = *(const sell_d2u *)(p + (gu - D) + 2 * lane);
+      sell_d2u c0 = *(const sell_d2u *)(p + gu + 2 * lane);
+      sell_d2v nprev = *(const sell_d2v *)(rec + (down ? gu : gu - D) * RS + 2 * LSB_SELL_ROWS + 2 * lane);
+      sell_d2u ca, cn;
+      symc_issue<RS, 2, true>(cur, ca, rec, p, r, gu, D, down, lane);
+      for (unsigned k = 0; k + 1 < K; k++) {
+        symc_issue<RS, 2, true>(nxt, cn, rec, p, r, gu + D, D, down, lane);
+        double a0, a1;
+        symc_compute<RS>(cur, nprev, down, cb, c0, ca, lane, a0, a1);
+        if (RS == 4)
+          SYMR_FINISH(a0, a1, cur.xd, cur.di, gu);
+        else
+          SYMR_FINISH(a0, a1, cur.xd, cur.d, gu);
+        nprev = cur.nl, cb = c0, c0 = ca, ca = cn, cur = nxt;
+        gu += D;
+      }
+      double a0, a1;
+      symc_compute<RS>(cur, nprev, down, cb, c0, ca, lane, a0, a1);
+      if (RS == 4)
+        SYMR_FINISH(a0, a1, cur.xd, cur.di, gu);
+      else
+        SYMR_FINISH(a0, a1, cur.xd, cur.d, gu);
+    } else {
+      for (unsigned k = 0; k < K; k++) {
+        const unsigned g0 = (s + k * period) * LSB_SELL_ROWS, row = g0 + 2 * lane;
+        const sell_d2v rv = *(const sell_d2v *)(r + row);
+        const sell_d2v dv = *(const sell_d2v *)(rec + (size_t)g0 * RS + (RS == 4 ? 3 * LSB_SELL_ROWS : 0) + 2 * lane);
+        double a0, a1;
+        sym_single<RS>(rec, g0, P, lane, [&](unsigned i) { return p[i]; }, a0, a1);
+        SYMR_FINISH(a0, a1, rv, dv, g0);
+      }
+    }
+  }
+#undef SYMR_FINISH
+  wg_sum<2>(acc, sred);
+  if (threadIdx.x == 0) {
+    partials2[2 * blockIdx.x + 0] = acc[0];
+    partials2[2 * blockIdx.x + 1] = acc[1];
+  }
+}
 
 __device__ __forceinline__ unsigned bin_pad(unsigned i) { return i + (i >> 3); }
 
@@ -1758,4 +2178,51 @@
                                             partials2);
 }
 
-}
+static void symcol_args(const char *who, unsigned period, const unsigned *plan, const double *rec, unsigned rs,
+                        unsigned n) {
+  if (period < NXCD || !plan || !rec || (rs != 3 && rs != 4) || n % (period * LSB_SELL_ROWS))
+    errx(EXIT_FAILURE, "%s: no column plan or no records (period %u, %u numbers per row, %u rows)", who, period, rs, n);
+}
+void lsb_k_spmv_symcol(unsigned grid_cap, unsigned period, const unsigned *plan, unsigned nitem, unsigned n,
+                       const double *rec, unsigned rs, const double *x, double *y, const double *xdot, double *partials,
+                       unsigned *npartials, const struct lsb_pcg_state *st, const struct lsb_ar_tail *tail_in,
+                       void *stream) {
+  symcol_args("lsb_k_spmv_symcol", period, plan, rec, rs, n);
+  const sell_launch L = sell_prologue("lsb_k_spmv_symcol", true, NULL, nitem, n, grid_cap, LSB_SYM_COL_GRID, period,
+                                      partials, npartials, tail_in);
+  const int dot = !partials || !xdot ? 0 : xdot == x ? 1 : 2;
+  static decltype(&k_spmv_symcol<3, 0>) const kern[2][3] = {
+      {k_spmv_symcol<3, 0>, k_spmv_symcol<3, 1>, k_spmv_symcol<3, 2>},
+      {k_spmv_symcol<4, 0>, k_spmv_symcol<4, 1>, k_spmv_symcol<4, 2>}};
+  kern[rs - 3][dot]<<<L.g, WG, 0, (hipStream_t)stream>>>(plan, L.period, n, rec, x, y, xdot, partials, st, L.tail);
+}
+
+void lsb_k_pcg_symcol_px(unsigned grid_cap, unsigned period, const unsigned *plan, unsigned nitem, unsigned n,
+                         const double *rec, unsigned rs, const double *r, const double *pold, double *pnew, double *x,
+                         int xupd, double *partials, unsigned *npartials, struct lsb_pcg_state *st, int parity,
+                         const double *parts2, unsigned nparts2, void *stream) {
+  symcol_args("lsb_k_pcg_symcol_px", period, plan, rec, rs, n);
+  if (pold == pnew)
+    errx(EXIT_FAILURE, "lsb_k_pcg_symcol_px: one direction buffer");
+  const sell_launch L = sell_prologue("lsb_k_pcg_symcol_px", true, NULL, nitem, n, grid_cap, LSB_SYM_COL_GRID, period,
+                                      partials, npartials, NULL);
+  static decltype(&k_pcg_symcol_px<3, 3, false>) const kern[2][2] = {
+      {k_pcg_symcol_px<3, 3, false>, k_pcg_symcol_px<3, 3, true>},
+      {k_pcg_symcol_px<4, 3, false>, k_pcg_symcol_px<4, 3, true>}};
+  kern[rs - 3][xupd != 0]<<<L.g, WG, 0, (hipStream_t)stream>>>(plan, L.period, n, rec, r, pold, pnew, x, partials, st,
+                                                                parity, parts2, nparts2);
+}
+
+void lsb_k_pcg_symcol_r(unsigned grid_cap, unsigned period, const unsigned *plan, unsigned nitem, unsigned n,
+                        const double *rec, unsigned rs, const double *p, double *r, struct lsb_pcg_state *st, int parity,
+                        int pbuf, int xtwo, int rev, const double *pq_parts, unsigned npq, double *partials2,
+                        unsigned *npartials, void *stream) {
+  symcol_args("lsb_k_pcg_symcol_r", period, plan, rec, rs, n);
+  const sell_launch L = sell_prologue("lsb_k_pcg_symcol_r", true, NULL, nitem, n, grid_cap, LSB_SYM_COL_GRID, period,
+                                      partials2, npartials, NULL);
+  const auto kern = rs == 3 ? k_pcg_symcol_r<3> : k_pcg_symcol_r<4>;
+  kern<<<L.g, WG, 0, (hipStream_t)stream>>>(plan, L.period, n, rec, p, r, st, parity, pbuf, xtwo, rev != 0, pq_parts,
+                                            npq, partials2);
+}
+
+}
diff --git a/lsbench_amd/csrc/hip_pcg.c b/lsbench_amd/csrc/hip_pcg.c
--- a/lsbench_amd/csrc/hip_pcg.c
+++ b/lsbench_amd/csrc/hip_pcg.c
@@ -17,7 +17,8 @@
     return PCG_CG1;
   if (sv->multi || s->mixed || getenv("LSBENCH_HIP_NO_FUSE_P"))
     return PCG_CLASSIC;
-  if (s->sell_form == SELL_COL && s->dinv_uniform && s->c16.tmpl.nfar >= 1 && s->c16.tmpl.nfar <= 2 &&
+  if (((s->sell_form == SELL_COL && s->dinv_uniform && s->c16.tmpl.nfar >= 1 && s->c16.tmpl.nfar <= 2) ||
+       s->sell_form == SELL_SYM) &&
       s->row_begin == 0 && s->n == s->n_glob && o->precond == LSB_PRECOND_JACOBI && !getenv("LSBENCH_HIP_NO_FUSE_PX"))
     return PCG_COL;
   return s->variant == LSB_SPMV_SUBWAVE && o->sample_spmv <= 0 ? PCG_SUBWAVE : PCG_CLASSIC;
@@ -200,16 +201,26 @@
     spmv_shard(s, buf[0], s->d_q, buf[0], s->d_parts_pq, &s->npq, s->d_st);
   } else {
     sample_open(sv, sample);
-    lsb_k_pcg_col_px(s->sp_grid, s->col.period, s->col.plan, s->col.items, s->n, &s->c16, s->d_r, buf[sv->pcur],
-                     buf[sv->pcur ^ 1], d_x,  parity == 0,
-                     s->dinv_const, s->d_parts_pq, &s->npq, s->d_st, parity ^ 1, s->d_parts2, s->np2, g_stream);
+    if (s->sell_form == SELL_SYM)
+      lsb_k_pcg_symcol_px(s->sp_grid, s->col.period, s->col.plan, s->col.items, s->n, s->sym.rec, s->sym.rs, s->d_r,
+                          buf[sv->pcur], buf[sv->pcur ^ 1], d_x, parity == 0, s->d_parts_pq, &s->npq, s->d_st, parity ^ 1,
+                          s->d_parts2, s->np2, g_stream);
+    else
+      lsb_k_pcg_col_px(s->sp_grid, s->col.period, s->col.plan, s->col.items, s->n, &s->c16, s->d_r, buf[sv->pcur],
+                       buf[sv->pcur ^ 1], d_x,  parity == 0,
+                       s->dinv_const, s->d_parts_pq, &s->npq, s->d_st, parity ^ 1, s->d_parts2, s->np2, g_stream);
     sample_close(sv, sample);
     sv->pcur ^= 1;
   }
-  lsb_k_pcg_col_r(s->sp_grid, s->col.period, s->col.plan, s->col.items, s->n, &s->c16, buf[sv->pcur], s->d_r,
-                  s->dinv_const, s->d_st,
-                  parity, sv->pcur,  parity != 0,  1,
-                  s->d_parts_pq, s->npq, s->d_parts2, &s->np2, g_stream);
+  if (s->sell_form == SELL_SYM)
+    lsb_k_pcg_symcol_r(s->sp_grid, s->col.period, s->col.plan, s->col.items, s->n, s->sym.rec, s->sym.rs, buf[sv->pcur],
+                       s->d_r, s->d_st, parity, sv->pcur, parity != 0,  1, s->d_parts_pq, s->npq, s->d_parts2,
+                       &s->np2, g_stream);
+  else
+    lsb_k_pcg_col_r(s->sp_grid, s->col.period, s->col.plan, s->col.items, s->n, &s->c16, buf[sv->pcur], s->d_r,
+                    s->dinv_const, s->d_st,
+                    parity, sv->pcur,  parity != 0,  1,
+                    s->d_parts_pq, s->npq, s->d_parts2, &s->np2, g_stream);
   if (pos & 2) {
     lsb_k_pcg_xfix(s->n, buf[0], buf[1], d_x, s->d_st, g_stream);
     lsb_k_pcg_update_p(s->n, s->d_r, DINV(s), buf[sv->pcur], buf[0], s->d_st, parity, s->d_parts2, s->np2,
diff --git a/lsbench_amd/csrc/hip_solver.c b/lsbench_amd/csrc/hip_solver.c
--- a/lsbench_amd/csrc/hip_solver.c
+++ b/lsbench_amd/csrc/hip_solver.c
@@ -297,6 +297,21 @@
   return TT;
 }
 
+static unsigned *col_plan_upload(const struct lsb_tmpl_cols *CC) {
+  const size_t nw = 16 + 4 * ((size_t)CC->nitem + 1), nd = CC->down ? ((size_t)CC->nitem + 31) / 32 : 0;
+  unsigned *plan = lsb_calloc(unsigned, nw + nd);
+  memcpy(plan, CC->xbeg, sizeof CC->xbeg);
+  memcpy(plan + 16, CC->item, 4 * (size_t)CC->nitem * sizeof(unsigned));
+  if (nd) {
+    plan[LSB_TMPL_COL_DOWN] = (unsigned)nw;
+    memcpy(plan + nw, CC->down, nd * sizeof(unsigned));
+  }
+  unsigned *d = (unsigned *)dev_upload(plan, (nw + nd) * sizeof(unsigned));
+  LSB_CHK_HIP(hipStreamSynchronize(g_stream));
+  free(plan);
+  return d;
+}
+
 static void col_build(struct shard *s, const struct lsb_sell *H, const struct lsb_sell_vc *V,
                       const struct lsb_sell_tmpls *TT) {
   struct shard_col *c = &s->col;
@@ -317,17 +332,7 @@
     char why[256];
     if (lsb_tmpl_cols_check(TT, CC, why, sizeof why))
       errx(EXIT_FAILURE, "hip_cdna4: z-column plan breaks a rule its kernel relies on: %s", why);
-    const size_t nw = 16 + 4 * ((size_t)CC->nitem + 1), nd = CC->down ? ((size_t)CC->nitem + 31) / 32 : 0;
-    unsigned *plan = lsb_calloc(unsigned, nw + nd);
-    memcpy(plan, CC->xbeg, sizeof CC->xbeg);
-    memcpy(plan + 16, CC->item, 4 * (size_t)CC->nitem * sizeof(unsigned));
-    if (nd) {
-      plan[LSB_TMPL_COL_DOWN] = (unsigned)nw;
-      memcpy(plan + nw, CC->down, nd * sizeof(unsigned));
-    }
-    unsigned *d = (unsigned *)dev_upload(plan, (nw + nd) * sizeof(unsigned));
-    LSB_CHK_HIP(hipStreamSynchronize(g_stream));
-    free(plan);
+    unsigned *d = col_plan_upload(CC);
     if (w == 0) {
       c->plan = d, c->items = CC->nitem, c->centre0 = CC->centre0, c->slices = CC->in_cols;
       c->bytes = 16ull * CC->nitem + (unsigned long long)TT->ntmpl * sizeof(struct lsb_sell_tmpl);
@@ -355,6 +360,42 @@
 static void col_free(struct shard_col *c) {
   lsb_hip_free(c->plan), lsb_hip_free(c->plan_in);
   memset(c, 0, sizeof *c);
+}
+
+static void sym_build(struct shard *s, const struct csr *G) {
+  struct shard_col *c = &s->col;
+  if (!s->sym.nxp || c->period != s->sym.nxp / LSB_SELL_ROWS || s->mixed || s->row_begin || s->n != s->n_glob ||
+      getenv("LSBENCH_HIP_NO_COL"))
+    return;
+  const char *ed = getenv("LSBENCH_HIP_SYM_DINV");
+  struct lsb_sym5 *Y = lsb_csr_sym5(G, s->sym.nxp, ed && atoi(ed));
+  struct lsb_sell_tmpls *TT = lsb_sym5_pattern(Y);
+  if (!TT) {
+    lsb_sym5_free(Y);
+    return;
+  }
+  const char *ek = getenv("LSBENCH_HIP_COL_K");
+  unsigned kauto = TT->nslice / 15000u;
+  kauto = kauto < 4u ? 4u : kauto > 16u ? 16u : kauto;
+  struct lsb_tmpl_cols *CC = lsb_sell_tmpl_columns(TT, c->period, ek ? (unsigned)atoi(ek) : kauto);
+  if (CC) {
+    char why[256];
+    if (lsb_tmpl_cols_check(TT, CC, why, sizeof why) || lsb_sym5_check(G, Y, CC, why, sizeof why))
+      errx(EXIT_FAILURE, "hip_cdna4: symmetric z-column plan breaks a rule its kernels rely on: %s", why);
+    c->plan = col_plan_upload(CC);
+    c->items = CC->nitem, c->centre0 = 1, c->slices = CC->in_cols;
+    s->sym.rs = Y->rs;
+    s->sym.rec = (double *)dev_upload(Y->rec, (size_t)Y->nrows * Y->rs * sizeof(double));
+    LSB_CHK_HIP(hipStreamSynchronize(g_stream));
+    c->bytes = 16ull * CC->nitem + 8ull * Y->rs * Y->nrows;
+    for (unsigned q = 0; q < CC->nitem; q++)
+      c->bytes += 8ull * LSB_SELL_ROWS;
+  }
+  lsb_tmpl_cols_free(CC), lsb_sell_tmpls_free(TT), lsb_sym5_free(Y);
+}
+static void sym_free(struct shard *s) {
+  lsb_hip_free(s->sym.rec);
+  s->sym.rec = NULL, s->sym.rs = 0;
 }
 
 double *shard_vec(struct shard *s, size_t count) {
@@ -418,6 +459,8 @@
     struct lsb_sell_tmpls *TT = V ? tmpl_build(s, H, V) : NULL;
     if (TT)
       col_build(s, H, V, TT);
+    else if (H)
+      sym_build(s, &G);
     LSB_CHK_HIP(hipStreamSynchronize(g_stream));
     lsb_sell_tmpls_free(TT), lsb_sell_vc_free(V), lsb_sell_free(H);
   }
@@ -505,7 +548,7 @@
 
 void shard_free(struct shard *s) {
   csr_free(&s->csr), panel_free(&s->panel), bins_free(&s->bins), tp_free(&s->tp);
-  sell32_free(&s->sell), c16_free(&s->c16), col_free(&s->col);
+  sell32_free(&s->sell), c16_free(&s->c16), col_free(&s->col), sym_free(s);
   shard_vec_free(s, s->d_dinv), shard_vec_free(s, s->d_r);
   shard_vec_free(s, s->d_q), shard_vec_free(s, s->d_pfull), lsb_hip_free(s->d_parts_pq);
   shard_vec_free(s, s->d_p1), shard_vec_free(s, s->d_s1), shard_vec_free(s, s->d_r1);
@@ -620,12 +663,17 @@
   double dir_seconds = 0.0;
   struct lsb_skyinv *dirW = o.krylov == LSB_KRYLOV_DIRECT ? direct_factor(S, &o, &dir_height, &dir_seconds) : NULL;
   int *padmap = NULL;
+  unsigned sym_nxp = 0;
   {
     const char *e = getenv("LSBENCH_HIP_PAD_LINES");
     const int want = e ? atoi(e) : (S->nrows >= 1000000u ? 1 : 0);
     if (want && !o.reorder && o.krylov != LSB_KRYLOV_DIRECT) {
       unsigned nx = 0, nxp = 0;
       struct csr *Sp = lsb_csr_pad_lines(S, LSB_SELL_ROWS, &nx, &nxp, &padmap);
+      const char *es = getenv("LSBENCH_HIP_SYM_COL");
+      if (!Sp && es && atoi(es) && o.nvirt <= 1 && o.precision == LSB_PREC_FP64 &&
+          (Sp = lsb_csr_pad_lines_sym(S, LSB_SELL_ROWS, &nx, &nxp, &padmap)) != NULL)
+        sym_nxp = nxp;
       if (Sp) {
         if (o.verbose)
           fprintf(stderr, "hip_cdna4: grid lines of %u rows padded to %u (%u -> %u rows)\n", nx, nxp, S->nrows,
@@ -666,6 +714,7 @@
   lsb_csr_partition_rows(S, (unsigned)P, bounds);
   unsigned *hull = lsb_calloc(unsigned, 4 * (size_t)P);
   sv->sh[0].slab_bx = sv->d_perm && P == 1;
+  sv->sh[0].sym.nxp = P == 1 ? sym_nxp : 0;
   for (int q = 0; q < P; q++) {
     shard_upload(&sv->sh[q], S, bounds[q], bounds[q + 1], 0, bounds[q], S->nrows, &o);
     hull[4 * q] = bounds[q], hull[4 * q + 1] = bounds[q + 1] - bounds[q];
@@ -867,7 +916,8 @@
   if (h->variant == LSB_SPMV_TWOPHASE || h->variant == LSB_SPMV_BINNED)
     return 0;
   const unsigned long long m[] = {12ull * h->nnz + 4ull * ((unsigned long long)h->n + 1),
-                                  h->sell.bytes, h->c16.bytes, h->c16.tmpl.bytes, h->col.bytes};
+                                  h->sell.bytes, h->c16.bytes, h->c16.tmpl.bytes, h->col.bytes,
+                                  h->col.bytes};
   return m[h->sell_form] + 16ull * h->n;
 }
 int lsb_hip_solver_overlaps(const lsb_hip_solver *s) { return can_overlap(s); }
@@ -887,7 +937,14 @@
   const struct shard_col *c = &s->col;
   const int col_all = s0 == 0 && ns == s->sell.nslice;
   const int col_in = c->plan_in && s0 == s->sell.split.first && ns == s->sell.split.last - s->sell.split.first;
-  if (s->sell_form == SELL_COL && (col_all || col_in) && !s->epi.zout)
+  if (s->sell_form == SELL_SYM && col_all && !s->epi.zout)
+    lsb_k_spmv_symcol(s->sp_grid, c->period, c->plan, c->items, s->n, s->sym.rec, s->sym.rs, xfull, y, xdot, partials, np,
+                      st, &s->tail, g_stream);
+  else if (s->sell_form == SELL_SYM)
+    lsb_k_spmv_sell(LSB_SP_C16 | LSB_SP_NT, LSB_SELL_GRID, s->sp_period, s->c16.sptr, s0, ns, s->n, s->row_begin, s->n_glob,
+                    s->c16.codes, s->c16.sbase, s->c16.vals, s->c16.vconst, s->c16.ulen, xfull, y, xdot, partials, np,
+                    st, &s->tail, &s->epi, g_stream);
+  else if (s->sell_form == SELL_COL && (col_all || col_in) && !s->epi.zout)
     lsb_k_spmv_tmpl_col(s->sp_flags | f32, s->sp_grid, c->period, col_all ? c->plan : c->plan_in,
                         col_all ? c->items : c->items_in, c->centre0, s->n, s->row_begin, s->n_glob, &s->c16, xfull,
                         y, xdot, partials, np, st, &s->tail, g_stream);
@@ -962,6 +1019,7 @@
   const unsigned f = s->sp_flags;
   return s->variant != LSB_SPMV_SELL               ? SELL_NONE
          : !(f & LSB_SP_C16) || !s->c16.codes      ? SELL_32
+         : (f & LSB_SP_COL) && s->sym.rec && s->col.plan ? SELL_SYM
          : !(f & LSB_SP_TMPL) || !s->c16.tmpl.srec ? SELL_16
          : (f & LSB_SP_COL) && s->col.plan         ? SELL_COL
                                                    : SELL_TMPL;
@@ -1010,6 +1068,14 @@
       if (period) {
         CAND(LSB_SPMV_SELL, c16 | LSB_SP_NT, grid0, period);
         CAND(LSB_SPMV_SELL, c16, grid0, period);
+      }
+      if (c16 && s->sym.rec && s->col.plan) {
+        const unsigned f = c16 | LSB_SP_NT | LSB_SP_TMPL | LSB_SP_COL;
+        if (o->spmv_grid <= 0) {
+          CAND(LSB_SPMV_SELL, f, 512, 0);
+          CAND(LSB_SPMV_SELL, f, LSB_SYM_COL_GRID, 0);
+        } else
+          CAND(LSB_SPMV_SELL, f, grid0, 0);
       }
       if (c16 && s->c16.tmpl.srec) {
         const unsigned f = c16 | LSB_SP_NT | LSB_SP_TMPL;
@@ -1078,7 +1144,7 @@
   if (!(sell && (bf & LSB_SP_C16)))
     c16_free(&s->c16);
   if (!(sell && (bf & LSB_SP_COL)))
-    col_free(&s->col);
+    col_free(&s->col), sym_free(s);
   if (any && !(sell && !(bf & LSB_SP_C16)))
     sell32_free(&s->sell);
 }
diff --git a/lsbench_amd/csrc/hip_solver.h b/lsbench_amd/csrc/hip_solver.h
--- a/lsbench_amd/csrc/hip_solver.h
+++ b/lsbench_amd/csrc/hip_solver.h
@@ -54,7 +54,7 @@
   unsigned first, last;
   int ok;
 };
-enum { SELL_NONE, SELL_32, SELL_16, SELL_TMPL, SELL_COL };
+enum { SELL_NONE, SELL_32, SELL_16, SELL_TMPL, SELL_COL, SELL_SYM };
 enum pcg_form {
   PCG_NONE,
   PCG_CLASSIC,
@@ -133,6 +133,11 @@
     unsigned long long slices;
     unsigned long long bytes;
   } col;
+  struct shard_sym {
+    unsigned nxp;
+    unsigned rs;
+    double *rec;
+  } sym;
   double *d_dinv, *d_r, *d_q, *d_pfull;
   double *d_p1, *d_s1;
   unsigned npq, np2;
diff --git a/lsbench_amd/csrc/lsb_impl.h b/lsbench_amd/csrc/lsb_impl.h
--- a/lsbench_amd/csrc/lsb_impl.h
+++ b/lsbench_amd/csrc/lsb_impl.h
@@ -135,6 +135,17 @@
                      const struct lsb_sell16_dev *c, const double *p, double *r, double dc, struct lsb_pcg_state *st,
                      int parity, int pbuf, int xtwo, int rev, const double *pq_parts, unsigned npq, double *partials2,
                      unsigned *npartials, void *stream);
+void lsb_k_spmv_symcol(unsigned grid_cap, unsigned period, const unsigned *plan, unsigned nitem, unsigned n,
+                       const double *rec, unsigned rs, const double *x, double *y, const double *xdot, double *partials,
+                       unsigned *npartials, const struct lsb_pcg_state *st, const struct lsb_ar_tail *tail, void *stream);
+void lsb_k_pcg_symcol_px(unsigned grid_cap, unsigned period, const unsigned *plan, unsigned nitem, unsigned n,
+                         const double *rec, unsigned rs, const double *r, const double *pold, double *pnew, double *x,
+                         int xupd, double *partials, unsigned *npartials, struct lsb_pcg_state *st, int parity,
+                         const double *parts2, unsigned nparts2, void *stream);
+void lsb_k_pcg_symcol_r(unsigned grid_cap, unsigned period, const unsigned *plan, unsigned nitem, unsigned n,
+                        const double *rec, unsigned rs, const double *p, double *r, struct lsb_pcg_state *st, int parity,
+                        int pbuf, int xtwo, int rev, const double *pq_parts, unsigned npq, double *partials2,
+                        unsigned *npartials, void *stream);
 void lsb_k_pcg_xfix(unsigned n, const double *p0, const double *p1, double *x, const struct lsb_pcg_state *st,
                     void *stream);
 #define LSB_SP_COL 256u
diff --git a/lsbench_amd/csrc/lsb_operator.c b/lsbench_amd/csrc/lsb_operator.c
--- a/lsbench_amd/csrc/lsb_operator.c
+++ b/lsbench_amd/csrc/lsb_operator.c
@@ -87,7 +87,15 @@
   return S;
 }
 
-struct csr *lsb_csr_pad_lines(const struct csr *S, unsigned slice, unsigned *nx_out, unsigned *nxp_out, int **map_out) {
+static int sym_partner(const struct csr *S, unsigned c, unsigned r, const double *v) {
+  for (unsigned k = S->offs[c]; k < S->offs[c + 1]; k++)
+    if (S->cols[k] == r)
+      return !memcmp(&S->vals[k], v, sizeof(double));
+  return 0;
+}
+
+static struct csr *pad_lines(const struct csr *S, unsigned slice, int sym, unsigned *nx_out, unsigned *nxp_out,
+                             int **map_out) {
   if (!S || S->base != 0 || slice < 2 || S->nrows < 4 * slice)
     return NULL;
   const unsigned n = S->nrows;
@@ -95,7 +103,7 @@
   for (unsigned r = 0; r < n && !nx; r++)
     if (S->offs[r + 1] > S->offs[r] && S->cols[S->offs[r + 1] - 1] > r + 1)
       nx = S->cols[S->offs[r + 1] - 1] - r;
-  if (nx < 2 * slice || n % nx || n / nx < 3)
+  if (nx < 2 * slice || n % nx || n / nx < (sym ? 8u : 3u))
     return NULL;
   const unsigned ny = n / nx, nxp = (nx + slice - 1) / slice * slice;
   if (nxp == nx || (unsigned long long)(nxp - nx) * 16 > nx || (unsigned long long)ny * nxp > 0x7fffffffull)
@@ -109,7 +117,11 @@
       const int w = d == -(long long)nx ? 0 : d == -1 ? 1 : d == 0 ? 2 : d == 1 ? 3 : d == (long long)nx ? 4 : -1;
       if (w < 0 || (w == 1 && r % nx == 0) || (w == 3 && r % nx == nx - 1))
         return NULL;
-      if (!have[w])
+      if (sym) {
+        if (S->vals[k] == 0.0 || S->vals[k] != S->vals[k] || (w != 2 && !sym_partner(S, S->cols[k], r, &S->vals[k])))
+          return NULL;
+        have[w] = 1;
+      } else if (!have[w])
         val[w] = S->vals[k], have[w] = 1;
       else if (memcmp(&val[w], &S->vals[k], sizeof(double)))
         return NULL;
@@ -118,8 +130,10 @@
     if (!diag)
       return NULL;
   }
-  if (!have[0] || !have[1] || !have[3] || !have[4] || val[2] == 0.0)
-    return NULL;
+  if (!have[0] || !have[1] || !have[3] || !have[4] || (!sym && val[2] == 0.0))
+    return NULL;
+  if (sym)
+    val[0] = val[1] = val[3] = val[4] = 0.0, val[2] = 1.0;
   const unsigned np = ny * nxp;
   const unsigned long long cap = (unsigned long long)S->offs[n] + 5ull * (unsigned long long)ny * (nxp - nx);
   if (cap > 0xffffffffull)
@@ -142,14 +156,14 @@
         }
       } else {
         map[row] = -1;
-        if (j > 0)
+        if (j > 0 && !sym)
           Pd->cols[at] = row - nxp, Pd->vals[at] = val[0], at++;
-        if (i > nx)
+        if (i > nx && !sym)
           Pd->cols[at] = row - 1, Pd->vals[at] = val[1], at++;
         Pd->cols[at] = row, Pd->vals[at] = val[2], at++;
-        if (i + 1 < nxp)
+        if (i + 1 < nxp && !sym)
           Pd->cols[at] = row + 1, Pd->vals[at] = val[3], at++;
-        if (j + 1 < ny)
+        if (j + 1 < ny && !sym)
           Pd->cols[at] = row + nxp, Pd->vals[at] = val[4], at++;
       }
     }
@@ -163,6 +177,136 @@
   else
     free(map);
   return Pd;
+}
+
+struct csr *lsb_csr_pad_lines(const struct csr *S, unsigned slice, unsigned *nx_out, unsigned *nxp_out, int **map_out) {
+  return pad_lines(S, slice, 0, nx_out, nxp_out, map_out);
+}
+
+struct csr *lsb_csr_pad_lines_sym(const struct csr *S, unsigned slice, unsigned *nx_out, unsigned *nxp_out,
+                                  int **map_out) {
+  return pad_lines(S, slice, 1, nx_out, nxp_out, map_out);
+}
+
+struct lsb_sym5 *lsb_csr_sym5(const struct csr *Sp, unsigned nxp, int with_dinv) {
+  if (!Sp || Sp->base != 0 || !nxp || nxp % LSB_SELL_ROWS || nxp / LSB_SELL_ROWS < 8 || Sp->nrows % nxp ||
+      Sp->nrows / nxp < 3)
+    return NULL;
+  const unsigned n = Sp->nrows, rs = with_dinv ? 4u : 3u;
+  struct lsb_sym5 *Y = lsb_calloc(struct lsb_sym5, 1);
+  Y->nrows = n, Y->nslice = n / LSB_SELL_ROWS, Y->period = nxp / LSB_SELL_ROWS, Y->rs = rs;
+  Y->rec = lsb_calloc(double, (size_t)n * rs + 1);
+  for (unsigned r = 0; r < n; r++) {
+    double *R = Y->rec + (size_t)(r / LSB_SELL_ROWS) * rs * LSB_SELL_ROWS + r % LSB_SELL_ROWS;
+    int diag = 0;
+    for (unsigned k = Sp->offs[r]; k < Sp->offs[r + 1]; k++) {
+      const unsigned c = Sp->cols[k];
+      const double v = Sp->vals[k];
+      int ok = v != 0.0 && v == v;
+      if (c == r)
+        R[0] = v, diag = 1;
+      else if (c == r + 1 && r % nxp != nxp - 1)
+        R[LSB_SELL_ROWS] = v, ok = ok && sym_partner(Sp, c, r, &v);
+      else if (c == r + nxp && c < n)
+        R[2 * LSB_SELL_ROWS] = v, ok = ok && sym_partner(Sp, c, r, &v);
+      else if ((r >= 1 && c == r - 1 && r % nxp != 0) || (r >= nxp && c == r - nxp))
+        ok = ok && sym_partner(Sp, c, r, &v);
+      else
+        ok = 0;
+      if (!ok) {
+        lsb_sym5_free(Y);
+        return NULL;
+      }
+    }
+    if (!diag) {
+      lsb_sym5_free(Y);
+      return NULL;
+    }
+    if (with_dinv)
+      R[3 * LSB_SELL_ROWS] = 1.0 / R[0];
+  }
+  return Y;
+}
+
+void lsb_sym5_free(struct lsb_sym5 *Y) {
+  if (!Y)
+    return;
+  free(Y->rec), free(Y);
+}
+
+struct lsb_sell_tmpls *lsb_sym5_pattern(const struct lsb_sym5 *Y) {
+  if (!Y || Y->nslice < 3 * Y->period)
+    return NULL;
+  struct lsb_sell_tmpls *T = lsb_calloc(struct lsb_sell_tmpls, 1);
+  const unsigned ns = Y->nslice;
+  T->nslice = ns, T->ntmpl = 1, T->nfar = 1;
+  T->tid = lsb_calloc(unsigned char, (size_t)ns + 8);
+  T->vbase = lsb_calloc(unsigned, 2 * ((size_t)ns + 8));
+  T->mask = lsb_calloc(unsigned long long, 2);
+  T->t = lsb_calloc(struct lsb_sell_tmpl, 1);
+  const int P = (int)(Y->period * LSB_SELL_ROWS);
+  const int base[5] = {-P, -1, 0, 1, P};
+  T->t[0].nslots = 5, T->t[0].shaped = 1;
+  for (int j = 0; j < LSB_TMPL_SLOTS; j++)
+    T->t[0].base[j] = j < 5 ? base[j] : 0, T->t[0].kidx[j] = -1;
+  for (unsigned s = 0; s < ns; s++)
+    T->tid[s] = s >= Y->period && s + Y->period < ns ? 0 : 255;
+  T->covered = T->shaped = ns - 2ull * Y->period;
+  T->kept_read = 0;
+  return T;
+}
+
+int lsb_sym5_check(const struct csr *Sp, const struct lsb_sym5 *Y, const struct lsb_tmpl_cols *C, char *why,
+                   size_t whylen) {
+#define SY_FAIL(code, ...)                                                                     \
+  do {                                                                                         \
+    if (why && whylen)                                                                         \
+      snprintf(why, whylen, __VA_ARGS__);                                                      \
+    return code;                                                                               \
+  } while (0)
+  if (!Sp || !Y || !Y->rec || Sp->base != 0)
+    SY_FAIL(1, "no operator or no records");
+  const unsigned n = Sp->nrows, rs = Y->rs, P = Y->period * LSB_SELL_ROWS;
+  if (Y->nrows != n || (rs != 3 && rs != 4) || Y->period < 8 || n % P || n / P < 3 || Y->nslice != n / LSB_SELL_ROWS)
+    SY_FAIL(2, "%u rows in %u slices, lines of %u slices, %u numbers per row", n, Y->nslice, Y->period, rs);
+#define SY_AT(r, w) Y->rec[(size_t)((r) / LSB_SELL_ROWS) * rs * LSB_SELL_ROWS + (size_t)(w) * LSB_SELL_ROWS + (r) % LSB_SELL_ROWS]
+  unsigned long long want = 0;
+  for (unsigned r = 0; r < n; r++) {
+    const double d = SY_AT(r, 0), e = SY_AT(r, 1), nv = SY_AT(r, 2);
+    if (d == 0.0 || d != d)
+      SY_FAIL(3, "row %u: diagonal %g", r, d);
+    if (e != 0.0 && r % P == P - 1)
+      SY_FAIL(4, "row %u: an east value at the end of its line", r);
+    if (nv != 0.0 && r + P >= n)
+      SY_FAIL(5, "row %u: a north value on the last line", r);
+    if (rs == 4) {
+      const double q = 1.0 / d;
+      if (memcmp(&q, &SY_AT(r, 3), sizeof q))
+        SY_FAIL(6, "row %u: inverse diagonal %a, 1 / d is %a", r, SY_AT(r, 3), q);
+    }
+    want += 1u + 2u * (e != 0.0) + 2u * (nv != 0.0);
+    for (unsigned k = Sp->offs[r]; k < Sp->offs[r + 1]; k++) {
+      const unsigned c = Sp->cols[k];
+      const double *have = c == r ? &SY_AT(r, 0) : c == r + 1 ? &SY_AT(r, 1) : c == r + P ? &SY_AT(r, 2)
+                           : r >= 1 && c == r - 1 ? &SY_AT(c, 1) : r >= P && c == r - P ? &SY_AT(c, 2) : NULL;
+      if (!have || Sp->vals[k] == 0.0 || memcmp(have, &Sp->vals[k], sizeof(double)))
+        SY_FAIL(7, "row %u: entry in column %u is %a, the records say %a", r, c, Sp->vals[k], have ? *have : 0.0);
+    }
+  }
+  if (want != Sp->offs[n])
+    SY_FAIL(8, "the records stand for %llu entries, the operator holds %u", want, Sp->offs[n]);
+  for (unsigned i = 0; C && i < C->nitem; i++) {
+    const unsigned s = C->item[4 * (size_t)i], run = C->item[4 * (size_t)i + 1] & ~LSB_TMPL_COL_LOCKSTEP;
+    if (run < 1 || (unsigned long long)s + (unsigned long long)(run - 1) * Y->period >= Y->nslice)
+      SY_FAIL(9, "item %u: %u slices from slice %u of %u", i, run, s, Y->nslice);
+    if (run >= 2 && (s < Y->period || (unsigned long long)s + (unsigned long long)run * Y->period >= Y->nslice))
+      SY_FAIL(10, "item %u: a column of %u slices from slice %u reaches the first or last line", i, run, s);
+  }
+  if (C && (C->period != Y->period || C->s_lo != 0 || C->s_hi != Y->nslice))
+    SY_FAIL(11, "plan of slices [%u, %u), lines of %u slices", C->s_lo, C->s_hi, C->period);
+  return 0;
+#undef SY_AT
+#undef SY_FAIL
 }
 
 struct csr *lsb_csr_row_slice(const struct csr *A, unsigned r0, unsigned r1) {
```

New measurement: 1.141. 1.5% lower.
